# StuLiu/RegDA

Measured on AMD Instinct MI355X. Metric: src+tgt 512x512 image-pairs/sec (SSL step), higher is better.
Workload: dtype bf16; 1 GPU; st.regda.2potsdam SSL step, resnet101 DeepLabV2(PPM), batch 8+8 512x512 per GPU, online EMA teacher; global_batch=8, parallelism=dp1

## Files before the change

### include/rgda_hip.h

```cpp
#ifndef RGDA_HIP_H
#define RGDA_HIP_H

#include <stddef.h>
#include <stdint.h>

#ifdef __cplusplus
extern "C" {
#endif

#define RGDA_ABI_VERSION 10
#define RGDA_STAT_REPLICAS 8
#define RGDA_STAT_FRAC_FWD 26
#define RGDA_STAT_FRAC_BWD 40
typedef int64_t rgda_stat_t;
#define RGDA_LAYOUT_TILE 64

typedef void* rgda_stream_t;

enum rgda_status {
    RGDA_OK = 0,
    RGDA_ERR_ARG = -1,
    RGDA_ERR_WORKSPACE = -2,
    RGDA_ERR_LAUNCH = -3,
    RGDA_ERR_UNSUPPORTED = -4
// ... 5 lines not shown
size_t rgda_class_lds_limit(int which);
const char* rgda_strerror(int status);


size_t rgda_pseudo_select_workspace(int b, int c);
int rgda_pseudo_select(const float* soft, int64_t* out, int b, int c, int hw, float cutoff_top,
                       float cutoff_low, int ignore_label, int classmax_ready, void* ws,
                       size_t ws_bytes, rgda_stream_t stream);

size_t rgda_lrh_workspace(int b, int max_regions, int class_num);
int rgda_lrh(const int64_t* labels, const int64_t* regions, int64_t* out, int b, int hw,
             int class_num, int ignore_label, float percent, int max_regions, void* ws,
             size_t ws_bytes, rgda_stream_t stream);

size_t rgda_pseudo_lrh_workspace(int b, int hw, int max_regions, int class_num);
int rgda_pseudo_lrh(const float* soft, const float* classmax, const int64_t* regions, int64_t* out, int b, int hw,
                    int class_num, float cutoff_top, float cutoff_low, int ignore_label, float percent,
                    int max_regions, void* ws, size_t ws_bytes, rgda_stream_t stream);

int rgda_masks_to_regions(const uint8_t* masks, const int64_t* areas, int32_t* regions, int K, int64_t HW,
                          int64_t area_threshold, rgda_stream_t stream);

size_t rgda_label_refine_workspace(int b, int c, int h, int w);
size_t rgda_label_refine_classmax_offset(int b, int c, int h, int w);
int rgda_label_refine(const float* feat, const float* protos, const float* p1, const float* p2,
                      const float* soft, float* out, int b, int k, int c, int h, int w, int H,
                      int W, float temp, void* ws, size_t ws_bytes, rgda_stream_t stream);
int rgda_label_refine_views(const float* feat, const float* protos, const float* p1, const float* p2,
                            const float* soft, float* out, int b, int k, int c, int h, int w, int H,
                            int W, float temp, int views, void* ws, size_t ws_bytes,
                            rgda_stream_t stream);

size_t rgda_label_refine_sup_workspace(int b, int c, int h, int w, int max_regions);
size_t rgda_label_refine_sup_flag_offset(int b, int c, int h, int w, int max_regions);
int rgda_label_refine_sup(const float* feat, const float* protos, const float* p1, const float* p2,
                          const float* soft, const int64_t* label_t_sup, float* out, int b, int k, int c,
                          int h, int w, int H, int W, float temp, int views, int max_regions, void* ws,
                          size_t ws_bytes, rgda_stream_t stream);

size_t rgda_proto_update_workspace(int c, int k);
int rgda_proto_update(const float* feat, const int64_t* label, float* protos, int64_t* label_ds,
                      int b, int k, int c, int h, int w, int scale, int ignore_label,
                      float min_ratio, float decay, void* ws, size_t ws_bytes,
                      rgda_stream_t stream);
int rgda_proto_stats(const float* feat, const int64_t* label, int64_t* label_ds, int b, int k, int c,
                     int h, int w, int scale, int ignore_label, float min_ratio, void* stats,
                     size_t stats_bytes, rgda_stream_t stream);
int rgda_proto_apply(float* protos, const void* stats, int c, int k, float decay, rgda_stream_t stream);

size_t rgda_upsample_ce_workspace(int b, int c, int h, int w, int H, int W);
int rgda_upsample_ce(const float* p1, const float* p2, const int64_t* label,
                     const float* class_weight, float* loss, float* g1, float* g2, int b, int c,
                     int h, int w, int H, int W, int ignore_label, void* ws, size_t ws_bytes,
                     rgda_stream_t stream);

enum rgda_loss_kind {
    RGDA_LOSS_OHEM = 1,
    RGDA_LOSS_FOCAL = 2,
    RGDA_LOSS_GHM = 3,
    RGDA_LOSS_UPS = 4,
    RGDA_LOSS_UVEM = 5,
    RGDA_LOSS_GDP = 6
};
size_t rgda_upsample_loss_workspace(int kind, int b, int c, int h, int w, int H, int W);
int rgda_upsample_loss(int kind, int heads, const float* p1, const float* p2, const int64_t* label,
                       const float* soft, const float* class_weight, float* acc_sum, double m, double t, double gamma, float thresh,
                       double momentum, float* loss, float* g1, float* g2, int b, int c, int h, int w, int H,
                       int W, int ignore_label, void* ws, size_t ws_bytes, rgda_stream_t stream);

size_t rgda_upsample_gdp_workspace(int b, int c, int h, int w, int H, int W);
int rgda_upsample_gdp(int heads, const float* p1, const float* p2, const int64_t* label,
                      const float* pixel_weight, const float* class_weight, float* acc_sum, float* bins_weight,
                      double momentum, float* loss, float* g1, float* g2, int b, int c, int h, int w, int H,
                      int W, int ignore_label, void* ws, size_t ws_bytes, rgda_stream_t stream);

enum rgda_reg_term { RGDA_REG_ENT = 1, RGDA_REG_KLD = 2 };
size_t rgda_upsample_reg_workspace(int b, int c, int h, int w, int H, int W);
int rgda_upsample_reg(int heads, const float* p1, const float* p2, const int64_t* label, const float* w_ent,
                      const float* w_kld, int terms, float lambda_ent, float lambda_kld, int accumulate,
                      int empty_is_zero, float* loss, float* g1, float* g2, int b, int c, int h, int w, int H, int W,
                      int ignore_label, void* ws, size_t ws_bytes, rgda_stream_t stream);

#define RGDA_IAST_BINS 0x7C01
size_t rgda_iast_workspace(int n, int c, int H, int W);
int rgda_iast_hist(const float* probs, int n, int c, int H, int W, void* ws, size_t ws_bytes, rgda_stream_t stream);
int rgda_iast_percentile(const double* prepend, const double* q, float* out, int c, const void* ws, size_t ws_bytes,
                         rgda_stream_t stream);
int rgda_iast_label(const double* cls_thresh, uint8_t* label, int n, int c, int H, int W, const void* ws,
                    size_t ws_bytes, rgda_stream_t stream);

#define RGDA_ANALYSIS_MAX_BINS 256
size_t rgda_pseudo_analysis_workspace(int b, int c, int R);
int rgda_pseudo_analysis(const float* soft, const int64_t* gt, const float* lo, const float* hi, int b, int c, int H, int W,
                         int R, float cutoff_top, float cutoff_low, int ignore_label, void* tables, size_t tables_bytes,
                         rgda_stream_t stream);
size_t rgda_pseudo_analysis_fold_workspace(int c, int R);
int rgda_pseudo_analysis_fold(const void* tables, size_t tables_bytes, int b, int c, int R, void* state, size_t state_bytes,
                              rgda_stream_t stream);

size_t rgda_proto_pixel_weight_workspace(int b, int c, int k, int h, int w);
int rgda_proto_pixel_weight(const float* feat, const float* protos, const float* sim, const int64_t* label,
                            float* out, int b, int k, int c, int h, int w, int H, int W, int ignore_label,
                            void* ws, size_t ws_bytes, rgda_stream_t stream);

int rgda_teacher_probs(const float* p1, const float* p2, float* probs, int b, int c, int h, int w,
                       int H, int W, rgda_stream_t stream);

int rgda_class_count(const int64_t* label, int32_t* cnt, int64_t n, int c, rgda_stream_t stream);


int rgda_conv2d(const void* x, int ldx, const void* wgt, void* y, int ldy, const void* res,
                int ldres, const uint8_t* res_relu_mask, rgda_stat_t* stats, int stat_groups, int N, int H, int W,
                int Cin, int Ho, int Wo, int Cout, int kh, int kw, int stride, int pad, int dil, int mode,
                rgda_stream_t stream);

typedef struct rgda_conv2d_desc {
    const void* x; const void* wgt; void* y; const void* res; const uint8_t* res_relu_mask; rgda_stat_t* stats;
    int ldx, ldy, ldres, stat_groups;
    int N, H, W, Cin, Ho, Wo, Cout, kh, kw, stride, pad, dil, mode;
} rgda_conv2d_desc;
int rgda_conv2d_grouped(const rgda_conv2d_desc* descs, int n, rgda_stream_t stream);
int rgda_conv2d_grouped_launches(const rgda_conv2d_desc* descs, int n);

int rgda_conv2d_bneval(const void* x, int ldx, const void* wgt, void* y, int ldy, const void* res, int ldres,
                       const float* running_mean, const float* running_var, const float* gamma,
                       const float* beta, float eps, int relu, int N, int H, int W, int Cin, int Ho, int Wo,
                       int Cout, int kh, int kw, int stride, int pad, int dil, rgda_stream_t stream);

int rgda_conv2d_bnbwd(const void* x, int ldx, const void* wgt, void* y, int ldy, const void* res, int ldres,
                      const uint8_t* res_relu_mask, rgda_stat_t* sums, int groups, const void* bn_y, int bn_ldy, const uint8_t* bn_relu_mask,
                      const void* bn_x, int bn_ldx,
                      const float* bn_mi, const float* bn_nscale, int rows_per_image, int relu,
                      const float* bn_gamma, const float* bn_beta, int N, int H,
                      int W, int Cin, int Ho, int Wo, int Cout, int kh, int kw, int stride, int pad, int dil,
                      int mode, rgda_stream_t stream);

typedef struct rgda_bn_operand {
    const rgda_stat_t* stats;
    const float* gamma;
    const float* beta;
    float* mi;
    float* running_mean;
    float* running_var;
    int64_t* num_batches_tracked;
    float eps, momentum;
    int groups;
    int relu;
} rgda_bn_operand;
int rgda_conv2d_bnin_supported(int64_t M, int Cout, int Cin, int kh, int kw, int stride, int pad, int dil, int H, int W,
                               int Ho, int Wo, int groups);
int rgda_conv2d_bnin(const rgda_bn_operand* bn_in, const void* x, int ldx, const void* wgt, void* y, int ldy,
                     const void* res, int ldres, rgda_stat_t* stats, int stat_groups, int N, int H, int W, int Cin,
                     int Ho, int Wo, int Cout, int kh, int kw, int stride, int pad, int dil, rgda_stream_t stream);

const char* rgda_conv2d_kernel(int variant, int N, int H, int W, int Cin, int Ho, int Wo, int Cout, int kh, int kw,
                               int stride, int pad, int dil, int mode, int has_stats, int stat_groups);

int rgda_conv2d_tile(int64_t M, int Cout, int kh, int kw, int Cin, int rows_per_group);

int rgda_conv2d_wgrad(const void* x, int ldx, const void* dy, int lddy, float* dw, int N, int H,
                      int W, int Cin, int Ho, int Wo, int Cout, int kh, int kw, int stride,
                      int pad, int dil, void* ws, size_t ws_bytes, rgda_stream_t stream);

typedef struct rgda_wgrad_desc {
    const void* x;
    const void* dy;
    float* dw;
    int ldx, lddy;
    int N, H, W, Cin, Ho, Wo, Cout, kh, kw, stride, pad, dil;
    int lddw, co_split;
} rgda_wgrad_desc;
size_t rgda_conv2d_wgrad_workspace(const rgda_wgrad_desc* descs, int n);
const char* rgda_conv2d_wgrad_kernel(const rgda_wgrad_desc* desc);
int rgda_conv2d_wgrad_grouped(const rgda_wgrad_desc* descs, int n, void* ws, size_t ws_bytes, rgda_stream_t stream);

int rgda_stem_im2col(const float* img, void* col, int N, int H, int W, int Ho, int Wo, int Kp,
                     rgda_stream_t stream);

int rgda_stem_conv(const float* img, const void* wgt, void* y, int ldy, rgda_stat_t* stats, int stat_groups, int N,
                   int H, int W, int Ho, int Wo, rgda_stream_t stream);
int rgda_stem_conv_bneval(const float* img, const void* wgt, void* y, int ldy, const float* running_mean,
                          const float* running_var, const float* gamma, const float* beta, float eps, int relu,
                          int N, int H, int W, int Ho, int Wo, rgda_stream_t stream);

int rgda_bn_stats(const void* x, int ldx, rgda_stat_t* stats, int64_t M, int C, rgda_stream_t stream);
int rgda_bn_finalize(const rgda_stat_t* stats, float* mi, float* running_mean, float* running_var,
                     int64_t* num_batches_tracked, int64_t M, int C, int groups, float eps,
                     float momentum, rgda_stream_t stream);
int rgda_bn_apply(const void* x, int ldx, const float* mi, const float* gamma, const float* beta,
                  const void* res, int ldres, const float* nscale, int rows_per_image, void* y,
                  int ldy, int64_t M, int C, int relu, int groups, rgda_stream_t stream);
int rgda_bn_train_apply(const void* x, int ldx, const rgda_stat_t* stats, float* mi, float* running_mean,
                        float* running_var, int64_t* num_batches_tracked, const float* gamma,
                        const float* beta, const void* res, int ldres, const float* nscale,
                        int rows_per_image, void* y, int ldy, uint8_t* relu_mask, int64_t M, int C, int relu,
                        int groups, float eps, float momentum, rgda_stream_t stream);
int rgda_bn_bwd_reduce(const void* g, int ldg, const void* y, int ldy, const uint8_t* relu_mask, const void* x,
                       int ldx, const float* mi, const float* nscale, int rows_per_image, rgda_stat_t* sums,
                       int64_t M, int C, int relu, const float* gamma, const float* beta, int groups,
                       rgda_stream_t stream);
int rgda_bn_bwd_apply(const void* g, int ldg, const void* y, int ldy, const uint8_t* relu_mask, const void* x,
                      int ldx, const float* mi, const float* gamma, const float* nscale,
                      int rows_per_image, const rgda_stat_t* sums, void* dx, int lddx, void* gmask,
                      int ldgm, float* dgamma, float* dbeta, int64_t M, int C, int relu, const float* beta,
                      void* act_out, int ldact, int groups, rgda_stream_t stream);

typedef struct rgda_bn_small_fwd_desc {
    const void* x; void* y; uint8_t* relu_mask; const float* gamma; const float* beta; float* mi;
    float* running_mean; float* running_var; int64_t* num_batches_tracked;
    int64_t M; int ldx, ldy, C, groups, relu; float eps, momentum;
} rgda_bn_small_fwd_desc;
typedef struct rgda_bn_small_bwd_desc {
    const void* g; const void* y; const uint8_t* relu_mask; const void* x; void* dx; const float* mi; const float* gamma;
    float* dgamma; float* dbeta;
    int64_t M; int ldg, ldy, ldx, lddx, C, groups, relu;
} rgda_bn_small_bwd_desc;
int rgda_bn_train_small(const rgda_bn_small_fwd_desc* descs, int n, rgda_stream_t stream);
int rgda_bn_bwd_small(const rgda_bn_small_bwd_desc* descs, int n, rgda_stream_t stream);

int rgda_maxpool_fwd(const void* x, void* y, uint8_t* idx, int N, int H, int W, int C, int Ho,
                     int Wo, rgda_stream_t stream);
int rgda_maxpool_bwd(const void* gy, const uint8_t* idx, void* gx, int N, int H, int W, int C,
                     int Ho, int Wo, rgda_stream_t stream);
int rgda_maxpool_fwd_bnin(const rgda_bn_operand* bn_in, const void* x, void* y, uint8_t* idx, int N, int H, int W,
                          int C, int Ho, int Wo, rgda_stream_t stream);

int rgda_instnorm_fwd(const void* x, int ldx, void* y0, void* y1, int ldy, float* feat_nchw,
                      float* mi, int N, int HW, int C, float eps, rgda_stream_t stream);
int rgda_instnorm_bwd(const void* ga, const void* gb, int ldg, const void* gc, int ldgc,
                      const void* x, int ldx, const float* mi, void* dx, int lddx, int N, int HW,
                      int C, rgda_stream_t stream);

int rgda_spatial_mix(const void* in, int ldin, const float* Mx, void* out, int ldout, int N, int I,
                     int J, int C, int accumulate, int out_f32, rgda_stream_t stream);

int rgda_spatial_mix_multi(int nsrc, const void* const* ins, const int* ldins, const float* const* mats,
                           const int* Js, void* out, int ldout, int N, int I, int C, rgda_stream_t stream);

int rgda_classifier_fwd(const void* hidden, int ldh, const float* w, const float* bias,
                        float* logits, int N, int HW, int C, int ncls, rgda_stream_t stream);
size_t rgda_classifier_bwd_workspace(int64_t M, int C, int ncls);
int rgda_classifier_bwd(const void* hidden, int ldh, const float* w, const float* glogits,
                        void* dhidden, int lddh, float* dw, float* db, int N, int HW, int C,
                        int ncls, void* ws, size_t ws_bytes, rgda_stream_t stream);


int rgda_sumsq(const float* g, int64_t n, float* out, float* ws, rgda_stream_t stream);

int rgda_sgd_step(float* p, const float* g, float* v, float* shadow, void* p_bf16, void* shadow_bf16,
                  const float* gnorm_sq, const float* lr_dev, int64_t n, float momentum,
                  float weight_decay, float max_norm, float gscale, float ema_decay,
                  int first_step, rgda_stream_t stream);

size_t rgda_stem_wgrad_workspace(int N, int H, int W);
int rgda_stem_wgrad(const float* img, const void* dy, int lddy, float* dw, void* ws, size_t ws_bytes, int N, int H,
                    int W, int Ho, int Wo, rgda_stream_t stream);

int rgda_weight_transpose_bf16(const float* w, void* wt, int Co, int T, int Ci, rgda_stream_t stream);
int rgda_weight_transpose_batched(const int64_t* table, int n, int64_t total_blocks, rgda_stream_t stream);
int rgda_cast_bf16(const float* src, void* dst, int64_t n, rgda_stream_t stream);
int rgda_cast_f32(const void* src_bf16, float* dst, int64_t n, rgda_stream_t stream);
int rgda_ddp_accumulate_bf16(const void* recv, int world, void* out, int64_t shard_elems, rgda_stream_t stream);

typedef void* rgda_comm_t;
#define RGDA_COMM_ID_BYTES 128
#define RGDA_COMM_F32 0
#define RGDA_COMM_BF16 1
#define RGDA_COMM_I64 2
#define RGDA_COMM_F64 3
int rgda_comm_unique_id(void* id_128_bytes);
int rgda_comm_init(const void* id_128_bytes, int rank, int world, rgda_comm_t* comm);
int rgda_comm_destroy(rgda_comm_t comm);
int rgda_comm_all_reduce(rgda_comm_t comm, void* buf, int64_t n, int dtype, rgda_stream_t stream);
int rgda_comm_all_gather(rgda_comm_t comm, const void* send, void* recv, int64_t n_per_rank, int dtype,
                         rgda_stream_t stream);
int rgda_comm_all_to_all(rgda_comm_t comm, const void* send, void* recv, int64_t n_per_rank, int dtype,
                         rgda_stream_t stream);
int rgda_pad_cast_bf16(const float* src, void* dst, int R, int K, int Kp, rgda_stream_t stream);
int rgda_unpad_acc_f32(const float* src, float* dst, int R, int K, int Kp, rgda_stream_t stream);
int rgda_fill_zero(void* p, size_t bytes, rgda_stream_t stream);
int rgda_copy_multi(int n, void* const* dsts, const void* const* srcs, const size_t* bytes, rgda_stream_t stream);
int rgda_set_f32(float* p, float value, rgda_stream_t stream);
int rgda_dropout_mask(float* out, int64_t n, float p, uint64_t seed, rgda_stream_t stream);
int rgda_add_bf16(const void* a, int lda, const void* b, int ldb, void* out, int ldo, int64_t M,
                  int C, rgda_stream_t stream);


int rgda_dihedral_nchw(const float* src, float* dst, int N, int C, int Hs, int Ws, int hflip, int rot_k,
                       int flip_first, float scale, int accumulate, rgda_stream_t stream);

int rgda_pad_rows_nchw(const float* src, float* dst, int N, int C, int h, int w, int top, int bottom,
                       rgda_stream_t stream);
int rgda_window_crop(const float* full, float* tile, int N, int C, int Hf, int Wf, int y1, int x1, int h, int w,
                     int Th, int Tw, rgda_stream_t stream);
int rgda_window_accumulate(const float* tile, float* full, float* count, int N, int C, int Hf, int Wf, int y1,
                           int x1, int h, int w, int Th, int Tw, rgda_stream_t stream);
int rgda_window_normalise(float* full, const float* count, int N, int C, int Hf, int Wf, rgda_stream_t stream);

int rgda_window_gather(const float* src_f32, const uint8_t* src_u8, const float* lut, const int32_t* windows, int K,
                       int views, int n, int C, int H, int W, int Th, int Tw, float* out, int* flag,
                       rgda_stream_t stream);
int rgda_window_scatter(const float* pred, const int32_t* windows, int K, int views, int n, int C, int H, int W, int Th,
                        int Tw, int row0, int rows, float* full, float* count, int* flag, rgda_stream_t stream);
int rgda_window_finish(float* full, const float* count, int n, int C, int H, int W, uint8_t* labels_u8,
                       int64_t* labels_i64, const int64_t* y_true, int64_t* cm, int* flag, rgda_stream_t stream);

// ... 193 lines not shown
```

### regda_amd/csrc/common.h

```cpp
#pragma once
#include <hip/hip_runtime.h>
#include <stdint.h>

#include "../../include/rgda_hip.h"

#define RGDA_CHECK_LAUNCH()                                   \
    do {                                                      \
        if (hipGetLastError() != hipSuccess) return RGDA_ERR_LAUNCH; \
    } while (0)

typedef unsigned short bf16_t;
typedef __attribute__((ext_vector_type(8))) __bf16 bf16x8;
typedef __attribute__((ext_vector_type(8))) unsigned short u16x8;
typedef __attribute__((ext_vector_type(4))) unsigned short u16x4;
typedef __attribute__((ext_vector_type(4))) short s16x4;
typedef __attribute__((ext_vector_type(16))) float f32x16;
typedef __attribute__((ext_vector_type(4))) float f32x4;

typedef __attribute__((ext_vector_type(2))) __bf16 bf16x2_t;
typedef __attribute__((ext_vector_type(2))) float f32x2_t;
static __device__ __forceinline__ float bf2f(bf16_t h) { return __uint_as_float(((unsigned)h) << 16); }
static __device__ __forceinline__ unsigned pack2bf(float lo, float hi) {
    f32x2_t v = {lo, hi};
    bf16x2_t b = __builtin_convertvector(v, bf16x2_t);
    return __builtin_bit_cast(unsigned, b);
}
static __device__ __forceinline__ bf16_t f2bf(float f) { return (bf16_t)(pack2bf(f, 0.f) & 0xffffu); }

static __device__ __forceinline__ float wave_sum(float v) {
#pragma unroll
    for (int o = 32; o > 0; o >>= 1) v += __shfl_xor(v, o, 64);
    return v;
}
template <int O>
static __device__ __forceinline__ float xor_add(float v) {
    static_assert(O == 8 || O == 16 || O == 32, "xor_add: 8, 16 or 32");
    const unsigned u = __float_as_uint(v);
    if constexpr (O == 8) {
        return v + __uint_as_float((unsigned)__builtin_amdgcn_update_dpp(0, (int)u, 0x128 , 0xf, 0xf, false));
    } else if constexpr (O == 16) {
        auto r = __builtin_amdgcn_permlane16_swap(u, u, false, false);
        return __uint_as_float(r[0]) + __uint_as_float(r[1]);
    } else {
        auto r = __builtin_amdgcn_permlane32_swap(u, u, false, false);
        return __uint_as_float(r[0]) + __uint_as_float(r[1]);
    }
}

struct Lerp {
    int i0, i1;
    float l0, l1;
};
static __device__ __forceinline__ Lerp lerp_ac(int dst, int in, int out) {
    float scale = (out > 1) ? __fdiv_rn((float)(in - 1), (float)(out - 1)) : 0.f;
    float src = __fmul_rn(scale, (float)dst);
    Lerp r;
    r.i0 = (int)src;
    r.i1 = r.i0 + ((r.i0 < in - 1) ? 1 : 0);
    r.l1 = __fsub_rn(src, (float)r.i0);
    r.l0 = __fsub_rn(1.f, r.l1);
    return r;
}

static __device__ __forceinline__ float wave_max(float v) {
#pragma unroll
    for (int o = 32; o > 0; o >>= 1) v = fmaxf(v, __shfl_xor(v, o, 64));
    return v;
}

#define NREP RGDA_STAT_REPLICAS

#define RGDA_STAT_POISON (3ll << 60)
static __device__ __forceinline__ long long stat_fix(float v, int frac) {
    const float x = ldexpf(v, frac);
    if (!(fabsf(x) < 0x1p59f)) return RGDA_STAT_POISON;
    const float hi = truncf(x * 0x1p-31f);
    const float lo = x - hi * 0x1p31f;
    return ((long long)__float2int_rz(hi) << 31) + (long long)__float2int_rn(lo);
}
static __device__ __forceinline__ void stat_add(rgda_stat_t* p, float v, int frac) {
    atomicAdd((unsigned long long*)p, (unsigned long long)stat_fix(v, frac));
}
static __device__ __forceinline__ double stat_total(const rgda_stat_t* __restrict__ st, int C, int c, int which, int frac) {
    __int128 t = 0;
#pragma unroll
    for (int r = 0; r < NREP; ++r) t += st[(size_t)(2 * r + which) * C + c];
    if (t >= (__int128)(1ll << 59) || t <= -(__int128)(1ll << 59)) return (double)__builtin_nan("");
    return (double)(long long)t * (1.0 / (double)(1ll << frac));
}

static __device__ __forceinline__ void stat_moments(const rgda_stat_t* __restrict__ st, int C, int c, double invM, float eps,
                                                    float& mean, float& var, float& istd) {
    const double m = stat_total(st, C, c, 0, RGDA_STAT_FRAC_FWD) * invM;
    double v = stat_total(st, C, c, 1, RGDA_STAT_FRAC_FWD) * invM - m * m;
    if (v < 0.0) v = 0.0;
    mean = (float)m;
    var = (float)v;
    istd = 1.f / sqrtf((float)v + eps);
}

struct BnOperand {
    const rgda_stat_t* stats;
    const float* gamma;
    const float* beta;
    float* mi;
    float* rm;
    float* rv;
    long long* nbt;
    float eps, mom;
    int groups, relu, C;
    int rows_per_group;
};
static __device__ __forceinline__ void bn_scale_shift(float mean, float istd, float gamma, float beta, float& sc, float& sh) {
    sc = gamma * istd;
    sh = __builtin_fmaf(-mean, sc, beta);
}
static __device__ __forceinline__ float bn_affine(float x, float sc, float sh) { return __builtin_fmaf(x, sc, sh); }
typedef float f32x2v __attribute__((ext_vector_type(2)));
static __device__ __forceinline__ uint4 bn_operand8(uint4 v, const float (&sc)[8], const float (&sh)[8], bool relu) {
    unsigned w[4] = {v.x, v.y, v.z, v.w};
#pragma unroll
    for (int e = 0; e < 4; ++e) {
        f32x2v x = {__uint_as_float(w[e] << 16), __uint_as_float(w[e] & 0xffff0000u)};
        f32x2v s = {sc[2 * e], sc[2 * e + 1]}, h = {sh[2 * e], sh[2 * e + 1]};
        f32x2v f = __builtin_elementwise_fma(x, s, h);
        if (relu) { f.x = fmaxf(f.x, 0.f); f.y = fmaxf(f.y, 0.f); }
        w[e] = pack2bf(f.x, f.y);
    }
    return uint4{w[0], w[1], w[2], w[3]};
}
template <int NT>
static __device__ __forceinline__ void bn_operand_table(const BnOperand& b, int grp, bool leader, float* tab) {
    const int C = b.C;
    const double invM = 1.0 / (double)b.rows_per_group;
    for (int c = threadIdx.x; c < C; c += NT) {
        float mean, var, istd, sc, sh;
        stat_moments(b.stats + (size_t)grp * NREP * 2 * C, C, c, invM, b.eps, mean, var, istd);
        bn_scale_shift(mean, istd, b.gamma[c], b.beta[c], sc, sh);
        tab[c] = sc;
        tab[C + c] = sh;
        if (leader) {
            const float unb = (b.rows_per_group > 1) ? (float)b.rows_per_group / (float)(b.rows_per_group - 1) : 1.f;
            float rm = b.rm ? b.rm[c] : 0.f, rv = b.rm ? b.rv[c] : 0.f;
            for (int g = 0; g < b.groups; ++g) {
                float gm, gv, gi;
                stat_moments(b.stats + (size_t)g * NREP * 2 * C, C, c, invM, b.eps, gm, gv, gi);
                if (b.mi) { b.mi[(size_t)g * 2 * C + c] = gm; b.mi[(size_t)g * 2 * C + C + c] = gi; }
                rm = (1.f - b.mom) * rm + b.mom * gm;
                rv = (1.f - b.mom) * rv + b.mom * gv * unb;
            }
            if (b.rm) { b.rm[c] = rm; b.rv[c] = rv; }
            if (c == 0 && b.nbt) *b.nbt += b.groups;
        }
    }
}

#include <stdlib.h>
#ifdef RGDA_TUNING
#define TUNE_ENV(name) getenv(name)
#else
#define TUNE_ENV(name) ((const char*)nullptr)
#endif
static inline hipStream_t to_stream(rgda_stream_t s) { return (hipStream_t)s; }
static inline int zero_bytes(void* p, size_t bytes, rgda_stream_t stream) {
    if (!((uintptr_t)p & 15)) return rgda_fill_zero(p, bytes, stream);
    return hipMemsetAsync(p, 0, bytes, (hipStream_t)stream) == hipSuccess ? RGDA_OK : RGDA_ERR_LAUNCH;
}
static inline int cdiv(long long a, long long b) { return (int)((a + b - 1) / b); }

#include <type_traits>
#define RGDA_MIN_CLASSES 6
#define RGDA_MAX_CLASSES 16
static inline bool class_count_ok(int c) { return c >= RGDA_MIN_CLASSES && c <= RGDA_MAX_CLASSES; }
size_t loss_row_lds_bytes(int c, int w, int W, bool want);
size_t pcl_lds_bytes(int C, int K);
size_t refine_lds_bytes(int C, int k);
#define RGDA_LOSS_ROW_LDS_MAX ((size_t)150 * 1024)
#define RGDA_LDS_MAX ((size_t)160 * 1024)
template <int LO = RGDA_MIN_CLASSES, int HI = RGDA_MAX_CLASSES, class F>
static inline int with_classes(int c, F&& f) {
    if constexpr (LO > HI) {
        return RGDA_ERR_UNSUPPORTED;
    } else {
        if (c == LO) return f(std::integral_constant<int, LO>{});
        return with_classes<LO + 1, HI>(c, f);
    }
}
```

### regda_amd/csrc/conv_kernels.hip

```cpp
#include <stdio.h>
#include <stdlib.h>
#include <string.h>

#include "common.h"
#include <type_traits>
#include <vector>

struct ConvArgs {
    const bf16_t* x;
    const bf16_t* w;
    bf16_t* y;
    const bf16_t* res;
    rgda_stat_t* stats;
    int ldx, ldy, ldres;
    int N, H, W, Cin, Ho, Wo, Cout, KH, KW, stride, pad, dil, mode;
    int M;
    int tiles_c, tiles_p;
    int rows_per_group;
    int howo_shift, wo_shift;
    unsigned long long* dbg;
    int tpw;
    int skip;
    const unsigned char* res_mask;
    const bf16_t* bn_y;
    const unsigned char* bn_mask;
    const bf16_t* bn_x;
    const float* bn_mi;
    const float* bn_nscale;
    int bn_ldy, bn_ldx, bn_rpi, bn_relu;
    const float* ev_rm;
    const float* ev_rv;
    const float* ev_gamma;
    const float* ev_beta;
    float ev_eps;
    int ev_relu;
    const float* bn_gamma;
    const float* bn_beta;
    BnOperand xf;
};

#ifdef RGDA_TUNING
#define TDBG(a) ((a).dbg)
#define TSKIP(a) ((a).skip)
#else
#define TDBG(a) ((unsigned long long*)nullptr)
#define TSKIP(a) 0
#endif

static __device__ __forceinline__ int xcd_remap(int bid, int nwg) {
    int q = nwg >> 3, r = nwg & 7, xcd = bid & 7, k = bid >> 3;
    return (xcd < r ? xcd * (q + 1) : r * (q + 1) + (xcd - r) * q) + k;
}

static __device__ __forceinline__ void src_coord(int mode, int base, int t, int dil, int stride, int lim, int& out,
                                                 bool& ok) {
    if (mode == 0) {
        out = base + t * dil;
        ok = (out >= 0) && (out < lim);
    } else {
        int th = base - t * dil;
        ok = th >= 0;
        if (stride == 1) {
            out = th;
        } else {
            ok = ok && (th % stride == 0);
            out = th / stride;
        }
        ok = ok && (out < lim);
    }
}

#define LDS_PTR(p) ((__attribute__((address_space(3))) void*)(p))
#define WAIT_VMCNT(n) asm volatile("s_waitcnt vmcnt(%0)" ::"n"(n) : "memory")

typedef __attribute__((ext_vector_type(4))) int i32x4;
static __device__ __forceinline__ i32x4 dma_rsrc(const void* base, unsigned bytes) {
    const unsigned long long b = (unsigned long long)base;
    i32x4 r = {(int)(unsigned)b, (int)((unsigned)(b >> 32) & 0xffffu), (int)bytes, 0x00020000};
    return r;
}
static __device__ __forceinline__ void dma16_to_lds(i32x4 rsrc, const unsigned char* lds_dst, int voffset, int soffset) {
    const unsigned m0 = (unsigned)(__UINTPTR_TYPE__)LDS_PTR(lds_dst);
    asm volatile("s_mov_b32 m0, %0\n\ts_nop 0\n\tbuffer_load_dwordx4 %1, %2, %3 offen lds"
                 :: "s"(m0), "v"(voffset), "s"(rsrc), "s"(soffset) : "memory");
}


enum { EPI_PLAIN = 0, EPI_STATS, EPI_RES, EPI_RES_STATS, EPI_EV, EPI_BNX, EPI_BNX2 };
typedef float f32x2 __attribute__((ext_vector_type(2)));
typedef __attribute__((ext_vector_type(4))) unsigned u32x4r;
#define RGDA_BNIN_MAX_C 512
static __device__ __forceinline__ f32x2 bf2f_pair(unsigned u) {
    f32x2 r;
    r.x = __uint_as_float(u << 16);
    r.y = __uint_as_float(u & 0xffff0000u);
    return r;
}
static __device__ __forceinline__ unsigned pack2bf(f32x2 v) { return pack2bf(v.x, v.y); }

struct EpiParams { f32x2 k0[4], k1[4], k2[4], k3[4]; };
template <int KIND>
static __device__ __forceinline__ void epilogue_params(const ConvArgs& a, int m0, int co, bool cok, EpiParams& P) {
#pragma unroll
    for (int e = 0; e < 4; ++e) {
        P.k0[e] = f32x2{0.f, 0.f}; P.k1[e] = f32x2{0.f, 0.f};
        P.k2[e] = f32x2{0.f, 0.f}; P.k3[e] = f32x2{0.f, 0.f};
    }
    constexpr bool BNX = KIND == EPI_BNX || KIND == EPI_BNX2;
    if (BNX && cok) {
        const float* mi = a.bn_mi + (size_t)(m0 / a.rows_per_group) * 2 * a.Cout + co;
#pragma unroll
        for (int e = 0; e < 4; ++e) {
            P.k1[e] = f32x2{mi[2 * e], mi[2 * e + 1]};
            P.k0[e] = f32x2{mi[a.Cout + 2 * e], mi[a.Cout + 2 * e + 1]};
        }
        if constexpr (KIND == EPI_BNX2) {
#pragma unroll
            for (int e = 0; e < 8; ++e) {
                float sc, sh;
                bn_scale_shift(P.k1[e >> 1][e & 1], P.k0[e >> 1][e & 1], a.bn_gamma[co + e], a.bn_beta[co + e], sc, sh);
                P.k2[e >> 1][e & 1] = sc;
                P.k3[e >> 1][e & 1] = sh;
            }
        }
    }
    if (KIND == EPI_EV && cok) {
#pragma unroll
        for (int e = 0; e < 8; ++e) {
            const float sc = a.ev_gamma[co + e] / sqrtf(a.ev_rv[co + e] + a.ev_eps);
            P.k0[e >> 1][e & 1] = sc;
            P.k1[e >> 1][e & 1] = a.ev_beta[co + e] - a.ev_rm[co + e] * sc;
        }
    }
}

template <int WMAP>
static __device__ __forceinline__ int tile_row(const ConvArgs& a, int row) {
    return WMAP ? ((row >> 5) * a.W + (row & 31)) : row;
}
template <int BC, int BP, int NT, int KIND, bool FULL = false, int WMAP = 0>
static __device__ __forceinline__ void epilogue_rows(const ConvArgs& a, const unsigned char* smem, int m0, int c0,
                                                     float (&s)[8], float (&q)[8], const EpiParams* pre = nullptr) {
    constexpr int CSTR = BC * 2 + 16;
    constexpr int VPR = BC / 8, RPP = NT / VPR, NIT = BP / RPP;
    constexpr int CH = NIT < 4 ? NIT : 4;
    static_assert(NIT % CH == 0, "row passes");
    const int t = threadIdx.x;
    const int cv = t % VPR, rr = t / VPR;
    const int co = c0 + cv * 8;
    const bool cok = FULL || co < a.Cout;
    EpiParams P;
    if (pre) P = *pre; else epilogue_params<KIND>(a, m0, co, cok, P);
    f32x2 (&k0)[4] = P.k0, (&k1)[4] = P.k1, (&k2)[4] = P.k2, (&k3)[4] = P.k3;
    f32x2 s2[4], q2[4];
#pragma unroll
    for (int e = 0; e < 4; ++e) { s2[e] = f32x2{s[2 * e], s[2 * e + 1]}; q2[e] = f32x2{q[2 * e], q[2 * e + 1]}; }
    constexpr bool BNX = KIND == EPI_BNX || KIND == EPI_BNX2;
    const bool has_res = (KIND == EPI_RES || KIND == EPI_RES_STATS) || ((KIND == EPI_EV || BNX) && a.res);
    const bool res_gate = (KIND != EPI_EV) && has_res && a.res_mask;
    constexpr bool STATS = KIND == EPI_STATS || KIND == EPI_RES_STATS;
#pragma unroll
    for (int p0 = 0; p0 < NIT; p0 += CH) {
        uint4 val[CH], rv[CH], xv[CH], yv[CH];
        unsigned rmb[CH], bmb[CH];
        bool ok[CH];
#pragma unroll
        for (int i = 0; i < CH; ++i) {
            const int row = rr + (p0 + i) * RPP;
            const int m = m0 + tile_row<WMAP>(a, row);
            ok[i] = FULL || (cok && m < a.M);
            val[i] = *(const uint4*)(smem + row * CSTR + cv * 16);
            rv[i] = uint4{0u, 0u, 0u, 0u}; xv[i] = rv[i]; yv[i] = rv[i]; rmb[i] = 0xffu; bmb[i] = 0xffu;
            if (ok[i]) {
                if (has_res) {
                    rv[i] = *(const uint4*)(a.res + (size_t)m * a.ldres + co);
                    if (res_gate) rmb[i] = a.res_mask[(size_t)m * (a.Cout >> 3) + (co >> 3)];
                }
                if (BNX) {
                    xv[i] = *(const uint4*)(a.bn_x + (size_t)m * a.bn_ldx + co);
                    if (KIND == EPI_BNX && a.bn_relu) {
                        if (a.bn_mask) bmb[i] = a.bn_mask[(size_t)m * (a.Cout >> 3) + (co >> 3)];
                        else yv[i] = *(const uint4*)(a.bn_y + (size_t)m * a.bn_ldy + co);
                    }
                }
            }
        }
#pragma unroll
        for (int i = 0; i < CH; ++i) {
            const int m = m0 + tile_row<WMAP>(a, rr + (p0 + i) * RPP);
            const unsigned vw[4] = {val[i].x, val[i].y, val[i].z, val[i].w};
            const unsigned rw[4] = {rv[i].x, rv[i].y, rv[i].z, rv[i].w};
            unsigned ow[4];
            if (KIND == EPI_PLAIN || KIND == EPI_STATS) {
#pragma unroll
                for (int e = 0; e < 4; ++e) ow[e] = vw[e];
            } else if (KIND == EPI_EV) {
#pragma unroll
                for (int e = 0; e < 4; ++e) {
                    f32x2 f = bf2f_pair(vw[e]) * k0[e] + k1[e];
                    if (has_res) f += bf2f_pair(rw[e]);
                    if (a.ev_relu) { f.x = fmaxf(f.x, 0.f); f.y = fmaxf(f.y, 0.f); }
                    ow[e] = pack2bf(f);
                }
            } else {
#pragma unroll
                for (int e = 0; e < 4; ++e) {
                    unsigned r = rw[e];
                    if (res_gate) {
                        const unsigned b0 = (rmb[i] >> (2 * e)) & 1u, b1 = (rmb[i] >> (2 * e + 1)) & 1u;
                        r &= (b0 ? 0x0000ffffu : 0u) | (b1 ? 0xffff0000u : 0u);
                    }
                    ow[e] = has_res ? pack2bf(bf2f_pair(vw[e]) + bf2f_pair(r)) : vw[e];
                }
            }
            if (ok[i]) {
                if (STATS) {
#pragma unroll
                    for (int e = 0; e < 4; ++e) {
                        const f32x2 f = bf2f_pair(ow[e]);
                        s2[e] += f;
                        q2[e] += f * f;
                    }
                }
                if (BNX) {
                    const unsigned xw[4] = {xv[i].x, xv[i].y, xv[i].z, xv[i].w};
                    const unsigned yw[4] = {yv[i].x, yv[i].y, yv[i].z, yv[i].w};
                    f32x2 ns[4];
#pragma unroll
                    for (int e = 0; e < 4; ++e) ns[e] = f32x2{1.f, 1.f};
                    if (a.bn_nscale) {
                        const float* np = a.bn_nscale + (size_t)(m / a.bn_rpi) * a.Cout + co;
#pragma unroll
                        for (int e = 0; e < 4; ++e) ns[e] = f32x2{np[2 * e], np[2 * e + 1]};
                    }
#pragma unroll
                    for (int e = 0; e < 4; ++e) {
                        f32x2 g = bf2f_pair(ow[e]);
                        if constexpr (KIND == EPI_BNX2) {
                            const f32x2 xx = bf2f_pair(xw[e]);
                            g.x = (bn_affine(xx.x, k2[e].x, k3[e].x) > 0.f) ? g.x : 0.f;
                            g.y = (bn_affine(xx.y, k2[e].y, k3[e].y) > 0.f) ? g.y : 0.f;
                        } else if (a.bn_relu) {
                            if (a.bn_mask) {
                                g.x = ((bmb[i] >> (2 * e)) & 1u) ? g.x : 0.f;
                                g.y = ((bmb[i] >> (2 * e + 1)) & 1u) ? g.y : 0.f;
                            } else {
                                const f32x2 yy = bf2f_pair(yw[e]);
                                g.x = (yy.x > 0.f) ? g.x : 0.f;
                                g.y = (yy.y > 0.f) ? g.y : 0.f;
                            }
                        }
                        if (a.bn_nscale) g *= ns[e];
                        s2[e] += g;
                        q2[e] += g * ((bf2f_pair(xw[e]) - k1[e]) * k0[e]);
                    }
                }
                if (!(TSKIP(a) & 128)) *(uint4*)(a.y + (size_t)m * a.ldy + co) = uint4{ow[0], ow[1], ow[2], ow[3]};
            }
        }
    }
#pragma unroll
    for (int e = 0; e < 4; ++e) { s[2 * e] = s2[e].x; s[2 * e + 1] = s2[e].y; q[2 * e] = q2[e].x; q[2 * e + 1] = q2[e].y; }
}

template <int BC, int BP, int WC, int WP, bool RAW = false, int KIND = -1, int WMAP = 0>
static __device__ __forceinline__ void conv_epilogue(const ConvArgs& a, f32x16 (&acc)[BC / WC / 32][BP / WP / 32],
                                                     unsigned char* smem, int m0, int c0, float (&s)[8], float (&q)[8],
                                                     bool flush, int replica, const EpiParams* pre = nullptr) {
    constexpr int NW = WC * WP, NT = 64 * NW;
    constexpr int FI = BC / WC / 32, FJ = BP / WP / 32;
    constexpr int CSTR = BC * 2 + 16;
    const int t = threadIdx.x, lane = t & 63;
    const int wave = __builtin_amdgcn_readfirstlane(t >> 6);
    const int wc = wave % WC, wp = wave / WC;
    const int lrow = lane & 31, lk = lane >> 5;
#pragma unroll
    for (int i = 0; i < FI; ++i)
#pragma unroll
        for (int j = 0; j < FJ; ++j) {
            int px = wp * (BP / WP) + j * 32 + lrow;
#pragma unroll
            for (int g = 0; g < 4; ++g) {
                int co = wc * (BC / WC) + i * 32 + 8 * g + 4 * lk;
                uint2 pk;
                pk.x = pack2bf(acc[i][j][4 * g + 0], acc[i][j][4 * g + 1]);
                pk.y = pack2bf(acc[i][j][4 * g + 2], acc[i][j][4 * g + 3]);
                *(uint2*)(smem + px * CSTR + co * 2) = pk;
            }
        }
    if constexpr (RAW) {
        asm volatile("s_waitcnt lgkmcnt(0)" ::: "memory");
        __builtin_amdgcn_s_barrier();
    } else {
        __syncthreads();
    }
    if (TDBG(a) && t == 0) TDBG(a)[(16384 + blockIdx.x) * 4 + 0] = __builtin_readcyclecounter();
    constexpr int VPR = BC / 8;
    const int cv = t % VPR;
    if constexpr (KIND >= 0) epilogue_rows<BC, BP, NT, KIND, RAW, WMAP>(a, smem, m0, c0, s, q, pre);
    else if (a.ev_rm) epilogue_rows<BC, BP, NT, EPI_EV, false, WMAP>(a, smem, m0, c0, s, q);
    else if (a.bn_x) {
        if (a.bn_relu == 2) epilogue_rows<BC, BP, NT, EPI_BNX2, false, WMAP>(a, smem, m0, c0, s, q);
        else epilogue_rows<BC, BP, NT, EPI_BNX, false, WMAP>(a, smem, m0, c0, s, q);
    }
    else if (a.res) {
        if (a.stats) epilogue_rows<BC, BP, NT, EPI_RES_STATS, false, WMAP>(a, smem, m0, c0, s, q);
        else epilogue_rows<BC, BP, NT, EPI_RES, false, WMAP>(a, smem, m0, c0, s, q);
    } else if (a.stats) epilogue_rows<BC, BP, NT, EPI_STATS, false, WMAP>(a, smem, m0, c0, s, q);
    else epilogue_rows<BC, BP, NT, EPI_PLAIN, false, WMAP>(a, smem, m0, c0, s, q);
    if (TDBG(a) && t == 0) TDBG(a)[(16384 + blockIdx.x) * 4 + 1] = __builtin_readcyclecounter();
    if (a.stats && flush) {
#pragma unroll
        for (int e = 0; e < 8; ++e) {
            if constexpr (VPR <= 8) { s[e] = xor_add<8>(s[e]); q[e] = xor_add<8>(q[e]); }
            if constexpr (VPR <= 16) { s[e] = xor_add<16>(s[e]); q[e] = xor_add<16>(q[e]); }
            if constexpr (VPR <= 32) { s[e] = xor_add<32>(s[e]); q[e] = xor_add<32>(q[e]); }
        }
        float* red = (float*)(smem + BP * CSTR);
        if (lane < VPR) {
#pragma unroll
            for (int e = 0; e < 8; ++e) {
                red[(wave * 2 + 0) * BC + cv * 8 + e] = s[e];
                red[(wave * 2 + 1) * BC + cv * 8 + e] = q[e];
            }
        }
        asm volatile("s_waitcnt lgkmcnt(0)" ::: "memory");
        __builtin_amdgcn_s_barrier();
        if (TDBG(a) && t == 0) TDBG(a)[(16384 + blockIdx.x) * 4 + 2] = __builtin_readcyclecounter();
        if (t < 2 * BC) {
            int which = t / BC, c = t % BC;
            float tot = 0.f;
#pragma unroll
            for (int wv = 0; wv < NW; ++wv) tot += red[(wv * 2 + which) * BC + c];
            if (c0 + c < a.Cout) {
                rgda_stat_t* dst = &a.stats[(((size_t)(m0 / a.rows_per_group) * NREP + replica) * 2 + which) * a.Cout + c0 + c];
#ifdef RGDA_TUNING
                if (TSKIP(a) & 16) {}
                else if (TSKIP(a) & 32) atomicAdd((float*)dst, tot);
                else
#endif
                stat_add(dst, tot, a.bn_x ? RGDA_STAT_FRAC_BWD : RGDA_STAT_FRAC_FWD);
            }
        }
    }
}

template <int BC, int BP, int STAGES, int WC, int WP, bool PIPE, bool XF>
static __device__ __forceinline__ void conv_igemm_body(const ConvArgs& a, const int bid) {
#if defined(__HIP_DEVICE_COMPILE__)
    constexpr int NW = WC * WP;
    constexpr int FI = BC / WC / 32, FJ = BP / WP / 32;
    constexpr int WL = BC / (NW * 8), XL = BP / (NW * 8);
    constexpr int LD = WL + XL;
    constexpr int TILE = (BC + BP) * 128;
    constexpr int CSTR = BC * 2 + 16;
    constexpr int EPI = BP * CSTR + NW * BC * 2 * 4;
    constexpr int SMEM = (STAGES * TILE > EPI) ? STAGES * TILE : EPI;
    constexpr int XFTAB = XF ? RGDA_BNIN_MAX_C * 2 * 4 : 0;
    static_assert(!XF || (STAGES == 2 && !PIPE), "the operand-transform loop is written for the 2-stage ring");
    __shared__ __attribute__((aligned(256))) unsigned char smem[SMEM + XFTAB];

    const int t = threadIdx.x, lane = t & 63;
    const int wave = __builtin_amdgcn_readfirstlane(t >> 6);
    const int wc = wave % WC, wp = wave / WC;
    const int logical = xcd_remap(bid, a.tiles_c * a.tiles_p);
    const int c0 = (logical % a.tiles_c) * BC;
    const int m0 = (logical / a.tiles_c) * BP;
    const int taps = a.KH * a.KW;
    const int lrow8 = lane >> 3, lslot = lane & 7;
    constexpr int OOB = (int)0x80000000;
    const __amdgpu_buffer_rsrc_t rs_w = __builtin_amdgcn_make_buffer_rsrc(
        (void*)a.w, 0, (int)((size_t)a.Cout * taps * a.Cin * 2), 0x00020000);
    const __amdgpu_buffer_rsrc_t rs_x = __builtin_amdgcn_make_buffer_rsrc(
        (void*)a.x, 0, (int)((((size_t)a.N * a.H * a.W - 1) * a.ldx + a.Cin) * 2), 0x00020000);

    int xn[XL], xh[XL], xw[XL], xsw[XL];
    bool xm[XL];
#pragma unroll
    for (int i = 0; i < XL; ++i) {
        int r = (i * NW + wave) * 8 + lrow8;
        int m = m0 + r;
        xm[i] = m < a.M;
        int mm = xm[i] ? m : 0;
        int n, rem, ho, wo;
        if (a.howo_shift >= 0) { n = mm >> a.howo_shift; rem = mm & ((1 << a.howo_shift) - 1); }
        else { n = mm / (a.Ho * a.Wo); rem = mm % (a.Ho * a.Wo); }
        if (a.wo_shift >= 0) { ho = rem >> a.wo_shift; wo = rem & ((1 << a.wo_shift) - 1); }
        else { ho = rem / a.Wo; wo = rem % a.Wo; }
        xn[i] = n * a.H * a.W;
        if (a.mode == 0) { xh[i] = ho * a.stride - a.pad; xw[i] = wo * a.stride - a.pad; }
        else             { xh[i] = ho + a.pad;            xw[i] = wo + a.pad; }
        xsw[i] = XF ? lslot * 16 : (lslot ^ ((r >> 1) & 7)) * 16;
    }
    int wvo[WL];
#pragma unroll
    for (int i = 0; i < WL; ++i) {
        int r = (i * NW + wave) * 8 + lrow8;
        int co = c0 + r;
        wvo[i] = (co < a.Cout) ? (co * taps * a.Cin * 2 + (lslot ^ ((r >> 1) & 7)) * 16) : OOB;
    }

    int tap = 0, kh = 0, kw = 0, ci0 = 0;
    int xvo[XL];
    auto retap = [&]() {
#pragma unroll
        for (int i = 0; i < XL; ++i) {
            int hi, wi;
            bool okh, okw;
            src_coord(a.mode, xh[i], kh, a.dil, a.stride, a.H, hi, okh);
            src_coord(a.mode, xw[i], kw, a.dil, a.stride, a.W, wi, okw);
            xvo[i] = (xm[i] && okh && okw) ? ((xn[i] + hi * a.W + wi) * a.ldx * 2 + xsw[i]) : OOB;
        }
    };
    retap();
    auto issue = [&](int stage) {
        unsigned char* wb = smem + stage * TILE + wave * 1024;
        const int so_w = (tap * a.Cin + ci0) * 2, so_x = ci0 * 2;
#pragma unroll
        for (int i = 0; i < WL; ++i)
            __builtin_amdgcn_raw_ptr_buffer_load_lds(rs_w, LDS_PTR(wb + i * NW * 1024), 16, wvo[i], so_w, 0, 0);
        unsigned char* xb = wb + BC * 128;
#pragma unroll
        for (int i = 0; i < XL; ++i)
            __builtin_amdgcn_raw_ptr_buffer_load_lds(rs_x, LDS_PTR(xb + i * NW * 1024), 16, xvo[i], so_x, 0, 0);
    };
    auto advance = [&]() {
        ci0 += 64;
        if (ci0 >= a.Cin) {
            ci0 = 0;
            ++tap;
            if (++kw == a.KW) { kw = 0; ++kh; }
            retap();
        }
    };

    f32x16 acc[FI][FJ];
#pragma unroll
    for (int i = 0; i < FI; ++i)
#pragma unroll
        for (int j = 0; j < FJ; ++j)
#pragma unroll
            for (int r = 0; r < 16; ++r) acc[i][j][r] = 0.f;

    const int KT = taps * (a.Cin >> 6);
    unsigned long long tq0 = 0, tq1 = 0, tq2 = 0, twait = 0, tbar = 0;
    if (TDBG(a)) tq0 = __builtin_readcyclecounter();
    const int lrow = lane & 31, lk = lane >> 5;
    int stage = 0;
    if constexpr (XF) {
        float* xtab = (float*)(smem + SMEM);
        auto issue_w = [&](int st) {
            unsigned char* wb = smem + st * TILE + wave * 1024;
// ... 360 lines not shown
        for (int k = 0; k < PXW; ++k) xf_piece(0, k);
    }
    int pend = 2, wstage = 0;
    bf16x8 fa0[2][FI], fb0[2][FJ], fa1[2][FI], fb1[2][FJ];
    if constexpr (PF) {
        WAIT_VMCNT(2 * (NS - 2));
        if constexpr (XF) asm volatile("s_waitcnt lgkmcnt(0)" ::: "memory");
        __builtin_amdgcn_s_barrier();
        read_half(swb, sxb, 0, 0, fa0, fb0);
    }
    if constexpr (PF) {
      for (int sl = 0; sl < S; ++sl) {
        const bool more = sl + 1 < S;
        const unsigned char* xb = sxb + (sl & 1) * XS;
        const unsigned char* xbn = sxb + ((sl + 1) & 1) * XS;
#pragma unroll
        for (int tp = 0; tp < 9; ++tp) {
            const int q = sl * 9 + tp;
            if (!(TSKIP(a) & 2)) { if (tp >= 1 && tp - 1 < PXW) WAIT_VMCNT(2 * (NS - 3) + 1); else WAIT_VMCNT(2 * (NS - 3)); }
            if constexpr (XF) asm volatile("s_waitcnt lgkmcnt(0)" ::: "memory");
            if (!(TSKIP(a) & 4)) __builtin_amdgcn_s_barrier();
            if (!(TSKIP(a) & 1)) {
            issue_w2((tp + AH) % 9, sl + (tp + AH) / 9, wstage >= 1 ? wstage - 1 : NS - 1, q + AH < KT);
            if (tp < PXW) issue_h(sl + 1, tp, more);
            }
            if constexpr (XF) {
                if (more) {
                    if (tp == 1) xf_load(sl + 1);
                    if (tp >= 2 && tp - 2 < PXW) xf_piece(sl + 1, tp - 2);
                }
            }
            read_half(swb + wstage * WS, xb, tp, 1, fa1, fb1);
            mfma_half(fa0, fb0);
            read_half(swb + (wstage == NS - 1 ? 0 : wstage + 1) * WS, tp == 8 ? xbn : xb, tp == 8 ? 0 : tp + 1, 0, fa0, fb0);
            mfma_half(fa1, fb1);
#pragma unroll
            for (int i = 0; i < 4 * FI * FJ; ++i) {
                __builtin_amdgcn_sched_group_barrier(0x008, 1, 0);
                __builtin_amdgcn_sched_group_barrier(0x100, (FI + FJ + FI * FJ - 1) / (FI * FJ), 0);
            }
            wstage = (wstage == NS - 1) ? 0 : wstage + 1;
        }
      }
    } else {
    for (int sl = 0; sl < S; ++sl) {
        const bool more = sl + 1 < S;
        const unsigned char* xb = sxb + (sl & 1) * XS;
#pragma unroll
        for (int tp = 0; tp < 9; ++tp) {
            const int q = sl * 9 + tp;
            switch (pend) {
                case 0: WAIT_VMCNT(0); break;
                case 1: WAIT_VMCNT(1); break;
                case 2: WAIT_VMCNT(2); break;
                default: WAIT_VMCNT(3); break;
            }
            if constexpr (XF) asm volatile("s_waitcnt lgkmcnt(0)" ::: "memory");
            __builtin_amdgcn_s_barrier();
            pend = 0;
            if (!(TSKIP(a) & 1)) {
            if (q + 2 < KT) { issue_w(q + 2, wstage >= 1 ? wstage - 1 : 2); pend += 2; }
            if (more && tp < PXW) { issue_h(sl + 1, tp); pend += 1; }
            }
            if constexpr (XF) {
                if (more && !(TSKIP(a) & 512)) {
                    if (tp == 1) xf_load(sl + 1);
                    if (tp >= 2 && tp - 2 < PXW) xf_piece(sl + 1, tp - 2);
                }
            }
            const unsigned char* wb = swb + wstage * WS;
            if (!(TSKIP(a) & 8) || q == 0) {
            read_half(wb, xb, tp, 0, fa0, fb0);
            read_half(wb, xb, tp, 1, fa1, fb1);
            }
            mfma_half(fa0, fb0);
            mfma_half(fa1, fb1);
            wstage = (wstage == NS - 1) ? 0 : wstage + 1;
        }
    }
    }
    __syncthreads();
    float s[8], q8[8];
#pragma unroll
    for (int e = 0; e < 8; ++e) { s[e] = 0.f; q8[e] = 0.f; }
    conv_epilogue<BC, BP, WC, WP, false, -1, WIDE ? 1 : 0>(a, acc, smem, m0, c0, s, q8, true, blockIdx.x & (NREP - 1));
#endif
}
template <int D, int TR, bool XF = false, int NS = 3, bool PF = (NS == 4)>
__global__ void __launch_bounds__(512) conv3x3_halo_kernel(ConvArgs a) {
    conv3x3_halo_body<D, TR, XF, NS, PF, false>(a);
}
template <int D, int TR, int NS = 3, bool PF = (NS == 4), bool XF = false>
__global__ void __launch_bounds__(512) conv3x3_halo_wide_kernel(ConvArgs a) {
    conv3x3_halo_body<D, TR, XF, NS, PF, true>(a);
}

template <int KC, int BP, int WC, int WP, int KIND>
__global__ void __launch_bounds__(512) conv1x1_stream_kernel(ConvArgs a) {
#if defined(__HIP_DEVICE_COMPILE__)
    constexpr int BC = 128, NW = 8, FI = BC / WC / 32, NS = 2;
    static_assert(WC * WP == NW && BP / WP == 32, "one 32-pixel fragment column per wave");
    constexpr int XL = BP / (NW * 8);
    constexpr int SUB = BP * 128;
    constexpr int STAGE = KC * SUB;
    constexpr int CSTR = BC * 2 + 16;
    constexpr int EPI = BP * CSTR + NW * BC * 2 * 4;
    constexpr int SC = BP * BC * 2 / 16 / (64 * NW);
    __shared__ __attribute__((aligned(256))) unsigned char smem[NS * STAGE + EPI];
    unsigned char* se = smem + NS * STAGE;

    const int t = threadIdx.x, lane = t & 63;
    const int wave = __builtin_amdgcn_readfirstlane(t >> 6);
    const int wc = wave % WC, wp = wave / WC;
    const int lrow = lane & 31, lk = lane >> 5;
    const int lrow8 = lane >> 3, lslot = lane & 7;
    const int logical = xcd_remap(blockIdx.x, gridDim.x);
    const int c0 = (logical % a.tiles_c) * BC;
    const int T = a.tpw;
    const int mbase = (logical / a.tiles_c) * T * BP;

    bf16x8 fa[KC * 4][FI];
#pragma unroll
    for (int i = 0; i < FI; ++i) {
        const bf16_t* wrow = a.w + (size_t)(c0 + wc * (BC / WC) + i * 32 + lrow) * a.Cin + lk * 8;
#pragma unroll
        for (int kk = 0; kk < KC * 4; ++kk) fa[kk][i] = *(const bf16x8*)(wrow + kk * 16);
    }
#pragma unroll
    for (int i = 0; i < FI; ++i)
#pragma unroll
        for (int kk = 0; kk < KC * 4; ++kk) asm volatile("" ::"v"(fa[kk][i]));
    const i32x4 rs_x = dma_rsrc(a.x, (unsigned)((((size_t)a.M - 1) * a.ldx + a.Cin) * 2));
    int xvo[XL];
#pragma unroll
    for (int i = 0; i < XL; ++i) {
        const int r = (i * NW + wave) * 8 + lrow8;
        xvo[i] = r * a.ldx * 2 + (lslot ^ ((r >> 1) & 7)) * 16;
    }
    auto issue = [&](int tile, int stage) {
        const int so = (mbase + tile * BP) * a.ldx * 2;
#pragma unroll
        for (int kt = 0; kt < KC; ++kt)
#pragma unroll
            for (int i = 0; i < XL; ++i)
                dma16_to_lds(rs_x, smem + stage * STAGE + kt * SUB + (i * NW + wave) * 1024, xvo[i], so + kt * 128);
    };
    float s[8], q[8];
#pragma unroll
    for (int e = 0; e < 8; ++e) { s[e] = 0.f; q[e] = 0.f; }
    EpiParams P;
    epilogue_params<KIND>(a, mbase, c0 + (t % (BC / 8)) * 8, true, P);
#pragma unroll
    for (int e = 0; e < 4; ++e) asm volatile("" ::"v"(P.k0[e]), "v"(P.k1[e]), "v"(P.k2[e]), "v"(P.k3[e]));
    issue(0, 0);
    if (T > 1) { issue(1, 1); WAIT_VMCNT(XL * KC); } else WAIT_VMCNT(0);
    for (int i = 0; i < T; ++i) {
        const int stage = i & 1;
        __builtin_amdgcn_s_barrier();
        f32x16 acc[FI][1];
#pragma unroll
        for (int ii = 0; ii < FI; ++ii)
#pragma unroll
            for (int r = 0; r < 16; ++r) acc[ii][0][r] = 0.f;
        const int rb = wp * 32 + lrow;
        const unsigned char* xb = smem + stage * STAGE + rb * 128;
#pragma unroll
        for (int kt = 0; kt < KC; ++kt) {
            bf16x8 fb[4];
#pragma unroll
            for (int kk = 0; kk < 4; ++kk) fb[kk] = *(const bf16x8*)(xb + kt * SUB + (((kk * 2 + lk) ^ ((rb >> 1) & 7)) << 4));
#pragma unroll
            for (int kk = 0; kk < 4; ++kk)
#pragma unroll
                for (int ii = 0; ii < FI; ++ii)
                    acc[ii][0] = __builtin_amdgcn_mfma_f32_32x32x16_bf16(fa[kt * 4 + kk][ii], fb[kk], acc[ii][0], 0, 0, 0);
        }
        conv_epilogue<BC, BP, WC, WP, true, KIND>(a, acc, se, mbase + i * BP, c0, s, q, i + 1 == T, blockIdx.x & (NREP - 1), &P);
        __builtin_amdgcn_s_waitcnt(SC | (7 << 4) | (15 << 8));
        if (i + 2 < T && !(TSKIP(a) & 1)) issue(i + 2, stage);
    }
#endif
}

template <int TW, int KIND>
__global__ void __launch_bounds__(512) conv3x3_c64_kernel(ConvArgs a) {
#if defined(__HIP_DEVICE_COMPILE__)
    constexpr int BC = 64, BP = TW, WC = 2, WP = 4, NW = 8;
    constexpr int HP = TW + 2;
    constexpr int RI = (HP + 7) / 8;
    constexpr int SLOT = RI * 1024;
    constexpr int WBYTES = 9 * BC * 128;
    constexpr int CSTR = BC * 2 + 16;
    constexpr int EPI = BP * CSTR + NW * BC * 2 * 4;
    constexpr int SC = BP / (64 * NW / (BC / 8));
    __shared__ __attribute__((aligned(256))) unsigned char smem[WBYTES + 3 * SLOT + EPI];
    unsigned char* sw = smem;
    unsigned char* sr = smem + WBYTES;
    unsigned char* se = sr + 3 * SLOT;

    const int t = threadIdx.x, lane = t & 63;
    const int wave = __builtin_amdgcn_readfirstlane(t >> 6);
    const int wc = wave % WC, wp = wave / WC;
    const int lrow = lane & 31, lk = lane >> 5;
    const int lrow8 = lane >> 3, lslot = lane & 7;
    const int rpw = a.tpw;
    const int strip = blockIdx.x;
    const int row0 = strip * rpw;
    const int n = row0 / a.H, y0 = row0 % a.H;
    constexpr int OOB = (int)0x80000000;
    const i32x4 rs_w = dma_rsrc(a.w, 64 * 9 * 64 * 2);
    const i32x4 rs_x = dma_rsrc(a.x, (unsigned)((((size_t)a.N * a.H * a.W - 1) * a.ldx + a.Cin) * 2));
#pragma unroll
    for (int j = 0; j < 9; ++j) {
        const int r = (j * NW + wave) * 8 + lrow8;
        const int tap = r / BC, co = r % BC;
        const int vo = (co * 9 + tap) * 128 + (lslot ^ ((r >> 1) & 7)) * 16;
        dma16_to_lds(rs_w, sw + (j * NW + wave) * 1024, vo, 0);
    }
    int rvo[(RI + NW - 1) / NW];
#pragma unroll
    for (int i = 0; i < (RI + NW - 1) / NW; ++i) {
        const int q = i * NW + wave;
        const int hp = q * 8 + lrow8, ix = hp - 1;
        rvo[i] = (q < RI && hp < HP && ix >= 0 && ix < a.W) ? (ix * a.ldx * 2 + (lslot ^ ((hp >> 1) & 7)) * 16) : OOB;
    }
    auto issue_row = [&](int y) {
        const bool inside = y >= 0 && y < a.H;
        const int so = inside ? ((n * a.H + y) * a.W) * a.ldx * 2 : 0;
        unsigned char* rb = sr + ((y + 1) % 3) * SLOT;
#pragma unroll
        for (int i = 0; i < (RI + NW - 1) / NW; ++i) {
            const int q = i * NW + wave;
            if (q < RI)
                dma16_to_lds(rs_x, rb + q * 1024, inside ? rvo[i] : OOB, so);
        }
    };
    issue_row(y0 - 1);
    issue_row(y0);
    issue_row(y0 + 1);
    float s[8], q8[8];
#pragma unroll
    for (int e = 0; e < 8; ++e) { s[e] = 0.f; q8[e] = 0.f; }
    EpiParams P;
    epilogue_params<KIND>(a, row0 * BP, (t % (BC / 8)) * 8, true, P);
#pragma unroll
    for (int e = 0; e < 4; ++e) asm volatile("" ::"v"(P.k0[e]), "v"(P.k1[e]), "v"(P.k2[e]), "v"(P.k3[e]));
    WAIT_VMCNT(0);
    for (int ty = 0; ty < rpw; ++ty) {
        const int y = y0 + ty;
        __builtin_amdgcn_s_barrier();
        f32x16 acc[1][1];
#pragma unroll
        for (int r = 0; r < 16; ++r) acc[0][0][r] = 0.f;
        const int px = wp * 32 + lrow;
        const int ra = wc * 32 + lrow;
#pragma unroll
        for (int wr = 0; wr < 3; ++wr) {
            const unsigned char* rb = sr + ((y + wr) % 3) * SLOT;
            const int kh = (a.mode == 0) ? wr : 2 - wr;
#pragma unroll
            for (int kw = 0; kw < 3; ++kw) {
                const int hp = px + ((a.mode == 0) ? kw : 2 - kw);
                const unsigned char* wb = sw + (kh * 3 + kw) * (BC * 128);
#pragma unroll
                for (int kk = 0; kk < 4; ++kk) {
                    const bf16x8 fa = *(const bf16x8*)(wb + ra * 128 + (((kk * 2 + lk) ^ ((ra >> 1) & 7)) << 4));
                    const bf16x8 fb = *(const bf16x8*)(rb + hp * 128 + (((kk * 2 + lk) ^ ((hp >> 1) & 7)) << 4));
                    acc[0][0] = __builtin_amdgcn_mfma_f32_32x32x16_bf16(fa, fb, acc[0][0], 0, 0, 0);
                }
            }
            if (wr == 0) {
                asm volatile("s_waitcnt lgkmcnt(0)" ::: "memory");
                __builtin_amdgcn_s_barrier();
                if (ty + 1 < rpw) issue_row(y + 2);
            }
        }
        const int m0 = (row0 + ty) * BP;
        conv_epilogue<BC, BP, WC, WP, true, KIND>(a, acc, se, m0, 0, s, q8, ty + 1 == rpw, blockIdx.x & (NREP - 1), &P);
        __builtin_amdgcn_s_waitcnt(SC | (7 << 4) | (15 << 8));
    }
#endif
}

#ifdef RGDA_TUNING
#define TUNING_ONLY(...) __VA_ARGS__
#else
#define TUNING_ONLY(...)
#endif
#define CONV_IGEMM_ROUTES(T)                                                                                         \
    T(64, 64, 2, 2, 2, false, false) T(128, 64, 3, 2, 2, true, false) T(128, 128, 2, 2, 4, false, false)             \
    T(128, 128, 3, 2, 4, true, false) T(128, 256, 3, 2, 4, true, false) T(128, 128, 2, 2, 4, false, true)            \
    TUNING_ONLY(T(128, 128, 3, 2, 4, false, false) T(128, 256, 3, 2, 4, false, false) T(128, 64, 3, 2, 2, false, false) \
                T(128, 256, 3, 2, 2, false, false) T(256, 128, 3, 2, 2, false, false) T(128, 128, 2, 2, 2, false, false) \
                T(128, 128, 4, 2, 2, false, false) T(128, 128, 3, 2, 2, false, false) T(128, 64, 2, 2, 2, false, false) \
                T(128, 64, 4, 2, 2, false, false) T(64, 128, 3, 2, 2, false, false) T(64, 64, 4, 2, 2, false, false) \
                T(64, 64, 3, 2, 2, false, false))
#define IGEMM_ID(BC, BP, ST, WC, WP, PIPE, XF) R_IGEMM_##BC##x##BP##_##ST##_##WC##x##WP##_##PIPE##_##XF
#define IGEMM_ROUTE(BC, BP, ST, WC, WP, PIPE, XF)                                                                    \
    ROUTE(IGEMM_ID(BC, BP, ST, WC, WP, PIPE, XF), 64 * WC * WP, conv_igemm_kernel, BC, BP, ST, WC, WP, PIPE, XF)
#define PER_EPI_ROUTES(ID, KERNEL, ...)                                                                              \
    ROUTE(ID##0, 512, KERNEL, __VA_ARGS__, 0) ROUTE(ID##1, 512, KERNEL, __VA_ARGS__, 1)                              \
    ROUTE(ID##2, 512, KERNEL, __VA_ARGS__, 2) ROUTE(ID##3, 512, KERNEL, __VA_ARGS__, 3)                              \
    ROUTE(ID##4, 512, KERNEL, __VA_ARGS__, 4) ROUTE(ID##5, 512, KERNEL, __VA_ARGS__, 5)                              \
    ROUTE(ID##6, 512, KERNEL, __VA_ARGS__, 6)
#define CONV_ROUTES                                                                                                  \
    CONV_IGEMM_ROUTES(IGEMM_ROUTE)                                                                                   \
    ROUTE(R_HALO_1_4, 512, conv3x3_halo_kernel, 1, 4, false, 4, true)                                                \
    ROUTE(R_HALO_1_8, 512, conv3x3_halo_kernel, 1, 8, false, 4, true)                                                \
    ROUTE(R_HALO_2_8, 512, conv3x3_halo_kernel, 2, 8, false, 3, true)                                                \
    ROUTE(R_HALO_1_4_XF, 512, conv3x3_halo_kernel, 1, 4, true, 4, true)                                              \
    ROUTE(R_HALO_1_8_XF, 512, conv3x3_halo_kernel, 1, 8, true, 3, false)                                             \
    TUNING_ONLY(ROUTE(R_HALO_1_4_PLAIN, 512, conv3x3_halo_kernel, 1, 4, false, 3, false)                             \
                ROUTE(R_HALO_1_8_PLAIN, 512, conv3x3_halo_kernel, 1, 8, false, 3, false)                             \
                ROUTE(R_HALO_2_8_PLAIN, 512, conv3x3_halo_kernel, 2, 8, false, 3, false)                             \
                ROUTE(R_HALO_1_4_XF_PLAIN, 512, conv3x3_halo_kernel, 1, 4, true, 3, false))                          \
    ROUTE(R_HALOW_1_4, 512, conv3x3_halo_wide_kernel, 1, 4, 4, true, false)                                          \
    ROUTE(R_HALOW_1_8, 512, conv3x3_halo_wide_kernel, 1, 8, 4, true, false)                                          \
    ROUTE(R_HALOW_2_8, 512, conv3x3_halo_wide_kernel, 2, 8, 3, true, false)                                          \
    ROUTE(R_HALOW_1_4_XF, 512, conv3x3_halo_wide_kernel, 1, 4, 4, true, true)                                        \
    ROUTE(R_HALOW_1_8_XF, 512, conv3x3_halo_wide_kernel, 1, 8, 3, false, true)                                       \
    PER_EPI_ROUTES(R_C64_, conv3x3_c64_kernel, 128)                                                                  \
    PER_EPI_ROUTES(R_STREAM1_, conv1x1_stream_kernel, 1, 128, 2, 4)                                                  \
    PER_EPI_ROUTES(R_STREAM2_, conv1x1_stream_kernel, 2, 128, 2, 4)
#define ROUTE(ID, BLOCK, KERNEL, ...) ID,
enum { CONV_ROUTES CONV_ROUTE_COUNT };
#undef ROUTE
#define ROUTE(ID, BLOCK, KERNEL, ...) #KERNEL "<" #__VA_ARGS__ ">",
static const char* const CONV_ROUTE_NAMES[CONV_ROUTE_COUNT] = {CONV_ROUTES};
#undef ROUTE
constexpr int R_GROUPED = IGEMM_ID(128, 64, 3, 2, 2, true, false);

static int conv_launch(int route, const ConvArgs& a, int grid, hipStream_t st) {
    switch (route) {
#define ROUTE(ID, BLOCK, KERNEL, ...) case ID: KERNEL<__VA_ARGS__><<<grid, BLOCK, 0, st>>>(a); break;
        CONV_ROUTES
#undef ROUTE
    }
    RGDA_CHECK_LAUNCH();
    return RGDA_OK;
}

static inline int tune_int(const char* name, int dflt) { const char* e = TUNE_ENV(name); return e ? atoi(e) : dflt; }

static int conv_use_halo(long long M, int Cout, int Cin, int kh, int kw, int stride, int pad, int dil, int H, int W, int Ho,
                         int Wo, int rows_per_group) {
    if (const char* e = TUNE_ENV("RGDA_HALO")) { if (!atoi(e)) return 0; }
    if (kh != 3 || kw != 3 || stride != 1 || pad != dil || (dil != 1 && dil != 2)) return 0;
    if ((W & 31) || Wo != W || Ho != H || (Cin & 63)) return 0;
    const int min_tiles = tune_int("RGDA_HALO_MIN", 100), min8 = tune_int("RGDA_HALO_MIN8", 100);
    if ((long long)9 * Cin >= 4096 && !(H & 7) && !(rows_per_group % (8 * W)) && (M / 256) * cdiv(Cout, 128) >= min8) return 8;
    if ((long long)9 * Cin >= 2048 && dil == 1 && !(H & 3) && !(rows_per_group % (4 * W)) && (M / 128) * cdiv(Cout, 128) >= min_tiles) return 4;
    return 0;
}

struct ConvTile { int bc, bp, stages, wc, wp; bool pipe; };

static int pick_tile(long long M, int Cout, long long ktot, int rows_per_group, ConvTile& t) {
    t.bc = (Cout <= 64) ? 64 : 128;
    t.bp = 64;
    t.wc = 2;
    bool waves8 = false, ring3 = false;
    const int t82 = tune_int("RGDA_T82", 512), t83 = tune_int("RGDA_T83", 256);
    if (t.bc == 128 && ktot >= 4096 && (long long)cdiv(M, 256) * cdiv(Cout, t.bc) >= 240) { t.bp = 256; waves8 = true; }
    else if (t.bc == 128 && (long long)cdiv(M, 128) * cdiv(Cout, t.bc) >= t82) { t.bp = 128; waves8 = true; }
    else if (t.bc == 128 && (long long)cdiv(M, 128) * cdiv(Cout, t.bc) >= t83) { t.bp = 128; waves8 = ring3 = true; }
    if (rows_per_group) {
        while (t.bp > 64 && (rows_per_group % t.bp)) t.bp >>= 1;
        if (rows_per_group % t.bp) return 1;
    }
    t.wp = (waves8 && t.bp >= 128) ? 4 : 2;
    t.stages = (t.wp == 4) ? ((t.bp == 256 || ring3) ? 3 : 2) : ((t.bc == 64) ? 2 : 3);
    t.pipe = t.stages == 3 && !TUNE_ENV("RGDA_NO_PIPE");
    return 0;
}

static int igemm_route(const ConvTile& t) {
#define TILE(BC, BP, ST, WC, WP, PIPE, XF)                                                                           \
    if (!XF && t.bc == BC && t.bp == BP && t.stages == ST && t.wc == WC && t.wp == WP && t.pipe == PIPE)             \
        return IGEMM_ID(BC, BP, ST, WC, WP, PIPE, XF);
    CONV_IGEMM_ROUTES(TILE)
#undef TILE
    return -1;
}

extern "C" int rgda_conv2d_tile(int64_t M, int Cout, int kh, int kw, int Cin, int rows_per_group) {
    ConvTile t;
    if (pick_tile(M, Cout, (long long)kh * kw * Cin, rows_per_group, t)) return RGDA_ERR_UNSUPPORTED;
    return t.bc | (t.bp << 10) | ((t.wp == 4 ? 80 + t.stages : t.stages) << 20);
}

static int ilog2_exact(int v) {
    if (v <= 0 || (v & (v - 1))) return -1;
    int s = 0;
    while ((1 << s) < v) ++s;
    return s;
}
struct BnBwdFuse { const void* y; int ldy; const unsigned char* mask; const void* x; int ldx; const float* mi; const float* nscale; int rpi; int relu; const float* gamma; const float* beta; };
struct BnEvalFuse { const float* rm; const float* rv; const float* gamma; const float* beta; float eps; int relu; };
struct ConvFuse { const BnBwdFuse* bnb; const BnEvalFuse* bne; const rgda_bn_operand* bnin; };

static int conv_bnin_kind(long long M, int Cout, int Cin, int kh, int kw, int stride, int pad, int dil, int H, int W, int Ho,
                          int Wo, int groups) {
    if (groups < 1 || Ho <= 0 || Wo <= 0 || (M % ((long long)Ho * Wo)) || (M / ((long long)Ho * Wo)) % groups ||
        Cin > RGDA_BNIN_MAX_C || (Cin & 63))
        return 0;
    const int rpg = (int)(M / groups);
    if (const int tr = conv_use_halo(M, Cout, Cin, kh, kw, stride, pad, dil, H, W, Ho, Wo, rpg))
        return (tr == 4) ? 1 : (dil == 1 ? 2 : 0);
    ConvTile t;
    if (pick_tile(M, Cout, (long long)kh * kw * Cin, rpg, t)) return 0;
    return (t.bc == 128 && t.bp == 128 && t.wp == 4 && t.stages == 2) ? 3 : 0;
}

extern "C" int rgda_conv2d_bnin_supported(int64_t M, int Cout, int Cin, int kh, int kw, int stride, int pad, int dil, int H,
                                          int W, int Ho, int Wo, int groups) {
    if (!conv_bnin_kind(M, Cout, Cin, kh, kw, stride, pad, dil, H, W, Ho, Wo, groups)) return 0;
    return (Cin > 256 || (kh == 1 && Cin < 128)) ? 1 : 2;
}

static int conv_epi_kind(const ConvArgs& a) {
    return a.ev_rm ? EPI_EV : a.bn_x ? (a.bn_relu == 2 ? EPI_BNX2 : EPI_BNX)
         : a.res ? (a.stats ? EPI_RES_STATS : EPI_RES) : (a.stats ? EPI_STATS : EPI_PLAIN);
}

struct ConvPlan { ConvArgs a; int route, grid; };
static int conv_select(const rgda_conv2d_desc& d, const ConvFuse& f, ConvPlan& p) {
    const int N = d.N, H = d.H, W = d.W, Cin = d.Cin, Ho = d.Ho, Wo = d.Wo, Cout = d.Cout, kh = d.kh, kw = d.kw,
              stride = d.stride, pad = d.pad, dil = d.dil, mode = d.mode;
    const BnBwdFuse* bnb = f.bnb;
    const BnEvalFuse* bne = f.bne;
    const rgda_bn_operand* bnin = f.bnin;
    if (!d.x || !d.wgt || !d.y) return RGDA_ERR_ARG;
    if (N <= 0 || H <= 0 || W <= 0 || Ho <= 0 || Wo <= 0 || Cin <= 0 || Cout <= 0 || kh <= 0 || kw <= 0 ||
        stride <= 0 || dil <= 0 || pad < 0 || (mode != 0 && mode != 1))
        return RGDA_ERR_ARG;
    if ((Cin & 63) || (Cout & 7) || (d.ldx & 7) || (d.ldy & 7) || (d.res && (d.ldres & 7)) || d.ldx < Cin || d.ldy < Cout)
        return RGDA_ERR_ARG;
    ConvArgs& a = p.a = ConvArgs{};
    a.x = (const bf16_t*)d.x; a.w = (const bf16_t*)d.wgt; a.y = (bf16_t*)d.y; a.res = (const bf16_t*)d.res; a.stats = d.stats;
    if (d.res_relu_mask && (!d.res || bne)) return RGDA_ERR_ARG;
    a.res_mask = d.res_relu_mask;
    a.ldx = d.ldx; a.ldy = d.ldy; a.ldres = d.ldres;
    a.N = N; a.H = H; a.W = W; a.Cin = Cin; a.Ho = Ho; a.Wo = Wo; a.Cout = Cout; a.KH = kh; a.KW = kw;
    a.stride = stride; a.pad = pad; a.dil = dil; a.mode = mode;
    long long M = (long long)N * Ho * Wo;
    if (M > 0x7fffffffLL) return RGDA_ERR_ARG;
    a.M = (int)M;
    a.howo_shift = ilog2_exact(Ho * Wo);
    a.wo_shift = ilog2_exact(Wo);
    const int stat_groups = d.stat_groups < 1 ? 1 : d.stat_groups;
    if (N % stat_groups || M % stat_groups) return RGDA_ERR_ARG;
    a.rows_per_group = (int)(M / stat_groups);
    if (bnb) {
        if (!a.stats || !bnb->x || !bnb->mi || (bnb->relu == 1 && !bnb->y && !bnb->mask) || (bnb->ldx & 7) ||
            (bnb->relu == 1 && bnb->y && (bnb->ldy & 7)) || (bnb->nscale && bnb->rpi <= 0) || bnb->relu < 0 || bnb->relu > 2)
            return RGDA_ERR_ARG;
        a.bn_mask = bnb->relu == 1 ? bnb->mask : nullptr;
        a.bn_y = (const bf16_t*)bnb->y; a.bn_x = (const bf16_t*)bnb->x; a.bn_mi = bnb->mi; a.bn_nscale = bnb->nscale;
        a.bn_ldy = bnb->ldy; a.bn_ldx = bnb->ldx; a.bn_rpi = bnb->rpi; a.bn_relu = bnb->relu;
        if (bnb->relu == 2 && (!bnb->gamma || !bnb->beta)) return RGDA_ERR_ARG;
        a.bn_gamma = bnb->gamma; a.bn_beta = bnb->beta;
    }
    if (bne) {
        if (!bne->rm || !bne->rv || !bne->gamma || !bne->beta || a.stats) return RGDA_ERR_ARG;
        a.ev_rm = bne->rm; a.ev_rv = bne->rv; a.ev_gamma = bne->gamma; a.ev_beta = bne->beta; a.ev_eps = bne->eps;
        a.ev_relu = bne->relu;
    }
    if (const char* e = TUNE_ENV("RGDA_CONV_DBG")) a.dbg = (unsigned long long*)strtoull(e, nullptr, 0);
    a.skip = tune_int("RGDA_CONV_SKIP", 0);
    if (bnin) {
        if (mode != 0 || bne || bnb || !bnin->stats || !bnin->gamma || !bnin->beta || bnin->groups != stat_groups ||
            ((long long)N * H * W) % bnin->groups || (bnin->running_mean == nullptr) != (bnin->running_var == nullptr))
            return RGDA_ERR_ARG;
        if ((long long)N * H * W / bnin->groups < 2) return RGDA_ERR_ARG;
        const int kind = conv_bnin_kind(M, Cout, Cin, kh, kw, stride, pad, dil, H, W, Ho, Wo, stat_groups);
        if (!kind) return RGDA_ERR_UNSUPPORTED;
        a.xf.stats = bnin->stats; a.xf.gamma = bnin->gamma; a.xf.beta = bnin->beta; a.xf.mi = bnin->mi;
        a.xf.rm = bnin->running_mean; a.xf.rv = bnin->running_var; a.xf.nbt = (long long*)bnin->num_batches_tracked;
        a.xf.eps = bnin->eps; a.xf.mom = bnin->momentum; a.xf.groups = bnin->groups; a.xf.relu = bnin->relu; a.xf.C = Cin;
        a.xf.rows_per_group = (int)((long long)N * H * W / bnin->groups);
        a.tiles_c = cdiv(Cout, 128);
        if (kind == 3) {
            a.tiles_p = cdiv(M, 128);
            p.route = IGEMM_ID(128, 128, 2, 2, 4, false, true);
        } else {
            a.tiles_p = (int)(M / ((kind == 1 ? 4 : 8) * 32));
            if (W != 32) p.route = kind == 1 ? R_HALOW_1_4_XF : R_HALOW_1_8_XF;
            else p.route = kind == 1 ? R_HALO_1_4_XF : R_HALO_1_8_XF;
#ifdef RGDA_TUNING
            if (const char* e = TUNE_ENV("RGDA_HALO_NS")) { if (atoi(e) != 4 && W == 32 && kind == 1) p.route = R_HALO_1_4_XF_PLAIN; }
#endif
        }
        p.grid = a.tiles_c * a.tiles_p;
        return RGDA_OK;
    }
    if (tune_int("RGDA_C64", 1) && kh == 3 && kw == 3 && stride == 1 && pad == 1 && dil == 1 && Cin == 64 && Cout == 64 && W == 128 &&
        Wo == W && Ho == H && !(a.rows_per_group % (H * W))) {
        int rpw = (int)((long long)N * H / 256);
        while (rpw > 1 && (H % rpw)) --rpw;
        if (rpw >= 2) {
            a.tpw = rpw;
            a.tiles_c = 1;
            a.tiles_p = N * H;
            p.route = R_C64_0 + conv_epi_kind(a);
            p.grid = N * H / rpw;
            return RGDA_OK;
        }
    }
    if (const int tr = conv_use_halo(M, Cout, Cin, kh, kw, stride, pad, dil, H, W, Ho, Wo, a.rows_per_group)) {
        a.tiles_c = cdiv(Cout, 128);
        a.tiles_p = (int)(M / (tr * 32));
        if (W != 32) p.route = tr == 4 ? R_HALOW_1_4 : dil == 1 ? R_HALOW_1_8 : R_HALOW_2_8;
        else p.route = tr == 4 ? R_HALO_1_4 : dil == 1 ? R_HALO_1_8 : R_HALO_2_8;
#ifdef RGDA_TUNING
        if (const char* e = TUNE_ENV("RGDA_HALO_NS")) {
            if (atoi(e) != 4 && W == 32) p.route = tr == 4 ? R_HALO_1_4_PLAIN : dil == 1 ? R_HALO_1_8_PLAIN : R_HALO_2_8_PLAIN;
        }
#endif
        p.grid = a.tiles_c * a.tiles_p;
        return RGDA_OK;
    }
    const int wpc = tune_int("RGDA_STREAM_WPC", 1);
    if (tune_int("RGDA_STREAM", 1) && kh == 1 && kw == 1 && stride == 1 && pad == 0 && Ho == H && Wo == W &&
        (Cin == 64 || Cin == 128) && !(Cout & 127) && M >= 4 * 128 && !(M & 127) &&
        (long long)M * d.ldx * 2 < (1ll << 31)) {
        const int bp = 128;
        const int tiles_c = Cout / 128;
        const long long tiles_p = M / bp;
        int chunks = (256 * wpc) / tiles_c;
        while (chunks > 1 && ((tiles_p % chunks) || (a.rows_per_group % (int)(tiles_p / chunks * bp)))) chunks >>= 1;
        const long long T = chunks >= 1 ? tiles_p / chunks : 0;
        if (!(M % bp) && chunks >= 1 && T >= 4 && T <= 4096 && !(tiles_p % chunks) && !(a.rows_per_group % (int)(T * bp))) {
            a.tiles_c = tiles_c; a.tiles_p = (int)tiles_p; a.tpw = (int)T;
            p.route = (Cin == 64 ? R_STREAM1_0 : R_STREAM2_0) + conv_epi_kind(a);
            p.grid = tiles_c * chunks;
            return RGDA_OK;
        }
    }
    ConvTile t;
    if (pick_tile(M, Cout, (long long)kh * kw * Cin, (a.stats && stat_groups > 1) ? a.rows_per_group : 0, t))
        return RGDA_ERR_UNSUPPORTED;
    if (const char* e = TUNE_ENV("RGDA_TILE")) {
        t.wp = 2;
        sscanf(e, "%d,%d,%d,%d", &t.bc, &t.bp, &t.stages, &t.wp);
        t.pipe = !TUNE_ENV("RGDA_NO_PIPE");
        if (igemm_route(t) < 0) t.pipe = false;
    }
    a.tiles_c = cdiv(Cout, t.bc);
    a.tiles_p = cdiv(M, t.bp);
    p.route = igemm_route(t);
    p.grid = a.tiles_c * a.tiles_p;
    return p.route < 0 ? RGDA_ERR_UNSUPPORTED : RGDA_OK;
}

static int conv_run(const rgda_conv2d_desc& d, const ConvFuse& f, rgda_stream_t stream) {
    ConvPlan p;
    if (const int rc = conv_select(d, f, p)) return rc;
    return conv_launch(p.route, p.a, p.grid, to_stream(stream));
}

extern "C" const char* rgda_conv2d_kernel(int variant, int N, int H, int W, int Cin, int Ho, int Wo, int Cout, int kh, int kw,
                                          int stride, int pad, int dil, int mode, int has_stats, int stat_groups) {
    static rgda_stat_t dummy_stats;
    static const float dummy_f = 0.f;
    void* const ptr = (void*)&dummy_stats;
    rgda_stat_t* st = (has_stats || variant >= 2) ? &dummy_stats : nullptr;
    BnEvalFuse e = {&dummy_f, &dummy_f, &dummy_f, &dummy_f, 1e-5f, 1};
    BnBwdFuse b = {nullptr, 0, (const unsigned char*)ptr, ptr, (Cout + 7) & ~7, &dummy_f, nullptr, 0, 1, nullptr, nullptr};
    rgda_bn_operand o = {&dummy_stats, &dummy_f, &dummy_f, nullptr, nullptr, nullptr, nullptr, 1e-5f, 0.1f, stat_groups < 1 ? 1 : stat_groups, 1};
    const rgda_conv2d_desc d = {ptr, ptr, ptr, nullptr, nullptr, variant == 1 ? nullptr : st, (Cin + 7) & ~7, (Cout + 7) & ~7, 0,
                                stat_groups, N, H, W, Cin, Ho, Wo, Cout, kh, kw, stride, pad, dil, variant == 3 ? 0 : mode};
    ConvPlan p;
    return conv_select(d, {variant == 2 ? &b : nullptr, variant == 1 ? &e : nullptr, variant == 3 ? &o : nullptr}, p) == RGDA_OK ? CONV_ROUTE_NAMES[p.route] : nullptr;
}

static int conv_select_list(const rgda_conv2d_desc* descs, int n, std::vector<ConvPlan>& plans) {
    if (!descs || n < 0) return RGDA_ERR_ARG;
    plans.resize(n);
    for (int i = 0; i < n; ++i)
        if (const int rc = conv_select(descs[i], ConvFuse{}, plans[i])) return rc;
    return RGDA_OK;
}
static thread_local std::vector<ConvPlan> conv_plans;

extern "C" int rgda_conv2d_grouped(const rgda_conv2d_desc* descs, int n, rgda_stream_t stream) {
    if (const int rc = conv_select_list(descs, n, conv_plans)) return rc;
    hipStream_t st = to_stream(stream);
    ConvGroup g;
    g.n = 0; g.start[0] = 0;
    auto flush = [&]() -> int {
        int rc = RGDA_OK;
        if (g.n == 1) {
            rc = conv_launch(R_GROUPED, g.a[0], g.start[1], st);
        } else if (g.n > 1) {
            for (int i = g.n + 1; i <= CONV_GROUP_MAX; ++i) g.start[i] = g.start[g.n];
            conv_igemm_grouped_kernel<128, 64, 3, 2, 2, true><<<g.start[g.n], 256, 0, st>>>(g);
            RGDA_CHECK_LAUNCH();
        }
        g.n = 0;
        return rc;
    };
    for (int i = 0; i < n; ++i) {
        const ConvPlan& p = conv_plans[i];
        if (p.route == R_GROUPED) {
            g.a[g.n] = p.a;
            g.start[g.n + 1] = g.start[g.n] + p.grid;
            if (++g.n == CONV_GROUP_MAX) { if (int rc = flush()) return rc; }
        } else {
            if (const int rc = conv_launch(p.route, p.a, p.grid, st)) return rc;
        }
    }
    return flush();
}

extern "C" int rgda_conv2d_grouped_launches(const rgda_conv2d_desc* descs, int n) {
    if (const int rc = conv_select_list(descs, n, conv_plans)) return rc;
    int grouped = 0;
    for (const ConvPlan& p : conv_plans) grouped += p.route == R_GROUPED;
    return n - grouped + (grouped + CONV_GROUP_MAX - 1) / CONV_GROUP_MAX;
}

extern "C" int rgda_conv2d(const void* x, int ldx, const void* wgt, void* y, int ldy, const void* res, int ldres,
                           const uint8_t* res_relu_mask, rgda_stat_t* stats, int stat_groups, int N, int H, int W, int Cin,
                           int Ho, int Wo, int Cout, int kh, int kw, int stride, int pad, int dil, int mode,
                           rgda_stream_t stream) {
    return conv_run({x, wgt, y, res, res_relu_mask, stats, ldx, ldy, ldres, stat_groups, N, H, W, Cin, Ho, Wo, Cout, kh, kw,
                     stride, pad, dil, mode}, ConvFuse{}, stream);
}

extern "C" int rgda_conv2d_bneval(const void* x, int ldx, const void* wgt, void* y, int ldy, const void* res, int ldres,
                                  const float* running_mean, const float* running_var, const float* gamma,
                                  const float* beta, float eps, int relu, int N, int H, int W, int Cin, int Ho, int Wo,
                                  int Cout, int kh, int kw, int stride, int pad, int dil, rgda_stream_t stream) {
    const BnEvalFuse e = {running_mean, running_var, gamma, beta, eps, relu};
    return conv_run({x, wgt, y, res, nullptr, nullptr, ldx, ldy, ldres, 1, N, H, W, Cin, Ho, Wo, Cout, kh, kw, stride, pad, dil, 0},
                    ConvFuse{nullptr, &e, nullptr}, stream);
}

extern "C" int rgda_conv2d_bnin(const rgda_bn_operand* bn_in, const void* x, int ldx, const void* wgt, void* y, int ldy,
                                const void* res, int ldres, rgda_stat_t* stats, int stat_groups, int N, int H, int W, int Cin,
                                int Ho, int Wo, int Cout, int kh, int kw, int stride, int pad, int dil, rgda_stream_t stream) {
    if (!bn_in) return RGDA_ERR_ARG;
    return conv_run({x, wgt, y, res, nullptr, stats, ldx, ldy, ldres, stat_groups, N, H, W, Cin, Ho, Wo, Cout, kh, kw, stride, pad,
                     dil, 0}, ConvFuse{nullptr, nullptr, bn_in}, stream);
}

extern "C" int rgda_conv2d_bnbwd(const void* x, int ldx, const void* wgt, void* y, int ldy, const void* res, int ldres,
                                 const uint8_t* res_relu_mask, rgda_stat_t* sums, int groups, const void* bn_y, int bn_ldy, const uint8_t* bn_relu_mask,
                                 const void* bn_x, int bn_ldx,
                                 const float* bn_mi, const float* bn_nscale, int rows_per_image, int relu,
                                 const float* bn_gamma, const float* bn_beta, int N,
                                 int H, int W, int Cin, int Ho, int Wo, int Cout, int kh, int kw, int stride, int pad,
                                 int dil, int mode, rgda_stream_t stream) {
    const BnBwdFuse b = {bn_y, bn_ldy, bn_relu_mask, bn_x, bn_ldx, bn_mi, bn_nscale, rows_per_image, relu, bn_gamma, bn_beta};
    return conv_run({x, wgt, y, res, res_relu_mask, sums, ldx, ldy, ldres, groups, N, H, W, Cin, Ho, Wo, Cout, kh, kw, stride, pad,
                     dil, mode}, ConvFuse{&b, nullptr, nullptr}, stream);
}

template <int KIND>
__global__ void __launch_bounds__(256) __attribute__((amdgpu_waves_per_eu(3, 4))) stem_conv_kernel(ConvArgs a, const float* __restrict__ img, int rpw) {
#if defined(__HIP_DEVICE_COMPILE__)
    constexpr int BC = 64, BP = 64, WC = 2, WP = 2, NW = 4;
    constexpr int SWP = 136;
    constexpr int SROW = SWP * 8;
    constexpr int CSTR = BC * 2 + 16;
    constexpr int EPI = BP * CSTR + NW * BC * 2 * 4;
    __shared__ __attribute__((aligned(256))) unsigned char smem[EPI + 7 * SROW];
    unsigned char* se = smem;
    unsigned char* srow = smem + EPI;

    const int t = threadIdx.x, lane = t & 63;
    const int wave = __builtin_amdgcn_readfirstlane(t >> 6);
    const int wc = wave % WC, wp = wave / WC;
    const int lrow = lane & 31, lk = lane >> 5;
    const int H = a.H, W = a.W, Ho = a.Ho, Wo = a.Wo;
    const int wtiles = Wo / BP, rblocks = Ho / rpw;
    const int wo0 = (blockIdx.x % wtiles) * BP;
    const int ho0 = ((blockIdx.x / wtiles) % rblocks) * rpw, n = blockIdx.x / (wtiles * rblocks);
    const int hbase = ho0 * 2 - 3;

    bf16x8 fa[7][2];
    {
        const bf16_t* wrow = a.w + (size_t)(wc * 32 + lrow) * 192;
#pragma unroll
        for (int kh = 0; kh < 7; ++kh)
#pragma unroll
            for (int kk = 0; kk < 2; ++kk) {
                u16x8 v;
#pragma unroll
                for (int e = 0; e < 8; ++e) {
                    const int kw = kk * 4 + lk * 2 + (e >> 2), c = e & 3;
                    v[e] = (kw < 7 && c < 3) ? wrow[(kh * 7 + kw) * 3 + c] : (bf16_t)0;
                }
                fa[kh][kk] = __builtin_bit_cast(bf16x8, v);
            }
    }
    const size_t plane = (size_t)H * W;
    const float* const img_n = img + (size_t)n * 3 * plane;
    auto load_px = [&](int j, int x, float (&v)[3]) {
        const int hi = hbase + j, wi = wo0 * 2 - 3 + x;
        const bool ok = (unsigned)hi < (unsigned)H && (unsigned)wi < (unsigned)W && x < 134;
        const size_t o = (size_t)(ok ? hi : 0) * W + (ok ? wi : 0);
#pragma unroll
        for (int c = 0; c < 3; ++c) v[c] = ok ? img_n[c * plane + o] : 0.f;
    };
    auto store_px = [&](int j, int x, const float (&v)[3]) {
        uint2 p;
        p.x = pack2bf(v[0], v[1]);
        p.y = pack2bf(v[2], 0.f);
        *(uint2*)(srow + (j % 7) * SROW + x * 8) = p;
    };
#pragma unroll
    for (int i = 0; i < 4; ++i) {
        const int idx = t + 256 * i;
        if (idx < 7 * SWP) {
            float v[3];
            load_px(idx / SWP, idx % SWP, v);
            store_px(idx / SWP, idx % SWP, v);
        }
    }
    const int nj0 = t / SWP, nx0 = t % SWP;
    const int nj1 = (t + 256) / SWP, nx1 = (t + 256) % SWP;
    const bool second = t + 256 < 2 * SWP;
    float na0[3] = {0.f, 0.f, 0.f}, na1[3] = {0.f, 0.f, 0.f}, nb0[3] = {0.f, 0.f, 0.f}, nb1[3] = {0.f, 0.f, 0.f};
    if (1 < rpw) {
        load_px(7 + nj0, nx0, na0);
        if (second) load_px(7 + nj1, nx1, na1);
    }
    float s[8], q[8];
#pragma unroll
    for (int e = 0; e < 8; ++e) { s[e] = 0.f; q[e] = 0.f; }
    EpiParams P;
    epilogue_params<KIND>(a, ((n * Ho + ho0) * Wo + wo0), (t % (BC / 8)) * 8, true, P);
    for (int r = 0; r < rpw; ++r) {
        const int ho = ho0 + r;
        asm volatile("s_waitcnt lgkmcnt(0)" ::: "memory");
        __builtin_amdgcn_s_barrier();
        if (r + 2 < rpw) {
            load_px(2 * r + 9 + nj0, nx0, nb0);
            if (second) load_px(2 * r + 9 + nj1, nx1, nb1);
        }
        f32x16 acc[1][1], acc1;
#pragma unroll
        for (int e = 0; e < 16; ++e) { acc[0][0][e] = 0.f; acc1[e] = 0.f; }
        const int px = wp * 32 + lrow;
        const unsigned char* fbase = srow + px * 16 + lk * 16;
        const int s0 = (2 * r) % 7;
#pragma unroll
        for (int kh = 0; kh < 7; ++kh) {
            const int slot = (s0 + kh >= 7) ? s0 + kh - 7 : s0 + kh;
            const bf16x8 fb0 = *(const bf16x8*)(fbase + slot * SROW);
            const bf16x8 fb1 = *(const bf16x8*)(fbase + slot * SROW + 32);
            acc[0][0] = __builtin_amdgcn_mfma_f32_32x32x16_bf16(fa[kh][0], fb0, acc[0][0], 0, 0, 0);
            acc1 = __builtin_amdgcn_mfma_f32_32x32x16_bf16(fa[kh][1], fb1, acc1, 0, 0, 0);
        }
#pragma unroll
        for (int e = 0; e < 16; ++e) acc[0][0][e] += acc1[e];
        const int m0 = (n * Ho + ho) * Wo + wo0;
        conv_epilogue<BC, BP, WC, WP, true, KIND>(a, acc, se, m0, 0, s, q, r + 1 == rpw, blockIdx.x & (NREP - 1), &P);
        if (r + 1 < rpw) {
            store_px(2 * r + 7 + nj0, nx0, na0);
            if (second) store_px(2 * r + 7 + nj1, nx1, na1);
        }
#pragma unroll
        for (int c = 0; c < 3; ++c) { na0[c] = nb0[c]; na1[c] = nb1[c]; }
    }
#endif
}

static int stem_conv_launch(const float* img, const void* wgt, void* y, int ldy, rgda_stat_t* stats, int stat_groups,
                            const BnEvalFuse* bne, int N, int H, int W, int Ho, int Wo, rgda_stream_t stream) {
    if (!img || !wgt || !y || N <= 0 || H <= 0 || W <= 0 || (ldy & 7) || ldy < 64) return RGDA_ERR_ARG;
    if (Ho != (H + 6 - 7) / 2 + 1 || Wo != (W + 6 - 7) / 2 + 1) return RGDA_ERR_ARG;
    if (Wo % 64) return RGDA_ERR_UNSUPPORTED;
    if ((long long)3 * H * W >= (1ll << 28)) return RGDA_ERR_UNSUPPORTED;
    if (stat_groups < 1) stat_groups = 1;
    if ((N % stat_groups) || (bne && stats)) return RGDA_ERR_ARG;
    const long long M = (long long)N * Ho * Wo;
    if (M > 0x7fffffffLL) return RGDA_ERR_ARG;
    ConvArgs a;
    a.x = nullptr; a.w = (const bf16_t*)wgt; a.y = (bf16_t*)y; a.res = nullptr; a.stats = stats; a.res_mask = nullptr;
    a.ldx = 0; a.ldy = ldy; a.ldres = 0;
    a.N = N; a.H = H; a.W = W; a.Cin = 3; a.Ho = Ho; a.Wo = Wo; a.Cout = 64; a.KH = 7; a.KW = 7;
    a.stride = 2; a.pad = 3; a.dil = 1; a.mode = 0;
    a.M = (int)M; a.tiles_c = 1; a.tiles_p = 0;
    a.rows_per_group = (int)(M / stat_groups);
    a.howo_shift = a.wo_shift = -1; a.dbg = nullptr; a.tpw = 0; a.skip = 0;
    a.bn_y = a.bn_x = nullptr; a.bn_mask = nullptr; a.bn_mi = a.bn_nscale = nullptr; a.bn_ldy = a.bn_ldx = a.bn_rpi = a.bn_relu = 0;
    a.bn_gamma = a.bn_beta = nullptr; a.xf.stats = nullptr;
    a.ev_rm = a.ev_rv = a.ev_gamma = a.ev_beta = nullptr; a.ev_eps = 0.f; a.ev_relu = 0;
    if (bne) {
        if (!bne->rm || !bne->rv || !bne->gamma || !bne->beta) return RGDA_ERR_ARG;
        a.ev_rm = bne->rm; a.ev_rv = bne->rv; a.ev_gamma = bne->gamma; a.ev_beta = bne->beta; a.ev_eps = bne->eps; a.ev_relu = bne->relu;
    }
    int rpw = 8;
    if (const char* e = TUNE_ENV("RGDA_STEM_RPW")) rpw = atoi(e);
    else while (rpw < 64 && (long long)N * (Ho / (2 * rpw)) * (Wo / 64) >= 512 && !(Ho % (2 * rpw))) rpw *= 2;
// ... 918 lines not shown
```

### regda_amd/csrc/norm_kernels.hip

```cpp
#include <stdlib.h>
#include "common.h"

struct RowLayout {
    int vpr;
    int vpb;
    int rpb;
};
static RowLayout row_layout(int C) {
    RowLayout L;
    L.vpr = C / 8;
    int v = 1;
    while (v < L.vpr && v < 256) v <<= 1;
    L.vpb = v;
    L.rpb = 256 / v;
    return L;
}

static int reduce_rows_per_block(long long M, const RowLayout& L) {
    int ny = cdiv(L.vpr, L.vpb);
    long long want = 512 / ny;
    if (const char* e = TUNE_ENV("RGDA_RED_WANT")) want = atoi(e) / ny;
    if (want < 1) want = 1;
    long long rows = (M + want - 1) / want;
    long long minrows = (long long)L.rpb * 4;
    if (rows < minrows) rows = minrows;
    rows = (rows + L.rpb - 1) / L.rpb * L.rpb;
    return (int)rows;
}

static __device__ __forceinline__ void load8(const bf16_t* p, float (&f)[8]) {
    u16x8 v = *(const u16x8*)p;
#pragma unroll
    for (int e = 0; e < 8; ++e) f[e] = bf2f(v[e]);
}
static __device__ __forceinline__ void cvt8(const u16x8& v, float (&f)[8]) {
#pragma unroll
    for (int e = 0; e < 8; ++e) f[e] = bf2f(v[e]);
}
#ifndef ROW_BATCH
#define ROW_BATCH 4
#endif
#ifndef RB_BWD
#define RB_BWD 2
#endif
#ifndef RB_APPLY
#define RB_APPLY ROW_BATCH
#endif
#ifndef RB_REDUCE
#define RB_REDUCE ROW_BATCH
#endif
#ifndef RB_BWD
#define RB_BWD ROW_BATCH
#endif
#ifndef RB_INORM
#define RB_INORM ROW_BATCH
#endif
#ifndef RB_MIX
#define RB_MIX ROW_BATCH
#endif
#ifndef RB_CLS
#define RB_CLS ROW_BATCH
#endif
static __device__ __forceinline__ unsigned char relu_bits(const uint4& v) {
    auto pos = [](unsigned h) { return (unsigned)((h & 0x7fffu) != 0 && (h & 0x8000u) == 0); };
    return (unsigned char)(pos(v.x & 0xffffu) | pos(v.x >> 16) << 1 | pos(v.y & 0xffffu) << 2 | pos(v.y >> 16) << 3 |
                           pos(v.z & 0xffffu) << 4 | pos(v.z >> 16) << 5 | pos(v.w & 0xffffu) << 6 | pos(v.w >> 16) << 7);
}
static __device__ __forceinline__ void store8(bf16_t* p, const float (&f)[8]) {
    uint4 v;
    v.x = pack2bf(f[0], f[1]); v.y = pack2bf(f[2], f[3]); v.z = pack2bf(f[4], f[5]); v.w = pack2bf(f[6], f[7]);
    *(uint4*)p = v;
}

static __device__ __forceinline__ void block_reduce_atomic(float (&s)[8], float (&q)[8], int cvl, int rl, int vpb,
                                                           int rpb, int cglobal, bool cok, rgda_stat_t* out0,
                                                           rgda_stat_t* out1, float* lds, int frac) {
    __syncthreads();
#pragma unroll
    for (int e = 0; e < 8; ++e) {
        lds[((rl * vpb + cvl) * 8 + e) * 2 + 0] = s[e];
        lds[((rl * vpb + cvl) * 8 + e) * 2 + 1] = q[e];
    }
    __syncthreads();
    if (rl == 0 && cok) {
#pragma unroll
        for (int e = 0; e < 8; ++e) {
            float a = 0.f, b = 0.f;
            for (int r = 0; r < rpb; ++r) {
                a += lds[((r * vpb + cvl) * 8 + e) * 2 + 0];
                b += lds[((r * vpb + cvl) * 8 + e) * 2 + 1];
            }
            stat_add(out0 + cglobal + e, a, frac);
            stat_add(out1 + cglobal + e, b, frac);
        }
    }
}

__global__ void __launch_bounds__(256) bn_stats_kernel(const bf16_t* __restrict__ x, int ldx, rgda_stat_t* stats,
                                                       long long M, int C, int vpb, int rpb, int rows_per_block) {
    __shared__ float lds[256 * 16];
    const int cvl = threadIdx.x % vpb, rl = threadIdx.x / vpb;
    const int cg = (blockIdx.y * vpb + cvl) * 8;
    const bool cok = cg < C;
    float s[8] = {0}, q[8] = {0};
    long long r0 = (long long)blockIdx.x * rows_per_block, r1 = min(M, r0 + rows_per_block);
    if (cok)
        for (long long r = r0 + rl; r < r1; r += rpb) {
            float f[8];
            load8(x + r * ldx + cg, f);
#pragma unroll
            for (int e = 0; e < 8; ++e) { s[e] += f[e]; q[e] += f[e] * f[e]; }
        }
    rgda_stat_t* rep = stats + (size_t)((blockIdx.x + blockIdx.y * gridDim.x) & (NREP - 1)) * 2 * C;
    block_reduce_atomic(s, q, cvl, rl, vpb, rpb, cg, cok, rep, rep + C, lds, RGDA_STAT_FRAC_FWD);
}

extern "C" int rgda_bn_stats(const void* x, int ldx, rgda_stat_t* stats, int64_t M, int C, rgda_stream_t stream) {
    if (!x || !stats || M <= 0 || C <= 0 || (C & 7) || (ldx & 7)) return RGDA_ERR_ARG;
    RowLayout L = row_layout(C);
    if (L.vpb > 16) { L.vpb = 16; L.rpb = 16; }
    int rows_per_block = reduce_rows_per_block(M, L);
    dim3 grid(cdiv(M, rows_per_block), cdiv(L.vpr, L.vpb));
    bn_stats_kernel<<<grid, 256, 0, to_stream(stream)>>>((const bf16_t*)x, ldx, stats, M, C, L.vpb, L.rpb, rows_per_block);
    RGDA_CHECK_LAUNCH();
    return RGDA_OK;
}

__global__ void __launch_bounds__(256) bn_finalize_kernel(const rgda_stat_t* stats, float* mi, float* rm, float* rv,
                                                          long long* nbt, double M, int C, int groups, float eps,
                                                          float mom) {
    int c = blockIdx.x * 256 + threadIdx.x;
    if (c >= C) return;
    for (int g = 0; g < groups; ++g) {
        const rgda_stat_t* st = stats ? stats + (size_t)g * NREP * 2 * C : nullptr;
        float* m = mi + (size_t)g * 2 * C;
        if (st) {
            float mean, var, istd;
            stat_moments(st, C, c, 1.0 / M, eps, mean, var, istd);
            m[c] = mean;
            m[C + c] = istd;
            if (rm) {
                const float unb = (M > 1) ? (float)M / (float)(M - 1.0) : 1.f;
                rm[c] = (1.f - mom) * rm[c] + mom * mean;
                rv[c] = (1.f - mom) * rv[c] + mom * var * unb;
            }
            if (c == 0 && nbt) *nbt += 1;
        } else {
            m[c] = rm[c];
            m[C + c] = 1.f / sqrtf(rv[c] + eps);
        }
    }
}

extern "C" int rgda_bn_finalize(const rgda_stat_t* stats, float* mi, float* running_mean, float* running_var,
                                int64_t* num_batches_tracked, int64_t M, int C, int groups, float eps,
                                float momentum, rgda_stream_t stream) {
    if (!mi || C <= 0 || groups < 1 || (M % groups) || (!stats && (!running_mean || !running_var))) return RGDA_ERR_ARG;
    if (stats && M / groups < 2) return RGDA_ERR_ARG;
    bn_finalize_kernel<<<cdiv(C, 256), 256, 0, to_stream(stream)>>>(stats, mi, running_mean, running_var,
                                                                      (long long*)num_batches_tracked,
                                                                      (double)(M / groups), C, groups, eps, momentum);
    RGDA_CHECK_LAUNCH();
    return RGDA_OK;
}

static __device__ __forceinline__ void group_stats(const rgda_stat_t* __restrict__ stats, int grp, int C, int cg, float invM,
                                                   float eps, float (&mean)[8], float (&istd)[8], float (&var)[8]) {
    const rgda_stat_t* st = stats + (size_t)grp * NREP * 2 * C;
#pragma unroll
    for (int e = 0; e < 8; ++e) stat_moments(st, C, cg + e, (double)invM, eps, mean[e], var[e], istd[e]);
}

__global__ void __launch_bounds__(256) bn_apply_kernel(const bf16_t* __restrict__ x, int ldx,
                                                       const float* __restrict__ mi, const float* __restrict__ gamma,
                                                       const float* __restrict__ beta, const bf16_t* __restrict__ res,
                                                       int ldres, const float* __restrict__ nscale, int rpi,
                                                       bf16_t* __restrict__ y, int ldy, long long M, int C, int relu,
                                                       int vpb, int rpb, int rows_per_block, int bpg,
                                                       const rgda_stat_t* __restrict__ stats, float* mi_out, float* rm,
                                                       float* rv, long long* nbt, int groups, float eps, float mom,
                                                       uint8_t* __restrict__ mask_out) {
    const int cvl = threadIdx.x % vpb, rl = threadIdx.x / vpb;
    const int cg = (blockIdx.y * vpb + cvl) * 8;
    const int grp = blockIdx.x / bpg, chunk = blockIdx.x % bpg;
    __shared__ float smean[128], sistd[128];
    if (stats) {
        const double invM = 1.0 / (double)M;
        const rgda_stat_t* st = stats + (size_t)grp * NREP * 2 * C;
        for (int c = threadIdx.x; c < vpb * 8; c += 256) {
            int cc = blockIdx.y * vpb * 8 + c;
            if (cc < C) {
                float m, v0, is;
                stat_moments(st, C, cc, invM, eps, m, v0, is);
                smean[c] = m;
                sistd[c] = is;
                if (chunk == 0) {
                    mi_out[(size_t)grp * 2 * C + cc] = m;
                    mi_out[(size_t)grp * 2 * C + C + cc] = is;
                    if (grp == 0 && rm) {
                        const float unb = (M > 1) ? (float)M / (float)(M - 1) : 1.f;
                        float gm[8], gv[8];
#pragma unroll
                        for (int g = 0; g < 8; ++g) {
                            if (g < groups) {
                                float gis;
                                stat_moments(stats + (size_t)g * NREP * 2 * C, C, cc, invM, eps, gm[g], gv[g], gis);
                            }
                        }
                        float a = rm[cc], b = rv[cc];
#pragma unroll
                        for (int g = 0; g < 8; ++g) {
                            if (g < groups) {
                                a = (1.f - mom) * a + mom * gm[g];
                                b = (1.f - mom) * b + mom * gv[g] * unb;
                            }
                        }
                        rm[cc] = a;
                        rv[cc] = b;
                        if (cc == 0 && nbt) *nbt += groups;
                    }
                }
            }
        }
        __syncthreads();
    }
    if (cg >= C) return;
    float mean[8], sc[8], sh[8];
    if (stats) {
#pragma unroll
        for (int e = 0; e < 8; ++e) {
            mean[e] = smean[cvl * 8 + e];
            sc[e] = sistd[cvl * 8 + e] * gamma[cg + e];
            sh[e] = beta[cg + e];
        }
    } else {
        mi += (size_t)grp * 2 * C;
#pragma unroll
        for (int e = 0; e < 8; ++e) {
            mean[e] = mi[cg + e];
            sc[e] = mi[C + cg + e] * gamma[cg + e];
            sh[e] = beta[cg + e];
        }
    }
    long long r0 = (long long)grp * M + (long long)chunk * rows_per_block;
    long long r1 = min((long long)(grp + 1) * M, r0 + rows_per_block);
    for (long long rb = r0 + rl; rb < r1; rb += (long long)rpb * RB_APPLY) {
        u16x8 xv[RB_APPLY], rv[RB_APPLY];
#pragma unroll
        for (int u = 0; u < RB_APPLY; ++u) {
            const long long r = rb + (long long)u * rpb;
            if (r < r1) {
                xv[u] = *(const u16x8*)(x + r * ldx + cg);
                if (res) rv[u] = *(const u16x8*)(res + r * ldres + cg);
            }
        }
#pragma unroll
        for (int u = 0; u < RB_APPLY; ++u) {
            const long long r = rb + (long long)u * rpb;
            if (r >= r1) break;
            float f[8];
            cvt8(xv[u], f);
#pragma unroll
            for (int e = 0; e < 8; ++e) f[e] = (f[e] - mean[e]) * sc[e] + sh[e];
            if (res) {
                float g[8];
                cvt8(rv[u], g);
#pragma unroll
                for (int e = 0; e < 8; ++e) f[e] += g[e];
            }
            if (relu) {
#pragma unroll
                for (int e = 0; e < 8; ++e) f[e] = fmaxf(f[e], 0.f);
            }
            if (nscale) {
                const float* ns = nscale + (r / rpi) * C + cg;
#pragma unroll
                for (int e = 0; e < 8; ++e) f[e] *= ns[e];
            }
            uint4 pk;
            pk.x = pack2bf(f[0], f[1]); pk.y = pack2bf(f[2], f[3]); pk.z = pack2bf(f[4], f[5]); pk.w = pack2bf(f[6], f[7]);
            *(uint4*)(y + r * ldy + cg) = pk;
            if (mask_out) mask_out[r * (C >> 3) + (cg >> 3)] = relu_bits(pk);
        }
    }
}

static void elementwise_grid(long long M, int C, int groups, RowLayout& L, int& rows_per_block, int& bpg, dim3& grid,
                             int rows_mult = 8) {
    L = row_layout(C);
    if (L.vpb > 16) { L.vpb = 16; L.rpb = 16; }
    if (const char* e = TUNE_ENV("RGDA_BN_VPB")) {
        int v = atoi(e);
        RowLayout full = row_layout(C);
        if (v <= full.vpb) { L.vpb = v; L.rpb = 256 / v; }
    }
    if (const char* e = TUNE_ENV("RGDA_BN_ROWS")) rows_mult = atoi(e);
    rows_per_block = L.rpb * rows_mult;
    while ((long long)cdiv(M, rows_per_block) * groups * cdiv(L.vpr, L.vpb) > 8192) rows_per_block *= 2;
    bpg = cdiv(M, rows_per_block);
    grid = dim3(bpg * groups, cdiv(L.vpr, L.vpb));
}

extern "C" int rgda_bn_apply(const void* x, int ldx, const float* mi, const float* gamma, const float* beta,
                             const void* res, int ldres, const float* nscale, int rows_per_image, void* y, int ldy,
                             int64_t M, int C, int relu, int groups, rgda_stream_t stream) {
    if (!x || !mi || !gamma || !beta || !y || M <= 0 || C <= 0 || (C & 7) || (ldx & 7) || (ldy & 7)) return RGDA_ERR_ARG;
    if (res && (ldres & 7)) return RGDA_ERR_ARG;
    if (nscale && rows_per_image <= 0) return RGDA_ERR_ARG;
    if (groups < 1 || (M % groups)) return RGDA_ERR_ARG;
    RowLayout L; int rpbk, bpg; dim3 grid;
    elementwise_grid(M / groups, C, groups, L, rpbk, bpg, grid);
    bn_apply_kernel<<<grid, 256, 0, to_stream(stream)>>>((const bf16_t*)x, ldx, mi, gamma, beta, (const bf16_t*)res,
                                                          ldres, nscale, rows_per_image, (bf16_t*)y, ldy, M / groups, C,
                                                          relu, L.vpb, L.rpb, rpbk, bpg, nullptr, nullptr, nullptr,
                                                          nullptr, nullptr, groups, 0.f, 0.f, nullptr);
    RGDA_CHECK_LAUNCH();
    return RGDA_OK;
}

extern "C" int rgda_bn_train_apply(const void* x, int ldx, const rgda_stat_t* stats, float* mi, float* running_mean,
                                   float* running_var, int64_t* num_batches_tracked, const float* gamma,
                                   const float* beta, const void* res, int ldres, const float* nscale,
                                   int rows_per_image, void* y, int ldy, uint8_t* relu_mask, int64_t M, int C,
                                   int relu, int groups, float eps, float momentum, rgda_stream_t stream) {
    if (!x || !stats || !mi || !gamma || !beta || !y || M <= 0 || C <= 0 || (C & 7) || (ldx & 7) || (ldy & 7)) return RGDA_ERR_ARG;
    if (relu_mask && !relu) return RGDA_ERR_ARG;
    if (res && (ldres & 7)) return RGDA_ERR_ARG;
    if (nscale && rows_per_image <= 0) return RGDA_ERR_ARG;
    if (groups < 1 || groups > 8 || (M % groups) || M / groups < 2) return RGDA_ERR_ARG;
    if ((running_mean == nullptr) != (running_var == nullptr)) return RGDA_ERR_ARG;
    RowLayout L; int rpbk, bpg; dim3 grid;
    elementwise_grid(M / groups, C, groups, L, rpbk, bpg, grid);
    bn_apply_kernel<<<grid, 256, 0, to_stream(stream)>>>((const bf16_t*)x, ldx, nullptr, gamma, beta, (const bf16_t*)res,
                                                          ldres, nscale, rows_per_image, (bf16_t*)y, ldy, M / groups, C,
                                                          relu, L.vpb, L.rpb, rpbk, bpg, stats, mi, running_mean,
                                                          running_var, (long long*)num_batches_tracked, groups, eps,
                                                          momentum, relu_mask);
    RGDA_CHECK_LAUNCH();
    return RGDA_OK;
}

template <bool FROM_X>
__global__ void __launch_bounds__(256) bn_bwd_reduce_kernel(const bf16_t* __restrict__ g, int ldg,
                                                            const bf16_t* __restrict__ y, int ldy,
                                                            const uint8_t* __restrict__ rmask,
                                                            const bf16_t* __restrict__ x, int ldx,
                                                            const float* __restrict__ mi, const float* __restrict__ nscale,
                                                            int rpi, rgda_stat_t* sums, long long M, int C, int relu, int vpb,
                                                            int rpb, int rows_per_block, int bpg,
                                                            const float* __restrict__ gamma, const float* __restrict__ beta) {
    __shared__ float lds[256 * 16];
    const int cvl = threadIdx.x % vpb, rl = threadIdx.x / vpb;
    const int cg = (blockIdx.y * vpb + cvl) * 8;
    const bool cok = cg < C;
    const int grp = blockIdx.x / bpg, chunk = blockIdx.x % bpg;
    mi += (size_t)grp * 2 * C;
    sums += (size_t)grp * NREP * 2 * C;
    float s[8] = {0}, q[8] = {0};
    if (cok) {
        float mean[8], istd[8], fsc[8], fsh[8];
#pragma unroll
        for (int e = 0; e < 8; ++e) {
            mean[e] = mi[cg + e]; istd[e] = mi[C + cg + e];
            fsc[e] = 0.f; fsh[e] = 0.f;
            if constexpr (FROM_X) bn_scale_shift(mean[e], istd[e], gamma[cg + e], beta[cg + e], fsc[e], fsh[e]);
        }
        long long r0 = (long long)grp * M + (long long)chunk * rows_per_block;
        long long r1 = min((long long)(grp + 1) * M, r0 + rows_per_block);
        for (long long rb = r0 + rl; rb < r1; rb += (long long)rpb * RB_REDUCE) {
            u16x8 gv[RB_REDUCE], xv[RB_REDUCE], yv[RB_REDUCE];
            unsigned mb[RB_REDUCE];
#pragma unroll
            for (int u = 0; u < RB_REDUCE; ++u) {
                const long long r = rb + (long long)u * rpb;
// ... 1316 lines not shown
```

### regda_amd/models/Encoder.py

```python
import collections
import contextlib
import math
from typing import NamedTuple

import torch
import torch.nn as nn

from .. import ops
from .. import plan

BF = torch.bfloat16
LAYERS = {'resnet101': (3, 4, 23, 3), 'resnet50': (3, 4, 6, 3)}
POOL_SCALES = (1, 2, 3, 6)
NREP = 8
LAYOUT_TILE = 64


def _layout_blocks(co, ci, taps):
    return -(-ci // LAYOUT_TILE) * -(-co // LAYOUT_TILE) * taps

ASPP_DILATIONS = (6, 12, 18, 24)
STEM_KP = 192


# ... 193 lines not shown

class _WgradQueue:

    def __init__(self):
        self.items, self.flop, self._apart = [], 0.0, None

    def take(self):
        items, self.items, self.flop = self.items, [], 0.0
        return items

    def add(self, item, flop):
        if self._apart is not None:
            self._apart.append((item, flop))
        else:
            self.items.append(item)
            self.flop += flop

    def due(self, gflop):
        return self._apart is None and self.flop >= gflop * 1e9

    @contextlib.contextmanager
    def apart(self, side):
        self._apart = side
        try:
            yield
        finally:
            self._apart = None

    def join(self, side):
        for item, flop in side:
            self.add(item, flop)


def _attach(root, dotted, kind, tensor):
    parts = dotted.split('.')
    m = root
    for p in parts[:-1]:
        if p not in m._modules:
            m.add_module(p, _Container())
        m = m._modules[p]
    if kind == 'param':
        m.register_parameter(parts[-1], tensor)
    else:
        m.register_buffer(parts[-1], tensor)


def _pad64(n):
    return (n + 63) // 64 * 64


def _nchw(t, N, h, w):
    return t.float().reshape(N, h, w, -1).permute(0, 3, 1, 2)


def _param_entries(resnet_type, head_kind, num_classes):
    entries = []

    def conv(name, co, ci, k, bias=False):
        entries.append((name + '.weight', 'convw', (co, ci, k, k)))
        if bias:
            entries.append((name + '.bias', 'vec', (co,)))

    def bn(name, c):
        entries.append((name + '.weight', 'vec', (c,)))
        entries.append((name + '.bias', 'vec', (c,)))
        entries.append((name + '.running_mean', 'buf', (c,)))
        entries.append((name + '.running_var', 'buf', (c,)))
        entries.append((name + '.num_batches_tracked', 'nbt', ()))

    conv('encoder.resnet.conv1', 64, 3, 7); bn('encoder.resnet.bn1', 64)
    blocks = _block_specs(resnet_type)
    for p, inpl, planes, stride, dil, ds in blocks:
        conv(p + '.conv1', planes, inpl, 1); bn(p + '.bn1', planes)
        conv(p + '.conv2', planes, planes, 3); bn(p + '.bn2', planes)
        conv(p + '.conv3', planes * 4, planes, 1); bn(p + '.bn3', planes * 4)
        if ds:
            conv(p + '.downsample.0', planes * 4, inpl, 1); bn(p + '.downsample.1', planes * 4)
    for head in ('layer5', 'layer6'):
        if head_kind == 'aspp':
            for i in range(len(ASPP_DILATIONS)):
                conv(f'{head}.conv2d_list.{i}', num_classes, 2048, 3, bias=True)
            continue
        for i in range(4):
            conv(f'{head}.ppm.{i}.1', 512, 2048, 1); bn(f'{head}.ppm.{i}.2', 512)
        conv(f'{head}.conv_last.0', 512, 2048 + 4 * 512, 3); bn(f'{head}.conv_last.1', 512)
        conv(f'{head}.conv_last.4', num_classes, 512, 1, bias=True)
    head_first = 'ppm.0.1' if head_kind == 'ppm' else 'conv2d_list.0'

    return entries, blocks, head_first


def flat_layout(resnet_type='resnet101', head_kind='ppm', num_classes=6):
    entries, _, _ = _param_entries(resnet_type, head_kind, num_classes)
    out, op = {}, 0
    for name, kind, shape in entries:
        if kind in ('convw', 'vec'):
            n = math.prod(shape)
            out[name] = (op, n)
            op += _pad64(n)
    out['__total__'] = (op, 0)
    return out


def backward_progress_offsets(resnet_type='resnet101', head_kind='ppm', num_classes=6):
    lay = flat_layout(resnet_type, head_kind, num_classes)
    _, blocks, head_first = _param_entries(resnet_type, head_kind, num_classes)
    offs = [lay[f'layer5.{head_first}.weight'][0]]
    offs += [lay[p + '.conv1.weight'][0] for p, *_ in reversed(blocks)]
    return offs


def bucket_boundaries(resnet_type='resnet101', head_kind='ppm', num_classes=6):
    lay = flat_layout(resnet_type, head_kind, num_classes)
    _, blocks, head_first = _param_entries(resnet_type, head_kind, num_classes)
    return sorted([lay[p + '.conv1.weight'][0] for p, *_ in blocks] +
                  [lay[f'{h}.{head_first}.weight'][0] for h in ('layer5', 'layer6')])


class Deeplabv2(nn.Module):
    def __init__(self, config):
        super().__init__()
        cfg = dict(backbone=dict(resnet_type='resnet50', output_stride=16, pretrained=True), multi_layer=False,
                   cascade=False, use_ppm=False, ppm=dict(num_classes=7, use_aux=False), inchannels=2048,
                   num_classes=7, is_ins_norm=False)
        for k, v in dict(config).items():
            if isinstance(v, dict) and isinstance(cfg.get(k), dict):
                cfg[k] = dict(cfg[k], **v)
            else:
                cfg[k] = v
        self.config = cfg
        rt = cfg['backbone']['resnet_type']
        if not (cfg['multi_layer'] and not cfg['cascade'] and cfg['is_ins_norm']):
            raise NotImplementedError('regda_amd builds the st.regda.* model: multi_layer=True, cascade=False, '
                                      'is_ins_norm=True, with the PPM heads (use_ppm=True) or the ASPP heads '
                                      '(use_ppm=False); the cascade / single-head variants are not built')
        self.head_kind = 'ppm' if cfg['use_ppm'] else 'aspp'
        if rt not in LAYERS or cfg['backbone'].get('output_stride', 16) != 16:
            raise NotImplementedError('resnet50/resnet101 at output_stride 16 only')
        if not torch.cuda.is_available():
            raise RuntimeError('regda_amd.Deeplabv2 needs an MI355X: there is no CPU fallback')
        self.resnet_type = rt
        self.num_classes = int(cfg['num_classes'])
        self.device = torch.device('cuda', torch.cuda.current_device())
        self._build_params()
        self._init_weights()
        self._anchor = torch.zeros(1, device=self.device, requires_grad=True)
        self._drop_override = None
        self.wgrad_group_gflop = 500.0
        self.relu_sign_mask = 1
        self.factored_ppm = True
        self.group_small_convs = True
        self.small_bn = True
        self.bn_on_operand = True
        self.bn_operand_units = {'stem', 'bn1', 'bn2'}
        self.bn_operand_level = 2
        self._head_stream = None
        self._mat_cache = {}
        self._synced_version = -1
        self.sync_weights()

    def _build_params(self):
        dev = self.device
        entries, self.blocks, self._head_first = _param_entries(self.resnet_type, self.head_kind, self.num_classes)

        n_param = sum(_pad64(math.prod(s)) for _, k, s in entries if k in ('convw', 'vec'))
        n_buf = sum(_pad64(math.prod(s)) for _, k, s in entries if k == 'buf')
        n_nbt = sum(1 for _, k, _s in entries if k == 'nbt')
        self.flat_p = torch.zeros(n_param, device=dev)
        self.flat_g = torch.zeros(n_param, device=dev)
        self.flat_pb = torch.zeros(n_param, dtype=BF, device=dev)
        self.flat_buf = torch.zeros(n_buf, device=dev)
        self.flat_nbt = torch.zeros((n_nbt + 1) // 2 * 2, dtype=torch.int64, device=dev)
        self.n_param_elems = sum(math.prod(s) for _, k, s in entries if k in ('convw', 'vec'))
        self._views, self._gviews = {}, {}
        self.convs, self.bns = {}, {}
        op = ob = on = 0
        wt_total = 0
        for name, kind, shape in entries:
            n = math.prod(shape)
            if kind == 'convw':
                co, ci, k, _ = shape
                phys = self.flat_p[op:op + n].view(co, k, k, ci)
                gphys = self.flat_g[op:op + n].view(co, k, k, ci)
                par = nn.Parameter(phys.permute(0, 3, 1, 2))
                _attach(self, name, 'param', par)
                self._views[name], self._gviews[name] = par, gphys.permute(0, 3, 1, 2)
                c = _Conv()
                c.name, c.co, c.ci, c.k = name[:-7], co, ci, k
                c.stride, c.pad, c.dil = 1, 0, 1
                c.w, c.g = self.flat_p[op:op + n].view(co, k * k, ci), self.flat_g[op:op + n].view(co, k * k, ci)
                c.wb = self.flat_pb[op:op + n].view(co, k * k, ci)
                c.wtb, c.bias, c.gbias = None, None, None
                self.convs[c.name] = c
                wt_total += _pad64(n)
                op += _pad64(n)
            elif kind == 'vec':
                par = nn.Parameter(self.flat_p[op:op + n].view(shape))
                _attach(self, name, 'param', par)
                self._views[name], self._gviews[name] = par, self.flat_g[op:op + n].view(shape)
                base = name.rsplit('.', 1)[0]
                if base in self.convs:
                    self.convs[base].bias, self.convs[base].gbias = self.flat_p[op:op + n], self.flat_g[op:op + n]
                else:
                    b = self.bns.setdefault(base, _BN())
                    b.name, b.c = base, n
                    if name.endswith('.weight'):
                        b.gamma, b.dgamma = self.flat_p[op:op + n], self.flat_g[op:op + n]
                    else:
                        b.beta, b.dbeta = self.flat_p[op:op + n], self.flat_g[op:op + n]
                op += _pad64(n)
            elif kind == 'buf':
                t = self.flat_buf[ob:ob + n]
                _attach(self, name, 'buf', t)
                b = self.bns[name.rsplit('.', 1)[0]]
                if name.endswith('running_mean'):
                    b.rm = t
                else:
                    b.rv = t
                ob += _pad64(n)
            else:
                t = self.flat_nbt[on:on + 1].view(())
                _attach(self, name, 'buf', t)
                self.bns[name.rsplit('.', 1)[0]].nbt = t
                on += 1
        for p, inpl, planes, stride, dil, ds in self.blocks:
            c2 = self.convs[p + '.conv2']
            c2.stride, c2.pad, c2.dil = stride, dil, dil
            if ds:
                self.convs[p + '.downsample.0'].stride = stride
        for head in ('layer5', 'layer6'):
            if self.head_kind == 'aspp':
                for i, d in enumerate(ASPP_DILATIONS):
                    self.convs[f'{head}.conv2d_list.{i}'].pad = self.convs[f'{head}.conv2d_list.{i}'].dil = d
            else:
                self.convs[f'{head}.conv_last.0'].pad = 1
        self.flat_wt = torch.zeros(wt_total, dtype=BF, device=dev)
        o = 0
        for c in self.convs.values():
            if c.name == 'encoder.resnet.conv1' or c.bias is not None:
                continue
            n = c.co * c.k * c.k * c.ci
            c.wtb = self.flat_wt[o:o + n].view(c.ci, c.k * c.k, c.co)
            o += _pad64(n)
        rows, blk = [], 0
        for c in self.convs.values():
            if c.wtb is not None:
                T = c.k * c.k
                rows.append([self._mirror_ptr(c.w.data_ptr()), c.wtb.data_ptr(), c.co, T, c.ci, blk, c.ci, 0 | 16])
                blk += _layout_blocks(c.co, c.ci, T)
        self._wt_table = torch.tensor(rows, dtype=torch.int64, device=dev)
        self._wt_blocks = blk
        self.stem_wb = torch.zeros(64, 1, STEM_KP, dtype=BF, device=dev)
        self.grad_arena = torch.zeros(64 * STEM_KP, device=dev)
        self.stem_gtmp = self.grad_arena.view(64, 1, STEM_KP)
        self.head_w = {}
        self._hw_ready = None
        if self.head_kind == 'aspp':
            self._build_aspp_weights()
            return
        for head in ('layer5', 'layer6'):
            self.head_w[head] = {
                'wfeat': torch.zeros(512, 9, 2048, dtype=BF, device=dev),
                'wz': [torch.zeros(9 * 512, 1, 512, dtype=BF, device=dev) for _ in POOL_SCALES],
                'wzt': [torch.zeros(512, 1, 9 * 512, dtype=BF, device=dev) for _ in POOL_SCALES],
            }

        def table(kinds):
            rows, blk = [], 0
            for head, hw in self.head_w.items():
                wsrc = self._mirror_ptr(self.convs[f'{head}.conv_last.0'].w.data_ptr())
                if 'fwd' in kinds:
                    rows.append([wsrc, hw['wfeat'].data_ptr(), 512, 9, 2048, blk, 4096, 2 | 16])
                    blk += _layout_blocks(512, 2048, 9)
                for i in range(len(POOL_SCALES)):
                    src = wsrc + 2 * (2048 + 512 * i)
                    if 'fwd' in kinds:
                        rows.append([src, hw['wz'][i].data_ptr(), 512, 9, 512, blk, 4096, 1 | 16])
                        blk += _layout_blocks(512, 512, 9)
                    if 'bwd' in kinds:
                        rows.append([src, hw['wzt'][i].data_ptr(), 512, 9, 512, blk, 4096, 0 | 16])
                        blk += _layout_blocks(512, 512, 9)
            return torch.tensor(rows, dtype=torch.int64, device=dev), blk
        self._hw_fwd_table, self._hw_fwd_blocks = table(('fwd',))
        self._hw_bwd_table, self._hw_bwd_blocks = table(('bwd',))

    def _build_aspp_weights(self):
        dev, C = self.device, self.num_classes
        self.aspp_rows = 2 * len(ASPP_DILATIONS) * C * 9
        self.aspp_zc = (self.aspp_rows + 63) // 64 * 64
        self.aspp_wz = torch.zeros(self.aspp_zc, 1, 2048, dtype=BF, device=dev)
        self.aspp_wzt = torch.zeros(2048, 1, self.aspp_zc, dtype=BF, device=dev)
        self.aspp_gz = torch.zeros(self.aspp_zc, 1, 2048, device=dev)
        self.aspp_convs = [self.convs[f'{head}.conv2d_list.{i}'] for head in ('layer5', 'layer6')
                           for i in range(len(ASPP_DILATIONS))]
        rows, blk = [], 0
        for j, c in enumerate(self.aspp_convs):
            rows.append([self._mirror_ptr(c.w.data_ptr()), self.aspp_wz.data_ptr() + 2 * j * C * 9 * 2048, C, 9, 2048, blk, 2048, 2 | 16])
            blk += _layout_blocks(C, 2048, 9)
        self._hw_fwd_table, self._hw_fwd_blocks = torch.tensor(rows, dtype=torch.int64, device=dev), blk

    def _init_weights(self):
        with torch.no_grad():
            for name, par in self._views.items():
                if par.dim() == 4:
                    co, ci, k, _ = par.shape
                    if name.startswith('encoder.'):
                        par.copy_(torch.randn(co, ci, k, k, device=self.device) * math.sqrt(2.0 / (co * k * k)))
# ... 84 lines not shown
        if not mirror_is_fresh:
            ops.cast_bf16(self.flat_p, self.flat_pb)
        s = self.convs['encoder.resnet.conv1']
        ops.pad_cast_bf16(s.w, self.stem_wb, 64, 147, STEM_KP)
        self._sync_head_weights(False)
        self._synced_version = self.flat_p._version

    def set_drop_masks(self, m5, m6):
        self._drop_override = None if m5 is None else (m5, m6)

    def _side_stream(self):
        if self._head_stream is None:
            self._head_stream = torch.cuda.Stream(device=self.device)
        return self._head_stream

    def _relu_mask(self, relu, rows, ch):
        if relu and self.relu_sign_mask and ch >= self.relu_sign_mask:
            return torch.empty(rows, ch // 8, dtype=torch.uint8, device=self.device)
        return None

    def _mats(self, h, w):
        key = (h, w)
        if key not in self._mat_cache:
            d = {}
            for s in POOL_SCALES:
                P = pool_matrix(h, w, s)
                U = upsample_matrix(s, s, h, w)
                V = ppm_tap_matrix(h, w, s)
                d[s] = tuple(t.to(self.device).contiguous() for t in (P, P.t(), U, U.t(), V, V.t()))
            self._mat_cache[key] = d
        return self._mat_cache[key]

    def _ppm_maps(self, h, w):
        key = ('ppm', h, w)
        if key not in self._mat_cache:
            dev = self.device
            Wx, Ay = ppm_factored_maps(h, w)
            self._mat_cache[key] = {
                'R': Wx.shape[0], 'Wx': Wx.to(dev).contiguous(), 'Wxt': Wx.t().contiguous().to(dev),
                'fwd': tuple(t.to(dev) for t in _csr(Ay)),
                'bwd': tuple(t.to(dev) for t in _csr([torch.cat([A.t() for A in Ay], 0).contiguous()])),
            }
        return self._mat_cache[key]

    def _pool_maps(self, h, w):
        key = ('pool', h, w)
        if key not in self._mat_cache:
            dev = self.device
            Px, Qy = pool_factored_maps(h, w)
            self._mat_cache[key] = {
                'R': Px.shape[0], 'Px': Px.to(dev).contiguous(), 'Pxt': Px.t().contiguous().to(dev),
                'fwd': tuple(t.to(dev) for t in _csr([torch.cat(Qy, 0).contiguous()])),
                'bwd': tuple(t.to(dev) for t in _csr([Q.t().contiguous() for Q in Qy])),
            }
        return self._mat_cache[key]

    def build_maps(self, H, W):
        if self.head_kind != 'ppm':
            return
        h, w = H, W
        for _ in range(4):
            h, w = (h - 1) // 2 + 1, (w - 1) // 2 + 1
        if self.factored_ppm:
            self._pool_maps(h, w)
            self._ppm_maps(h, w)
        else:
            self._mats(h, w)

    def _conv_stats(self, x, w, c, stats, G, N, H, W, Ho, Wo, k, stride, pad, dil, res=None, queue=None):
        if G == 1 or stats is None:
            if queue is not None:
                queue.append((x, w, c, N, H, W, Ho, Wo, k, k, stride, pad, dil, 0, res, stats, 1))
            else:
                ops.conv2d(x, w, c, N, H, W, Ho, Wo, k, k, stride, pad, dil, 0, res, stats, 1)
            return
        whole = (x, w, c, N, H, W, Ho, Wo, k, k, stride, pad, dil, 0, res, stats, G)
        try:
            if queue is not None:
                ops.conv2d_grouped_launches([whole])
                queue.append(whole)
            else:
                ops.conv2d(*whole)
        except ValueError:
            Ng = N // G
            st = stats.view(G, -1)
            for g in range(G):
                ro = slice(g * Ng * Ho * Wo, (g + 1) * Ng * Ho * Wo)
                part = (x[g * Ng * H * W:(g + 1) * Ng * H * W], w, c[ro], Ng, H, W, Ho, Wo, k, k, stride, pad, dil, 0,
                        None if res is None else res[ro], st[g], 1)
                if queue is not None:
                    queue.append(part)
                else:
                    ops.conv2d(*part)

    def _materialise(self, T, lz):
        mi = torch.empty(lz.G, 2, lz.bn.c, device=self.device)
        y = torch.empty(lz.M, lz.bn.c, dtype=BF, device=self.device)
        rmask = self._relu_mask(lz.relu, lz.M, lz.bn.c)
        e = T[lz.key]
        _, _, _, Ho, Wo = e.dims
        ops.bn_train_apply(lz.c, lz.stats, mi, lz.bn.rm, lz.bn.rv, lz.bn.nbt, lz.bn.gamma, lz.bn.beta, y, lz.M, lz.bn.c,
                           lz.relu, None, None, Ho * Wo, groups=lz.G, relu_mask=rmask)
        T[lz.key] = _Unit(e.x, e.c, y, mi, e.dims, e.nscale, rmask)
        return y

    def _bn_operand(self, T, lz):
        mi = torch.empty(lz.G, 2, lz.bn.c, device=self.device)
        e = T[lz.key]
        T[lz.key] = _Unit(e.x, e.c, None, mi, e.dims, e.nscale, FROM_X)
        bnop = ops.bn_operand(lz.stats, lz.bn.gamma, lz.bn.beta, mi, lz.bn.rm, lz.bn.rv, lz.bn.nbt, lz.G, lz.relu)
        T['keep'].append(bnop)
        return bnop

    def _cbr_fwd(self, T, key, conv, bn, x, N, H, W, relu, res=None, nscale=None, wb=None, geom=None, defer=False,
                 preconv=None):
        Ho, Wo = conv.out_hw(H, W) if geom is None else geom
        M = N * Ho * Wo
        train = T is not None
        G = T['groups'] if train else 1
        if not train:
            y = torch.empty(M, conv.co, dtype=BF, device=self.device)
            if geom is None:
                ops.conv2d_bneval(x, conv.wb if wb is None else wb, y, N, H, W, Ho, Wo, conv.k, conv.k, conv.stride,
                                  conv.pad, conv.dil, bn.rm, bn.rv, bn.gamma, bn.beta, relu, res)
            else:
                ops.conv2d_bneval(x, wb, y, N, Ho, Wo, Ho, Wo, 1, 1, 1, 0, 1, bn.rm, bn.rv, bn.gamma, bn.beta, relu, res)
            return y, Ho, Wo
        if M // G < 2:
            raise ValueError('Expected more than 1 value per channel when training')
        if preconv is not None:
            c, stats = preconv
        else:
            c = torch.empty(M, conv.co, dtype=BF, device=self.device)
            stats = T['stats_pool'].take(G * NREP * 2 * conv.co) if train else None
        if isinstance(x, _Lazy):
            if geom is None and ops.conv2d_bnin_supported(M, conv.co, conv.ci, conv.k, conv.k, conv.stride, conv.pad,
                                                          conv.dil, H, W, Ho, Wo, G) >= self.bn_operand_level:
                ops.conv2d_bnin(self._bn_operand(T, x), x.c, conv.wb if wb is None else wb, c, N, H, W, Ho, Wo, conv.k,
                                conv.k, conv.stride, conv.pad, conv.dil, None, stats, G)
            else:
                x = self._materialise(T, x)
        if not isinstance(x, _Lazy) and preconv is None:
            if geom is None:
                self._conv_stats(x, conv.wb if wb is None else wb, c, stats, G, N, H, W, Ho, Wo, conv.k, conv.stride,
                                 conv.pad, conv.dil)
            else:
                self._conv_stats(x, wb, c, stats, G, N, Ho, Wo, Ho, Wo, 1, 1, 0, 1)
        if defer and self.bn_on_operand and res is None and nscale is None:
            T[key] = _Unit(x, c, None, None, (N, H, W, Ho, Wo), None, None)
            return _Lazy(key, c, stats, bn, G, relu, M), Ho, Wo
        mi = torch.empty(G, 2, conv.co, device=self.device)
        y = torch.empty(M, conv.co, dtype=BF, device=self.device)
        rmask = self._relu_mask(relu, M, conv.co)
        ops.bn_train_apply(c, stats, mi, bn.rm, bn.rv, bn.nbt, bn.gamma, bn.beta, y, M, conv.co, relu, res, nscale,
                           Ho * Wo, groups=G, relu_mask=rmask)
        T[key] = _Unit(x, c, y, mi, (N, H, W, Ho, Wo), nscale, rmask)
        return y, Ho, Wo

    def _head_last_fwd(self, T, head, xn, qs, N, h, w, nscale):
        bn = self.bns[f'{head}.conv_last.1']
        hw = self.head_w[head]
        dev = self.device
        HW, M = h * w, N * h * w
        zs, queue = [], []
        for i, s in enumerate(POOL_SCALES):
            z = torch.empty(N * s * s, 9 * 512, dtype=BF, device=dev)
            queue.append((qs[i], hw['wz'][i], z, N, s, s, s, s, 1, 1, 1, 0, 1))
            zs.append(z.view(N * s * s * 9, 512))
        if self.group_small_convs:
            ops.conv2d_grouped(queue)
        else:
            for it in queue:
                ops.conv2d(*it)
        ppm = torch.empty(M, 512, dtype=BF, device=dev)
        if self.factored_ppm:
            fm = self._ppm_maps(h, w)
            rows = torch.empty(N * h * fm['R'], 512, device=dev)
            ops.sparse_mix(zs, fm['fwd'], rows, N, 512)
            ops.group_mix(rows, fm['Wxt'], ppm, N * h, w, fm['R'], 512)
        else:
            mats = self._mats(h, w)
            ops.spatial_mix_multi(zs, [mats[s][4] for s in POOL_SCALES], ppm, N, HW, 512)
        train = T is not None
        G = T['groups'] if train else 1
        c = torch.empty(M, 512, dtype=BF, device=dev)
        stats = T['stats_pool'].take(G * NREP * 2 * 512) if train else None
        self._conv_stats(xn, hw['wfeat'], c, stats, G, N, h, w, h, w, 3, 1, 1, 1, res=ppm)
        mi = torch.empty(G, 2, 512, device=dev)
        y = torch.empty(M, 512, dtype=BF, device=dev)
        if train:
            ops.bn_train_apply(c, stats, mi, bn.rm, bn.rv, bn.nbt, bn.gamma, bn.beta, y, M, 512, True, None, nscale,
                               HW, groups=G)
            T[f'{head}.last'] = _Unit(xn, c, y, mi, (N, h, w, h, w), nscale, None)
            T[f'{head}.last.q'] = qs
        else:
            ops.bn_finalize(None, mi, bn.rm, bn.rv, None, M, 512)
            ops.bn_apply(c, mi, bn.gamma, bn.beta, y, M, 512, True, None, nscale, HW, groups=G)
        return y

    def _head_last_bwd(self, T, head, g, dfeat_prev):
        conv, bn = self.convs[f'{head}.conv_last.0'], self.bns[f'{head}.conv_last.1']
        dev = self.device
        e = T[f'{head}.last']
        N, h, w, _, _ = e.dims
        HW, M, G = h * w, N * h * w, T['groups']
        sums = T['sums_pool'].take(G * NREP * 2 * 512)
        ops.bn_bwd_reduce(g, e.y, e.c, e.mi, sums, M, 512, True, e.nscale, HW, groups=G)
        dc = torch.empty(M, 512, dtype=BF, device=dev)
        ops.bn_bwd_apply(g, e.y, e.c, e.mi, bn.gamma, sums, dc, M, 512, True, None, bn.dgamma, bn.dbeta, e.nscale, HW,
                         groups=G)
        gview = conv.g.view(512, 9, 4096)
        T['wgrads'].add((e.x, dc, gview[:, :, :2048], N, h, w, h, w, 3, 3, 1, 1, 1), 2.0 * M * 512 * 2048 * 9)
        dfeat = torch.empty(M, 2048, dtype=BF, device=dev)
        ops.conv2d(dc, conv.wtb[:2048], dfeat, N, h, w, h, w, 3, 3, 1, 1, 1, 1, dfeat_prev, None)
        T['keep'].append((dc, dfeat))
        return dfeat, dc

    def _head_last_bwd_tail(self, T, head, dc):
        conv = self.convs[f'{head}.conv_last.0']
        hw = self.head_w[head]
        dev = self.device
        N, h, w, _, _ = T[f'{head}.last'].dims
        qs = T[f'{head}.last.q']
        HW = h * w
        gview = conv.g.view(512, 9, 4096)
        dqs = []
        if self.factored_ppm:
            fm = self._ppm_maps(h, w)
            rows = torch.empty(N * h * fm['R'], 512, device=dev)
            ops.group_mix(dc, fm['Wx'], rows, N * h, fm['R'], w, 512)
            dzs = [torch.empty(N * s * s * 9, 512, dtype=BF, device=dev) for s in POOL_SCALES]
            ops.sparse_mix([rows], fm['bwd'], dzs, N, 512)
        queue = []
        for i, s in enumerate(POOL_SCALES):
            if self.factored_ppm:
                dz = dzs[i]
            else:
                dz = torch.empty(N * s * s * 9, 512, dtype=BF, device=dev)
                ops.spatial_mix(dc, self._mats(h, w)[s][5], dz, N, 9 * s * s, HW, 512)
            dzr = dz.view(N * s * s, 9 * 512)
            dq = torch.empty(N * s * s, 512, dtype=BF, device=dev)
            if self.group_small_convs:
                queue.append((dzr, hw['wzt'][i], dq, N, s, s, s, s, 1, 1, 1, 0, 1))
            else:
                ops.conv2d(dzr, hw['wzt'][i], dq, N, s, s, s, s, 1, 1, 1, 0, 1)
            T['wgrads'].add((qs[i], dzr, gview[:, :, 2048 + 512 * i: 2048 + 512 * (i + 1)], N, s, s, s, s, 1, 1, 1, 0, 1),
                            2.0 * N * s * s * 9 * 512 * 512)
            T['keep'].append((dz, dq))
            dqs.append(dq)
        if queue:
            ops.conv2d_grouped(queue)
        return dqs

    def _aspp_fwd(self, T, xn, N, h, w):
        dev, C = self.device, self.num_classes
        z = torch.empty(N * h * w, self.aspp_zc, dtype=BF, device=dev)
        ops.conv2d(xn, self.aspp_wz, z, N, h, w, h, w, 1, 1, 1, 0, 1, 0)
        x1 = torch.empty(N, C, h, w, device=dev)
        x2 = torch.empty(N, C, h, w, device=dev)
        ops.aspp_gather(z, [c.bias for c in self.aspp_convs], x1, x2, N, h, w, C, ASPP_DILATIONS)
        if T is not None:
            T['aspp'] = (xn, (N, h, w))
        return x1, x2

    def _aspp_bwd(self, T, g1, g2):
        dev, C = self.device, self.num_classes
        xn, (N, h, w) = T['aspp']
        dz = torch.empty(N * h * w, self.aspp_zc, dtype=BF, device=dev)
        ops.aspp_scatter(g1, g2, dz, [c.gbias for c in self.aspp_convs],
                         N, h, w, C, ASPP_DILATIONS)
        dxn = torch.empty(N * h * w, 2048, dtype=BF, device=dev)
        ops.conv2d(dz, self.aspp_wzt, dxn, N, h, w, h, w, 1, 1, 1, 0, 1, 0)
        plan.host(self.aspp_gz.zero_)
        ops.conv2d_wgrad(xn, dz, self.aspp_gz, N, h, w, h, w, 1, 1, 1, 0, 1)
        n = C * 9 * 2048
        for j, c in enumerate(self.aspp_convs):
            plan.host(lambda j=j, c=c: c.g.view(-1).add_(self.aspp_gz.view(-1)[j * n:(j + 1) * n]))
        return dxn

    def _flush_wgrads(self, T):
        pend = T['wgrads'].take()
        if pend:
            side = T.get('wgrad_stream')
            if side is None:
                ops.conv2d_wgrad_grouped(pend)
            else:
                plan.wait_event(side, plan.record_event(T['main_stream']))
                with ops.use_stream(side):
                    ops.conv2d_wgrad_grouped(pend)
                T['keep'].extend((it[0], it[1]) for it in pend)
        off = T.pop('progress_deferred', None)
        if off is not None:
            T['on_progress'](off)

    def _flush_wgrads_if_due(self, T):
        if T['wgrads'].due(self.wgrad_group_gflop):
            self._flush_wgrads(T)

    def _progress(self, T, offset):
        if T.get('on_progress') is None:
            return
        if T['wgrads'].items:
            T['progress_deferred'] = offset
        else:
            T['on_progress'](offset)

    def _cbr_bwd(self, T, key, conv, bn, g, relu, need_dx=True, want_gmask=False, dx_res=None, stem=False,
                 consumer=None, dx_res_mask=None, conv_queue=None, bn_queue=None):
# ... 464 lines not shown
```

### regda_amd/ops.py

```python
import ctypes

import torch

from ._lib import lib


MIN_CLASSES, MAX_CLASSES = 6, 16


def check_class_count(c, who='class_num'):
    if not MIN_CLASSES <= int(c) <= MAX_CLASSES:
        raise ValueError(f'{who}: {c} classes; the kernels serve {MIN_CLASSES} <= class_num <= {MAX_CLASSES}')


_LDS_LOSS_ROW, _LDS_PCL, _LDS_REFINE = 0, 1, 2


def check_step_shape(c, k, H, W, who='step'):
    check_class_count(c, who)
    L = lib()
    w = (int(W) + 15) // 16
    row, lim = L.size('rgda_class_lds', _LDS_LOSS_ROW, c, w, W), L.size('rgda_class_lds_limit', _LDS_LOSS_ROW)
    if row > lim:
        raise ValueError(f'{who}: {c} classes at {W}-pixel rows need {row} B of LDS in the fused upsample + loss row pass, '
# ... 521 lines not shown
               _stream())
    return state


def pseudo_analysis_state_views(state, c, R):
    rows = R + 1
    T = rows * (2 * c + 2)
    o = T * 8
    tot = state[:o].view(torch.int64)
    f = state[o:o + 16 * R].view(torch.float64)
    i = state[o + 16 * R + 8:o + 16 * R + 8 + 8 * R + 4].view(torch.int32)
    return dict(total_used=tot[:rows * c].view(rows, c), total_hit=tot[rows * c:2 * rows * c].view(rows, c),
                total_inbin=tot[2 * rows * c:2 * rows * c + rows], total_diff24=tot[2 * rows * c + rows:],
                acc_sum=f[:R], diffi_sum=f[R:], images=state[o + 16 * R:o + 16 * R + 8].view(torch.int64),
                acc_cnt=i[:R], diffi_cnt=i[R:2 * R], flag=i[2 * R:])


def proto_pixel_weight(feat, protos, label, sim=None, ignore_label=-1, out=None):
    _need_cuda(feat, protos, label, sim)
    label = label.contiguous()
    assert label.dtype == torch.int64 and label.dim() == 3
    b, H, W = label.shape
    L = lib()
    if sim is not None:
        assert sim.dtype == torch.float32 and sim.is_contiguous() and sim.dim() == 4 and sim.shape[0] == b
        c, (h, w), k = sim.shape[1], sim.shape[-2:], 0
        ws = None
    else:
        feat, protos = feat.contiguous().float(), protos.contiguous().float()
        k, (h, w), c = feat.shape[1], feat.shape[-2:], protos.shape[0]
        assert feat.shape[0] == b and protos.shape == (c, k)
        ws = _ws(L.size('rgda_proto_pixel_weight_workspace', b, c, k, h, w), label.device)
    if out is None:
        out = torch.empty(b * H * W, dtype=torch.float32, device=label.device)
    assert out.dtype == torch.float32 and out.is_contiguous() and out.numel() == b * H * W
    L.call('rgda_proto_pixel_weight', _p(feat if sim is None else None), _p(protos if sim is None else None), _p(sim),
           label.data_ptr(), out.data_ptr(), b, k, c, h, w, H, W, ignore_label, _p(ws), 0 if ws is None else ws.numel(),
           _stream())
    return out


def teacher_probs(p1, p2, size):
    _need_cuda(p1, p2)
    p1, p2 = p1.contiguous().float(), p2.contiguous().float()
    b, c, h, w = p1.shape
    H, W = size
    out = torch.empty((b, c, H, W), dtype=torch.float32, device=p1.device)
    lib().call('rgda_teacher_probs', p1.data_ptr(), p2.data_ptr(), out.data_ptr(), b, c, h, w, H, W, _stream())
    return out


def class_count(label, class_num):
    _need_cuda(label)
    label = label.contiguous()
    cnt = torch.zeros(class_num, dtype=torch.int32, device=label.device)
    lib().call('rgda_class_count', label.data_ptr(), cnt.data_ptr(), label.numel(), class_num, _stream())
    return cnt



def _ld(t):
    assert t.dim() == 2 and t.stride(1) == 1
    return t.stride(0)


def conv2d(x, w, y, N, H, W, Ho, Wo, kh, kw, stride, pad, dil, mode=0, res=None, stats=None, stat_groups=1,
           res_mask=None):
    Cout, taps, Cin = w.shape
    assert taps == kh * kw and x.shape[1] == Cin and y.shape[1] == Cout
    lib().call('rgda_conv2d', x.data_ptr(), _ld(x), w.data_ptr(), y.data_ptr(), _ld(y), _p(res),
               _ld(res) if res is not None else 0, _p(res_mask), _stat(stats), stat_groups, N, H, W, Cin, Ho, Wo, Cout, kh, kw, stride,
               pad, dil, mode, _stream())


class _ConvDesc(ctypes.Structure):
    _fields_ = [(k, ctypes.c_void_p) for k in ('x', 'wgt', 'y', 'res', 'res_relu_mask', 'stats')] + \
               [(k, ctypes.c_int) for k in ('ldx', 'ldy', 'ldres', 'stat_groups', 'N', 'H', 'W', 'Cin', 'Ho', 'Wo', 'Cout', 'kh',
                                            'kw', 'stride', 'pad', 'dil', 'mode')]


def _conv_descs(items):
    arr = (_ConvDesc * len(items))()
    for d, it in zip(arr, items):
        x, w, y, N, H, W, Ho, Wo, kh, kw, stride, pad, dil = it[:13]
        mode = it[13] if len(it) > 13 else 0
        res = it[14] if len(it) > 14 else None
        stats = it[15] if len(it) > 15 else None
        stat_groups = it[16] if len(it) > 16 else 1
        res_mask = it[17] if len(it) > 17 else None
        Cout, taps, Cin = w.shape
        assert taps == kh * kw and x.shape[1] == Cin and y.shape[1] == Cout
        d.x, d.wgt, d.y, d.res, d.res_relu_mask, d.stats = x.data_ptr(), w.data_ptr(), y.data_ptr(), _p(res), _p(res_mask), _stat(stats)
        d.ldx, d.ldy, d.ldres, d.stat_groups = _ld(x), _ld(y), (_ld(res) if res is not None else 0), stat_groups
        d.N, d.H, d.W, d.Cin, d.Ho, d.Wo, d.Cout = N, H, W, Cin, Ho, Wo, Cout
        d.kh, d.kw, d.stride, d.pad, d.dil, d.mode = kh, kw, stride, pad, dil, mode
    return arr


def conv2d_grouped(items):
    if not items:
        return
    arr = _conv_descs(items)
    lib().call('rgda_conv2d_grouped', ctypes.cast(arr, ctypes.c_void_p), len(items), _stream())


def conv2d_grouped_launches(items):
    arr = _conv_descs(items)
    n = lib().size('rgda_conv2d_grouped_launches', ctypes.cast(arr, ctypes.c_void_p), len(items))
    if n < 0:
        raise ValueError('rgda_conv2d_grouped: status %d' % n)
    return n


def conv2d_bneval(x, w, y, N, H, W, Ho, Wo, kh, kw, stride, pad, dil, rm, rv, gamma, beta, relu, res=None, eps=1e-5):
    Cout, taps, Cin = w.shape
    assert taps == kh * kw and x.shape[1] == Cin and y.shape[1] == Cout
    lib().call('rgda_conv2d_bneval', x.data_ptr(), _ld(x), w.data_ptr(), y.data_ptr(), _ld(y), _p(res),
               _ld(res) if res is not None else 0, rm.data_ptr(), rv.data_ptr(), gamma.data_ptr(), beta.data_ptr(), eps,
               int(relu), N, H, W, Cin, Ho, Wo, Cout, kh, kw, stride, pad, dil, _stream())


def conv2d_bnbwd(x, w, y, N, H, W, Ho, Wo, kh, kw, stride, pad, dil, mode, res, sums, groups, bn_y, bn_x, bn_mi, relu,
                 nscale=None, rows_per_image=0, relu_mask=None, res_mask=None, bn_gamma=None, bn_beta=None):
    Cout, taps, Cin = w.shape
    assert taps == kh * kw and x.shape[1] == Cin and y.shape[1] == Cout
    lib().call('rgda_conv2d_bnbwd', x.data_ptr(), _ld(x), w.data_ptr(), y.data_ptr(), _ld(y), _p(res),
               _ld(res) if res is not None else 0, _p(res_mask), _stat(sums), groups, _p(bn_y), _ld(bn_y) if bn_y is not None else 0,
               _p(relu_mask), bn_x.data_ptr(), _ld(bn_x), bn_mi.data_ptr(), _p(nscale), rows_per_image, int(relu),
               _p(bn_gamma), _p(bn_beta), N, H, W, Cin, Ho, Wo, Cout, kh, kw, stride, pad, dil, mode, _stream())


class _BnOperand(ctypes.Structure):
    _fields_ = [('stats', ctypes.c_void_p), ('gamma', ctypes.c_void_p), ('beta', ctypes.c_void_p), ('mi', ctypes.c_void_p),
                ('running_mean', ctypes.c_void_p), ('running_var', ctypes.c_void_p), ('num_batches_tracked', ctypes.c_void_p),
                ('eps', ctypes.c_float), ('momentum', ctypes.c_float), ('groups', ctypes.c_int), ('relu', ctypes.c_int)]


def bn_operand(stats, gamma, beta, mi=None, rm=None, rv=None, nbt=None, groups=1, relu=True, eps=1e-5, momentum=0.1):
    d = _BnOperand(_stat(stats), gamma.data_ptr(), beta.data_ptr(), _p(mi), _p(rm), _p(rv), _p(nbt), eps, momentum,
                   int(groups), int(bool(relu)))
    return ctypes.cast(ctypes.pointer(d), ctypes.c_void_p)


def conv2d_bnin_supported(M, Cout, Cin, kh, kw, stride, pad, dil, H, W, Ho, Wo, groups):
    return lib().size('rgda_conv2d_bnin_supported', M, Cout, Cin, kh, kw, stride, pad, dil, H, W, Ho, Wo, groups)


def conv2d_bnin(bnop, x, w, y, N, H, W, Ho, Wo, kh, kw, stride, pad, dil, res=None, stats=None, stat_groups=1):
    Cout, taps, Cin = w.shape
    assert taps == kh * kw and x.shape[1] == Cin and y.shape[1] == Cout
    lib().call('rgda_conv2d_bnin', bnop, x.data_ptr(), _ld(x), w.data_ptr(), y.data_ptr(), _ld(y), _p(res),
               _ld(res) if res is not None else 0, _stat(stats), stat_groups, N, H, W, Cin, Ho, Wo, Cout, kh, kw, stride, pad,
               dil, _stream())


def conv2d_wgrad(x, dy, dw, N, H, W, Ho, Wo, kh, kw, stride, pad, dil):
    Cout, taps, Cin = dw.shape
    assert dw.is_contiguous() and dw.dtype == torch.float32
    conv2d_wgrad_grouped([(x, dy, dw, N, H, W, Ho, Wo, kh, kw, stride, pad, dil)])


class _WgradDesc(ctypes.Structure):
    _fields_ = [('x', ctypes.c_void_p), ('dy', ctypes.c_void_p), ('dw', ctypes.c_void_p), ('ldx', ctypes.c_int),
                ('lddy', ctypes.c_int)] + [(k, ctypes.c_int) for k in
                                           ('N', 'H', 'W', 'Cin', 'Ho', 'Wo', 'Cout', 'kh', 'kw', 'stride', 'pad', 'dil',
                                            'lddw', 'co_split')]


_WGRAD_WS = {}
_WGRAD_WS_OLD = []


def _wgrad_ws(nbytes, device):
    key = (device.index, _stream())
    ws = _WGRAD_WS.get(key)
    if ws is None or ws.numel() < nbytes:
        if ws is not None:
            _WGRAD_WS_OLD.append(ws)
        ws = torch.empty(max(nbytes, 32 << 20), dtype=torch.uint8, device=device)
        ws[:65536].zero_()
        _WGRAD_WS[key] = ws
    return ws


def conv2d_wgrad_grouped(items):
    if not items:
        return
    arr = (_WgradDesc * len(items))()
    for d, (x, dy, dw, N, H, W, Ho, Wo, kh, kw, stride, pad, dil) in zip(arr, items):
        S, T, Cin = dw.shape
        assert dw.dtype == torch.float32 and dw.stride(2) == 1 and dw.stride(0) == T * dw.stride(1)
        stacked = kh * kw == 1 and T > 1
        assert stacked or T == kh * kw
        Cout = S * T if stacked else S
        d.x, d.dy, d.dw, d.ldx, d.lddy = x.data_ptr(), dy.data_ptr(), dw.data_ptr(), _ld(x), _ld(dy)
        d.N, d.H, d.W, d.Cin, d.Ho, d.Wo, d.Cout = N, H, W, Cin, Ho, Wo, Cout
        d.kh, d.kw, d.stride, d.pad, d.dil = kh, kw, stride, pad, dil
        d.lddw, d.co_split = dw.stride(1), (S if stacked else 0)
    L = lib()
    ap = ctypes.cast(arr, ctypes.c_void_p)
    ws = _wgrad_ws(L.size('rgda_conv2d_wgrad_workspace', ap, len(items)), items[0][0].device)
    L.call('rgda_conv2d_wgrad_grouped', ap, len(items), ws.data_ptr(), ws.numel(), _stream())


def stem_conv(img, wb, y, stats, N, H, W, Ho, Wo, stat_groups=1):
    lib().call('rgda_stem_conv', img.data_ptr(), wb.data_ptr(), y.data_ptr(), _ld(y), _stat(stats), stat_groups, N, H, W, Ho, Wo,
               _stream())


def stem_conv_bneval(img, wb, y, rm, rv, gamma, beta, relu, N, H, W, Ho, Wo, eps=1e-5):
    lib().call('rgda_stem_conv_bneval', img.data_ptr(), wb.data_ptr(), y.data_ptr(), _ld(y), rm.data_ptr(), rv.data_ptr(),
               gamma.data_ptr(), beta.data_ptr(), eps, int(relu), N, H, W, Ho, Wo, _stream())


def stem_im2col(img, col, N, H, W, Ho, Wo):
    lib().call('rgda_stem_im2col', img.data_ptr(), col.data_ptr(), N, H, W, Ho, Wo, col.shape[1], _stream())


_STEM_WS = {}
_STEM_WS_OLD = []


def stem_wgrad(img, dy, dw, N, H, W, Ho, Wo):
    assert dw.is_contiguous() and dw.dtype == torch.float32 and dw.numel() == 64 * 147 and img.is_contiguous()
    L = lib()
    nbytes = L.size('rgda_stem_wgrad_workspace', N, H, W)
    if nbytes == 0:
        raise ValueError('rgda_stem_wgrad: geometry not served (Wo % 64 != 0): use stem_im2col + conv2d_wgrad')
    key = (img.device.index, _stream())
    ws = _STEM_WS.get(key)
    if ws is None or ws.numel() < nbytes:
        if ws is not None:
            _STEM_WS_OLD.append(ws)
        ws = torch.empty(nbytes, dtype=torch.uint8, device=img.device)
        _STEM_WS[key] = ws
    L.call('rgda_stem_wgrad', img.data_ptr(), dy.data_ptr(), _ld(dy), dw.data_ptr(), ws.data_ptr(), ws.numel(), N, H, W, Ho, Wo,
           _stream())


def bn_stats(x, stats, M, C):
    lib().call('rgda_bn_stats', x.data_ptr(), _ld(x), _stat(stats), M, C, _stream())


def bn_finalize(stats, mi, rm, rv, nbt, M, C, eps=1e-5, momentum=0.1, groups=1):
    lib().call('rgda_bn_finalize', _stat(stats), mi.data_ptr(), _p(rm), _p(rv), _p(nbt), M, C, groups, eps, momentum,
               _stream())


def bn_apply(x, mi, gamma, beta, y, M, C, relu, res=None, nscale=None, rows_per_image=0, groups=1):
    lib().call('rgda_bn_apply', x.data_ptr(), _ld(x), mi.data_ptr(), gamma.data_ptr(), beta.data_ptr(), _p(res),
               _ld(res) if res is not None else 0, _p(nscale), rows_per_image, y.data_ptr(), _ld(y), M, C,
               int(relu), groups, _stream())


def bn_train_apply(x, stats, mi, rm, rv, nbt, gamma, beta, y, M, C, relu, res=None, nscale=None, rows_per_image=0,
                   groups=1, eps=1e-5, momentum=0.1, relu_mask=None):
    lib().call('rgda_bn_train_apply', x.data_ptr(), _ld(x), _stat(stats), mi.data_ptr(), _p(rm), _p(rv), _p(nbt),
               gamma.data_ptr(), beta.data_ptr(), _p(res), _ld(res) if res is not None else 0, _p(nscale),
               rows_per_image, y.data_ptr(), _ld(y), _p(relu_mask), M, C, int(relu), groups, eps, momentum, _stream())


def bn_bwd_reduce(g, y, x, mi, sums, M, C, relu, nscale=None, rows_per_image=0, groups=1, relu_mask=None, gamma=None,
                  beta=None):
    lib().call('rgda_bn_bwd_reduce', g.data_ptr(), _ld(g), _p(y), _ld(y) if y is not None else 0, _p(relu_mask),
               x.data_ptr(), _ld(x),
               mi.data_ptr(), _p(nscale), rows_per_image, _stat(sums), M, C, int(relu), _p(gamma), _p(beta), groups, _stream())


def bn_bwd_apply(g, y, x, mi, gamma, sums, dx, M, C, relu, gmask=None, dgamma=None, dbeta=None, nscale=None,
                 rows_per_image=0, groups=1, relu_mask=None, beta=None, act_out=None):
    lib().call('rgda_bn_bwd_apply', g.data_ptr(), _ld(g), _p(y), _ld(y) if y is not None else 0, _p(relu_mask),
               x.data_ptr(), _ld(x),
               mi.data_ptr(), gamma.data_ptr(), _p(nscale), rows_per_image, _stat(sums), dx.data_ptr(), _ld(dx),
               _p(gmask), _ld(gmask) if gmask is not None else 0, _p(dgamma), _p(dbeta), M, C, int(relu), _p(beta),
               _p(act_out), _ld(act_out) if act_out is not None else 0, groups, _stream())


class _BnSmallFwd(ctypes.Structure):
    _fields_ = [(k, ctypes.c_void_p) for k in ('x', 'y', 'relu_mask', 'gamma', 'beta', 'mi', 'running_mean', 'running_var',
                                               'num_batches_tracked')] + [('M', ctypes.c_int64)] + \
               [(k, ctypes.c_int) for k in ('ldx', 'ldy', 'C', 'groups', 'relu')] + [('eps', ctypes.c_float), ('momentum', ctypes.c_float)]


class _BnSmallBwd(ctypes.Structure):
    _fields_ = [(k, ctypes.c_void_p) for k in ('g', 'y', 'relu_mask', 'x', 'dx', 'mi', 'gamma', 'dgamma', 'dbeta')] + \
               [('M', ctypes.c_int64)] + [(k, ctypes.c_int) for k in ('ldg', 'ldy', 'ldx', 'lddx', 'C', 'groups', 'relu')]


BN_SMALL_MAX_ROWS = 320


def bn_train_small(items, eps=1e-5, momentum=0.1):
    if not items:
        return
    arr = (_BnSmallFwd * len(items))()
    for d, (x, y, mi, rm, rv, nbt, gamma, beta, M, C, relu, groups, rmask) in zip(arr, items):
        d.x, d.y, d.relu_mask, d.gamma, d.beta, d.mi = x.data_ptr(), y.data_ptr(), _p(rmask), gamma.data_ptr(), beta.data_ptr(), mi.data_ptr()
        d.running_mean, d.running_var, d.num_batches_tracked = _p(rm), _p(rv), _p(nbt)
        d.M, d.ldx, d.ldy, d.C, d.groups, d.relu, d.eps, d.momentum = M, _ld(x), _ld(y), C, groups, int(bool(relu)), eps, momentum
    lib().call('rgda_bn_train_small', ctypes.cast(arr, ctypes.c_void_p), len(items), _stream())


def bn_bwd_small(items):
    if not items:
        return
    arr = (_BnSmallBwd * len(items))()
# ... 1260 lines not shown
```

Measured before the change: 431.5 pairs/s.

## Fuse bn3 BatchNorm apply into a recomputed 1x1 conv stream kernel epilogue

```diff
diff --git a/include/rgda_hip.h b/include/rgda_hip.h
--- a/include/rgda_hip.h
+++ b/include/rgda_hip.h
@@ -181,6 +181,11 @@
 int rgda_conv2d_bnin(const rgda_bn_operand* bn_in, const void* x, int ldx, const void* wgt, void* y, int ldy,
                      const void* res, int ldres, rgda_stat_t* stats, int stat_groups, int N, int H, int W, int Cin,
                      int Ho, int Wo, int Cout, int kh, int kw, int stride, int pad, int dil, rgda_stream_t stream);
+int rgda_conv2d_bnapply(const rgda_bn_operand* bn_in, const void* x, int ldx, const void* wgt, const rgda_stat_t* stats,
+                        float* mi, float* running_mean, float* running_var, int64_t* num_batches_tracked,
+                        const float* gamma, const float* beta, const void* res, int ldres, void* y, int ldy,
+                        uint8_t* relu_mask, int relu, int groups, float eps, float momentum, int N, int H, int W, int Cin,
+                        int Ho, int Wo, int Cout, int kh, int kw, int stride, int pad, int dil, rgda_stream_t stream);
 
 const char* rgda_conv2d_kernel(int variant, int N, int H, int W, int Cin, int Ho, int Wo, int Cout, int kh, int kw,
                                int stride, int pad, int dil, int mode, int has_stats, int stat_groups);
diff --git a/regda_amd/csrc/common.h b/regda_amd/csrc/common.h
--- a/regda_amd/csrc/common.h
+++ b/regda_amd/csrc/common.h
@@ -155,6 +155,40 @@
     }
 }
 
+static __device__ __forceinline__ void bn_publish(const rgda_stat_t* __restrict__ stats, int grp, int cc, int C, long long M,
+                                                  double invM, float eps, float mom, int groups, float m, float is,
+                                                  float* mi_out, float* rm, float* rv, long long* nbt) {
+    mi_out[(size_t)grp * 2 * C + cc] = m;
+    mi_out[(size_t)grp * 2 * C + C + cc] = is;
+    if (grp == 0 && rm) {
+        const float unb = (M > 1) ? (float)M / (float)(M - 1) : 1.f;
+        float gm[8], gv[8];
+#pragma unroll
+        for (int g = 0; g < 8; ++g) {
+            if (g < groups) {
+                float gis;
+                stat_moments(stats + (size_t)g * NREP * 2 * C, C, cc, invM, eps, gm[g], gv[g], gis);
+            }
+        }
+        float a = rm[cc], b = rv[cc];
+#pragma unroll
+        for (int g = 0; g < 8; ++g) {
+            if (g < groups) {
+                a = (1.f - mom) * a + mom * gm[g];
+                b = (1.f - mom) * b + mom * gv[g] * unb;
+            }
+        }
+        rm[cc] = a;
+        rv[cc] = b;
+        if (cc == 0 && nbt) *nbt += groups;
+    }
+}
+static __device__ __forceinline__ unsigned char relu_bits(const uint4& v) {
+    auto pos = [](unsigned h) { return (unsigned)((h & 0x7fffu) != 0 && (h & 0x8000u) == 0); };
+    return (unsigned char)(pos(v.x & 0xffffu) | pos(v.x >> 16) << 1 | pos(v.y & 0xffffu) << 2 | pos(v.y >> 16) << 3 |
+                           pos(v.z & 0xffffu) << 4 | pos(v.z >> 16) << 5 | pos(v.w & 0xffffu) << 6 | pos(v.w >> 16) << 7);
+}
+
 #include <stdlib.h>
 #ifdef RGDA_TUNING
 #define TUNE_ENV(name) getenv(name)
diff --git a/regda_amd/csrc/conv_kernels.hip b/regda_amd/csrc/conv_kernels.hip
--- a/regda_amd/csrc/conv_kernels.hip
+++ b/regda_amd/csrc/conv_kernels.hip
@@ -37,6 +37,8 @@
     const float* bn_gamma;
     const float* bn_beta;
     BnOperand xf;
+    BnOperand ap;
+    unsigned char* ap_mask;
 };
 
 #ifdef RGDA_TUNING
@@ -86,7 +88,7 @@
 }
 
 
-enum { EPI_PLAIN = 0, EPI_STATS, EPI_RES, EPI_RES_STATS, EPI_EV, EPI_BNX, EPI_BNX2 };
+enum { EPI_PLAIN = 0, EPI_STATS, EPI_RES, EPI_RES_STATS, EPI_EV, EPI_BNX, EPI_BNX2, EPI_BNAPPLY };
 typedef float f32x2 __attribute__((ext_vector_type(2)));
 typedef __attribute__((ext_vector_type(4))) unsigned u32x4r;
 #define RGDA_BNIN_MAX_C 512
@@ -140,7 +142,8 @@
 }
 template <int BC, int BP, int NT, int KIND, bool FULL = false, int WMAP = 0>
 static __device__ __forceinline__ void epilogue_rows(const ConvArgs& a, const unsigned char* smem, int m0, int c0,
-                                                     float (&s)[8], float (&q)[8], const EpiParams* pre = nullptr) {
+                                                     float (&s)[8], float (&q)[8], const EpiParams* pre = nullptr,
+                                                     const uint4* rpre = nullptr) {
     constexpr int CSTR = BC * 2 + 16;
     constexpr int VPR = BC / 8, RPP = NT / VPR, NIT = BP / RPP;
     constexpr int CH = NIT < 4 ? NIT : 4;
@@ -156,8 +159,8 @@
 #pragma unroll
     for (int e = 0; e < 4; ++e) { s2[e] = f32x2{s[2 * e], s[2 * e + 1]}; q2[e] = f32x2{q[2 * e], q[2 * e + 1]}; }
     constexpr bool BNX = KIND == EPI_BNX || KIND == EPI_BNX2;
-    const bool has_res = (KIND == EPI_RES || KIND == EPI_RES_STATS) || ((KIND == EPI_EV || BNX) && a.res);
-    const bool res_gate = (KIND != EPI_EV) && has_res && a.res_mask;
+    const bool has_res = (KIND == EPI_RES || KIND == EPI_RES_STATS) || ((KIND == EPI_EV || KIND == EPI_BNAPPLY || BNX) && a.res);
+    const bool res_gate = (KIND != EPI_EV && KIND != EPI_BNAPPLY) && has_res && a.res_mask;
     constexpr bool STATS = KIND == EPI_STATS || KIND == EPI_RES_STATS;
 #pragma unroll
     for (int p0 = 0; p0 < NIT; p0 += CH) {
@@ -173,7 +176,7 @@
             rv[i] = uint4{0u, 0u, 0u, 0u}; xv[i] = rv[i]; yv[i] = rv[i]; rmb[i] = 0xffu; bmb[i] = 0xffu;
             if (ok[i]) {
                 if (has_res) {
-                    rv[i] = *(const uint4*)(a.res + (size_t)m * a.ldres + co);
+                    rv[i] = rpre ? rpre[p0 + i] : *(const uint4*)(a.res + (size_t)m * a.ldres + co);
                     if (res_gate) rmb[i] = a.res_mask[(size_t)m * (a.Cout >> 3) + (co >> 3)];
                 }
                 if (BNX) {
@@ -200,6 +203,14 @@
                     f32x2 f = bf2f_pair(vw[e]) * k0[e] + k1[e];
                     if (has_res) f += bf2f_pair(rw[e]);
                     if (a.ev_relu) { f.x = fmaxf(f.x, 0.f); f.y = fmaxf(f.y, 0.f); }
+                    ow[e] = pack2bf(f);
+                }
+            } else if (KIND == EPI_BNAPPLY) {
+#pragma unroll
+                for (int e = 0; e < 4; ++e) {
+                    f32x2 f = __builtin_elementwise_fma(bf2f_pair(vw[e]) - k1[e], k0[e], k2[e]);
+                    if (has_res) f += bf2f_pair(rw[e]);
+                    if (a.ap.relu) { f.x = fmaxf(f.x, 0.f); f.y = fmaxf(f.y, 0.f); }
                     ow[e] = pack2bf(f);
                 }
             } else {
@@ -256,6 +267,8 @@
                     }
                 }
                 if (!(TSKIP(a) & 128)) *(uint4*)(a.y + (size_t)m * a.ldy + co) = uint4{ow[0], ow[1], ow[2], ow[3]};
+                if (KIND == EPI_BNAPPLY && a.ap_mask)
+                    a.ap_mask[(size_t)m * (a.Cout >> 3) + (co >> 3)] = relu_bits(uint4{ow[0], ow[1], ow[2], ow[3]});
             }
         }
     }
@@ -266,7 +279,8 @@
 template <int BC, int BP, int WC, int WP, bool RAW = false, int KIND = -1, int WMAP = 0>
 static __device__ __forceinline__ void conv_epilogue(const ConvArgs& a, f32x16 (&acc)[BC / WC / 32][BP / WP / 32],
                                                      unsigned char* smem, int m0, int c0, float (&s)[8], float (&q)[8],
-                                                     bool flush, int replica, const EpiParams* pre = nullptr) {
+                                                     bool flush, int replica, const EpiParams* pre = nullptr,
+                                                     const uint4* rpre = nullptr) {
     constexpr int NW = WC * WP, NT = 64 * NW;
     constexpr int FI = BC / WC / 32, FJ = BP / WP / 32;
     constexpr int CSTR = BC * 2 + 16;
@@ -297,7 +311,7 @@
     if (TDBG(a) && t == 0) TDBG(a)[(16384 + blockIdx.x) * 4 + 0] = __builtin_readcyclecounter();
     constexpr int VPR = BC / 8;
     const int cv = t % VPR;
-    if constexpr (KIND >= 0) epilogue_rows<BC, BP, NT, KIND, RAW, WMAP>(a, smem, m0, c0, s, q, pre);
+    if constexpr (KIND >= 0) epilogue_rows<BC, BP, NT, KIND, RAW, WMAP>(a, smem, m0, c0, s, q, pre, rpre);
     else if (a.ev_rm) epilogue_rows<BC, BP, NT, EPI_EV, false, WMAP>(a, smem, m0, c0, s, q);
     else if (a.bn_x) {
         if (a.bn_relu == 2) epilogue_rows<BC, BP, NT, EPI_BNX2, false, WMAP>(a, smem, m0, c0, s, q);
@@ -964,8 +978,44 @@
     epilogue_params<KIND>(a, mbase, c0 + (t % (BC / 8)) * 8, true, P);
 #pragma unroll
     for (int e = 0; e < 4; ++e) asm volatile("" ::"v"(P.k0[e]), "v"(P.k1[e]), "v"(P.k2[e]), "v"(P.k3[e]));
+    uint4 rpre[SC];
+#pragma unroll
+    for (int r = 0; r < SC; ++r) rpre[r] = uint4{0u, 0u, 0u, 0u};
+    const bool pre_res = KIND == EPI_BNAPPLY && a.res;
+    auto load_res = [&](int tile) {
+        constexpr int VPR = BC / 8, RPP = 64 * NW / VPR;
+        static_assert(BP / RPP == SC, "one residual vector per row store");
+        const bf16_t* rp = a.res + (size_t)(mbase + tile * BP + t / VPR) * a.ldres + c0 + (t % VPR) * 8;
+#pragma unroll
+        for (int r = 0; r < SC; ++r) rpre[r] = *(const uint4*)(rp + (size_t)r * RPP * a.ldres);
+    };
     issue(0, 0);
-    if (T > 1) { issue(1, 1); WAIT_VMCNT(XL * KC); } else WAIT_VMCNT(0);
+    if constexpr (KIND == EPI_BNAPPLY) {
+        if (pre_res) load_res(0);
+        if (T > 1) issue(1, 1);
+        float* tab = (float*)se;
+        const int rpg = a.rows_per_group, grp = mbase / rpg;
+        if (t < BC) {
+            const double invM = 1.0 / (double)rpg;
+            float m, v0, is;
+            stat_moments(a.ap.stats + (size_t)grp * NREP * 2 * a.Cout, a.Cout, c0 + t, invM, a.ap.eps, m, v0, is);
+            tab[t] = m;
+            tab[BC + t] = is;
+            if (mbase == grp * rpg)
+                bn_publish(a.ap.stats, grp, c0 + t, a.Cout, rpg, invM, a.ap.eps, a.ap.mom, a.ap.groups, m, is, a.ap.mi, a.ap.rm,
+                           a.ap.rv, a.ap.nbt);
+        }
+        __syncthreads();
+        const int cl = (t % (BC / 8)) * 8;
+#pragma unroll
+        for (int e = 0; e < 8; ++e) {
+            P.k1[e >> 1][e & 1] = tab[cl + e];
+            P.k0[e >> 1][e & 1] = tab[BC + cl + e] * a.ap.gamma[c0 + cl + e];
+            P.k2[e >> 1][e & 1] = a.ap.beta[c0 + cl + e];
+        }
+#pragma unroll
+        for (int e = 0; e < 4; ++e) asm volatile("" ::"v"(P.k0[e]), "v"(P.k1[e]), "v"(P.k2[e]));
+    } else if (T > 1) { issue(1, 1); WAIT_VMCNT(XL * KC); } else WAIT_VMCNT(0);
     for (int i = 0; i < T; ++i) {
         const int stage = i & 1;
         __builtin_amdgcn_s_barrier();
@@ -987,8 +1037,11 @@
                 for (int ii = 0; ii < FI; ++ii)
                     acc[ii][0] = __builtin_amdgcn_mfma_f32_32x32x16_bf16(fa[kt * 4 + kk][ii], fb[kk], acc[ii][0], 0, 0, 0);
         }
-        conv_epilogue<BC, BP, WC, WP, true, KIND>(a, acc, se, mbase + i * BP, c0, s, q, i + 1 == T, blockIdx.x & (NREP - 1), &P);
-        __builtin_amdgcn_s_waitcnt(SC | (7 << 4) | (15 << 8));
+        conv_epilogue<BC, BP, WC, WP, true, KIND>(a, acc, se, mbase + i * BP, c0, s, q, i + 1 == T, blockIdx.x & (NREP - 1), &P,
+                                                  KIND == EPI_BNAPPLY ? rpre : nullptr);
+        if (KIND == EPI_BNAPPLY && a.ap_mask) __builtin_amdgcn_s_waitcnt(2 * SC | (7 << 4) | (15 << 8));
+        else __builtin_amdgcn_s_waitcnt(SC | (7 << 4) | (15 << 8));
+        if (pre_res) load_res(i + 1 < T ? i + 1 : i);
         if (i + 2 < T && !(TSKIP(a) & 1)) issue(i + 2, stage);
     }
 #endif
@@ -1133,7 +1186,10 @@
     ROUTE(R_HALOW_1_8_XF, 512, conv3x3_halo_wide_kernel, 1, 8, 3, false, true)                                       \
     PER_EPI_ROUTES(R_C64_, conv3x3_c64_kernel, 128)                                                                  \
     PER_EPI_ROUTES(R_STREAM1_, conv1x1_stream_kernel, 1, 128, 2, 4)                                                  \
-    PER_EPI_ROUTES(R_STREAM2_, conv1x1_stream_kernel, 2, 128, 2, 4)
+    PER_EPI_ROUTES(R_STREAM2_, conv1x1_stream_kernel, 2, 128, 2, 4)                                                  \
+    ROUTE(R_STREAM1_BNAPPLY, 512, conv1x1_stream_kernel, 1, 128, 2, 4, 7)                                            \
+    ROUTE(R_STREAM2_BNAPPLY, 512, conv1x1_stream_kernel, 2, 128, 2, 4, 7)
+static_assert(EPI_BNAPPLY == 7, "the stream kernel's BatchNorm-apply rows name the kind by its number");
 #define ROUTE(ID, BLOCK, KERNEL, ...) ID,
 enum { CONV_ROUTES CONV_ROUTE_COUNT };
 #undef ROUTE
@@ -1209,7 +1265,8 @@
 }
 struct BnBwdFuse { const void* y; int ldy; const unsigned char* mask; const void* x; int ldx; const float* mi; const float* nscale; int rpi; int relu; const float* gamma; const float* beta; };
 struct BnEvalFuse { const float* rm; const float* rv; const float* gamma; const float* beta; float eps; int relu; };
-struct ConvFuse { const BnBwdFuse* bnb; const BnEvalFuse* bne; const rgda_bn_operand* bnin; };
+struct BnApplyFuse { const rgda_stat_t* stats; float* mi; float* rm; float* rv; int64_t* nbt; const float* gamma; const float* beta; uint8_t* mask; int relu; float eps, mom; };
+struct ConvFuse { const BnBwdFuse* bnb; const BnEvalFuse* bne; const rgda_bn_operand* bnin; const BnApplyFuse* bna; };
 
 static int conv_bnin_kind(long long M, int Cout, int Cin, int kh, int kw, int stride, int pad, int dil, int H, int W, int Ho,
                           int Wo, int groups) {
@@ -1242,6 +1299,7 @@
     const BnBwdFuse* bnb = f.bnb;
     const BnEvalFuse* bne = f.bne;
     const rgda_bn_operand* bnin = f.bnin;
+    const BnApplyFuse* bna = f.bna;
     if (!d.x || !d.wgt || !d.y) return RGDA_ERR_ARG;
     if (N <= 0 || H <= 0 || W <= 0 || Ho <= 0 || Wo <= 0 || Cin <= 0 || Cout <= 0 || kh <= 0 || kw <= 0 ||
         stride <= 0 || dil <= 0 || pad < 0 || (mode != 0 && mode != 1))
@@ -1278,6 +1336,16 @@
         a.ev_rm = bne->rm; a.ev_rv = bne->rv; a.ev_gamma = bne->gamma; a.ev_beta = bne->beta; a.ev_eps = bne->eps;
         a.ev_relu = bne->relu;
     }
+    if (bna) {
+        if (mode != 0 || bne || bnb || a.stats || d.res_relu_mask || d.stat_groups < 1 || !bna->stats || !bna->mi || !bna->gamma || !bna->beta ||
+            stat_groups > 8 || M / stat_groups < 2 || (bna->rm == nullptr) != (bna->rv == nullptr) || (bna->mask && !bna->relu))
+            return RGDA_ERR_ARG;
+        if (bnin || kh != 1 || kw != 1) return RGDA_ERR_UNSUPPORTED;
+        a.ap.stats = bna->stats; a.ap.gamma = bna->gamma; a.ap.beta = bna->beta; a.ap.mi = bna->mi; a.ap.rm = bna->rm;
+        a.ap.rv = bna->rv; a.ap.nbt = (long long*)bna->nbt; a.ap.eps = bna->eps; a.ap.mom = bna->mom; a.ap.groups = stat_groups;
+        a.ap.relu = bna->relu; a.ap.C = Cout; a.ap.rows_per_group = a.rows_per_group;
+        a.ap_mask = bna->mask;
+    }
     if (const char* e = TUNE_ENV("RGDA_CONV_DBG")) a.dbg = (unsigned long long*)strtoull(e, nullptr, 0);
     a.skip = tune_int("RGDA_CONV_SKIP", 0);
     if (bnin) {
@@ -1341,14 +1409,16 @@
         const long long tiles_p = M / bp;
         int chunks = (256 * wpc) / tiles_c;
         while (chunks > 1 && ((tiles_p % chunks) || (a.rows_per_group % (int)(tiles_p / chunks * bp)))) chunks >>= 1;
+        while (bna && chunks > 1 && tiles_p / chunks < 4 && !(a.rows_per_group % (int)(tiles_p / (chunks >> 1) * bp))) chunks >>= 1;
         const long long T = chunks >= 1 ? tiles_p / chunks : 0;
         if (!(M % bp) && chunks >= 1 && T >= 4 && T <= 4096 && !(tiles_p % chunks) && !(a.rows_per_group % (int)(T * bp))) {
             a.tiles_c = tiles_c; a.tiles_p = (int)tiles_p; a.tpw = (int)T;
-            p.route = (Cin == 64 ? R_STREAM1_0 : R_STREAM2_0) + conv_epi_kind(a);
+            p.route = bna ? (Cin == 64 ? R_STREAM1_BNAPPLY : R_STREAM2_BNAPPLY) : (Cin == 64 ? R_STREAM1_0 : R_STREAM2_0) + conv_epi_kind(a);
             p.grid = tiles_c * chunks;
             return RGDA_OK;
         }
     }
+    if (bna) return RGDA_ERR_UNSUPPORTED;
     ConvTile t;
     if (pick_tile(M, Cout, (long long)kh * kw * Cin, (a.stats && stat_groups > 1) ? a.rows_per_group : 0, t))
         return RGDA_ERR_UNSUPPORTED;
@@ -1455,6 +1525,17 @@
     if (!bn_in) return RGDA_ERR_ARG;
     return conv_run({x, wgt, y, res, nullptr, stats, ldx, ldy, ldres, stat_groups, N, H, W, Cin, Ho, Wo, Cout, kh, kw, stride, pad,
                      dil, 0}, ConvFuse{nullptr, nullptr, bn_in}, stream);
+}
+
+extern "C" int rgda_conv2d_bnapply(const rgda_bn_operand* bn_in, const void* x, int ldx, const void* wgt,
+                                   const rgda_stat_t* stats, float* mi, float* running_mean, float* running_var,
+                                   int64_t* num_batches_tracked, const float* gamma, const float* beta, const void* res,
+                                   int ldres, void* y, int ldy, uint8_t* relu_mask, int relu, int groups, float eps,
+                                   float momentum, int N, int H, int W, int Cin, int Ho, int Wo, int Cout, int kh, int kw,
+                                   int stride, int pad, int dil, rgda_stream_t stream) {
+    const BnApplyFuse b = {stats, mi, running_mean, running_var, num_batches_tracked, gamma, beta, relu_mask, relu, eps, momentum};
+    return conv_run({x, wgt, y, res, nullptr, nullptr, ldx, ldy, ldres, groups, N, H, W, Cin, Ho, Wo, Cout, kh, kw, stride, pad,
+                     dil, 0}, ConvFuse{nullptr, nullptr, bn_in, &b}, stream);
 }
 
 extern "C" int rgda_conv2d_bnbwd(const void* x, int ldx, const void* wgt, void* y, int ldy, const void* res, int ldres,
diff --git a/regda_amd/csrc/norm_kernels.hip b/regda_amd/csrc/norm_kernels.hip
--- a/regda_amd/csrc/norm_kernels.hip
+++ b/regda_amd/csrc/norm_kernels.hip
@@ -61,11 +61,6 @@
 #ifndef RB_CLS
 #define RB_CLS ROW_BATCH
 #endif
-static __device__ __forceinline__ unsigned char relu_bits(const uint4& v) {
-    auto pos = [](unsigned h) { return (unsigned)((h & 0x7fffu) != 0 && (h & 0x8000u) == 0); };
-    return (unsigned char)(pos(v.x & 0xffffu) | pos(v.x >> 16) << 1 | pos(v.y & 0xffffu) << 2 | pos(v.y >> 16) << 3 |
-                           pos(v.z & 0xffffu) << 4 | pos(v.z >> 16) << 5 | pos(v.w & 0xffffu) << 6 | pos(v.w >> 16) << 7);
-}
 static __device__ __forceinline__ void store8(bf16_t* p, const float (&f)[8]) {
     uint4 v;
     v.x = pack2bf(f[0], f[1]); v.y = pack2bf(f[2], f[3]); v.z = pack2bf(f[4], f[5]); v.w = pack2bf(f[6], f[7]);
@@ -194,32 +189,7 @@
                 stat_moments(st, C, cc, invM, eps, m, v0, is);
                 smean[c] = m;
                 sistd[c] = is;
-                if (chunk == 0) {
-                    mi_out[(size_t)grp * 2 * C + cc] = m;
-                    mi_out[(size_t)grp * 2 * C + C + cc] = is;
-                    if (grp == 0 && rm) {
-                        const float unb = (M > 1) ? (float)M / (float)(M - 1) : 1.f;
-                        float gm[8], gv[8];
-#pragma unroll
-                        for (int g = 0; g < 8; ++g) {
-                            if (g < groups) {
-                                float gis;
-                                stat_moments(stats + (size_t)g * NREP * 2 * C, C, cc, invM, eps, gm[g], gv[g], gis);
-                            }
-                        }
-                        float a = rm[cc], b = rv[cc];
-#pragma unroll
-                        for (int g = 0; g < 8; ++g) {
-                            if (g < groups) {
-                                a = (1.f - mom) * a + mom * gm[g];
-                                b = (1.f - mom) * b + mom * gv[g] * unb;
-                            }
-                        }
-                        rm[cc] = a;
-                        rv[cc] = b;
-                        if (cc == 0 && nbt) *nbt += groups;
-                    }
-                }
+                if (chunk == 0) bn_publish(stats, grp, cc, C, M, invM, eps, mom, groups, m, is, mi_out, rm, rv, nbt);
             }
         }
         __syncthreads();
diff --git a/regda_amd/models/Encoder.py b/regda_amd/models/Encoder.py
--- a/regda_amd/models/Encoder.py
+++ b/regda_amd/models/Encoder.py
@@ -369,7 +369,8 @@
         self.group_small_convs = True
         self.small_bn = True
         self.bn_on_operand = True
-        self.bn_operand_units = {'stem', 'bn1', 'bn2'}
+        self.bn_operand_units = {'stem', 'bn1', 'bn2', 'bn3'}
+        self._bnapply_served = {}
         self.bn_operand_level = 2
         self._head_stream = None
         self._mat_cache = {}
@@ -760,8 +761,20 @@
         mi = torch.empty(G, 2, conv.co, device=self.device)
         y = torch.empty(M, conv.co, dtype=BF, device=self.device)
         rmask = self._relu_mask(relu, M, conv.co)
-        ops.bn_train_apply(c, stats, mi, bn.rm, bn.rv, bn.nbt, bn.gamma, bn.beta, y, M, conv.co, relu, res, nscale,
-                           Ho * Wo, groups=G, relu_mask=rmask)
+        fused = False
+        if (res is not None and nscale is None and geom is None and preconv is None and not isinstance(x, _Lazy)
+                and self.bn_on_operand and 'bn3' in self.bn_operand_units and conv.k == 1 and conv.stride == 1
+                and conv.ci in (64, 128) and self._bnapply_served.get((M, conv.ci, conv.co, G), True)):
+            try:
+                ops.conv2d_bnapply(x, conv.wb if wb is None else wb, stats, mi, bn.rm, bn.rv, bn.nbt, bn.gamma, bn.beta, y,
+                                   N, H, W, Ho, Wo, conv.k, conv.k, conv.stride, conv.pad, conv.dil, relu, res, groups=G,
+                                   relu_mask=rmask)
+                fused = True
+            except ValueError:
+                self._bnapply_served[(M, conv.ci, conv.co, G)] = False
+        if not fused:
+            ops.bn_train_apply(c, stats, mi, bn.rm, bn.rv, bn.nbt, bn.gamma, bn.beta, y, M, conv.co, relu, res, nscale,
+                               Ho * Wo, groups=G, relu_mask=rmask)
         T[key] = _Unit(x, c, y, mi, (N, H, W, Ho, Wo), nscale, rmask)
         return y, Ho, Wo
 
diff --git a/regda_amd/ops.py b/regda_amd/ops.py
--- a/regda_amd/ops.py
+++ b/regda_amd/ops.py
@@ -697,6 +697,15 @@
     lib().call('rgda_conv2d_bnin', bnop, x.data_ptr(), _ld(x), w.data_ptr(), y.data_ptr(), _ld(y), _p(res),
                _ld(res) if res is not None else 0, _stat(stats), stat_groups, N, H, W, Cin, Ho, Wo, Cout, kh, kw, stride, pad,
                dil, _stream())
+
+
+def conv2d_bnapply(x, w, stats, mi, rm, rv, nbt, gamma, beta, y, N, H, W, Ho, Wo, kh, kw, stride, pad, dil, relu, res=None,
+                   groups=1, eps=1e-5, momentum=0.1, relu_mask=None, bnop=None):
+    Cout, taps, Cin = w.shape
+    assert taps == kh * kw and x.shape[1] == Cin and y.shape[1] == Cout
+    lib().call('rgda_conv2d_bnapply', bnop, x.data_ptr(), _ld(x), w.data_ptr(), _stat(stats), mi.data_ptr(), _p(rm), _p(rv),
+               _p(nbt), gamma.data_ptr(), beta.data_ptr(), _p(res), _ld(res) if res is not None else 0, y.data_ptr(), _ld(y),
+               _p(relu_mask), int(relu), groups, eps, momentum, N, H, W, Cin, Ho, Wo, Cout, kh, kw, stride, pad, dil, _stream())
 
 
 def conv2d_wgrad(x, dy, dw, N, H, W, Ho, Wo, kh, kw, stride, pad, dil):
```

After: 428.6 pairs/s. No clear change (-0.7%).
